# InternetMaximalism/plonky2_bn254

Measured on AMD Instinct MI355X. Metric: G1 scalar-mul STARK proofs/sec (256-bit scalars), higher is better.
Workload: dtype u64 (Goldilocks p = 2^64-2^32+1; BN254 Fq as 10x26-bit Montgomery limbs); 1 GPU; configs[1]: batch of 1024 G1 scalar-muls on 1 GPU per step = 8 proofs x 128 instances, 2^16 rows, W=781, standard_fast_config; instances_per_proof=128, steps_in_flight=4, parallelism=1 GPU, no collective

## Files before the change

### include/bn254_stark.h

```cpp
#ifndef BN254_STARK_H
#define BN254_STARK_H

#include <stddef.h>
#include <stdint.h>

#ifdef __cplusplus
extern "C" {
#endif

#define BN254S_ABI_VERSION 1

enum {
  BN254S_OK = 0,
  BN254S_E_INVALID_ARG = -1,
  BN254S_E_HIP = -2,
  BN254S_E_OOM = -3,
  BN254S_E_INVALID_POINT = -4,
  BN254S_E_UNSUPPORTED = -5,
  BN254S_E_TRANSCRIPT = -6,
  BN254S_E_INTERNAL = -7,
  BN254S_E_VERIFY = -8
};

typedef struct bn254s_ctx bn254s_ctx;
// ... 49 lines not shown
  BN254S_SEC_AUX_CAP = 1,
  BN254S_SEC_QUOTIENT_CAP = 2,
  BN254S_SEC_LOCAL_VALUES = 3,
  BN254S_SEC_NEXT_VALUES = 4,
  BN254S_SEC_AUX_POLYS = 5,
  BN254S_SEC_AUX_POLYS_NEXT = 6,
  BN254S_SEC_CTL_ZS_FIRST = 7,
  BN254S_SEC_QUOTIENT_POLYS = 8,
  BN254S_SEC_FRI_CAPS = 9,
  BN254S_SEC_QUERY_ROUNDS = 10,
  BN254S_SEC_FINAL_POLY = 11,
  BN254S_SEC_POW_WITNESS = 12,
  BN254S_SEC_INIT_CHALLENGER_STATE = 13,
  BN254S_SEC_COUNT = 14
};
int bn254s_proof_section(const bn254s_proof* p, int id, const uint64_t** data, size_t* len);
int bn254s_proof_degree_bits(const bn254s_proof* p);
int bn254s_proof_outputs(const bn254s_proof* p, const uint64_t** data, size_t* len);
int bn254s_proof_stage_ms(const bn254s_proof* p, const float** ms, size_t* n_stages);
const char* bn254s_stage_name(size_t stage);
size_t bn254s_proof_serialize(const bn254s_proof* p, uint8_t* buf, size_t cap);
void bn254s_proof_free(bn254s_proof* p);

int bn254s_verify(bn254s_ctx* ctx, int kind, const bn254s_params* params, uint32_t degree_bits, const uint64_t* words,
                  size_t n_words, const uint64_t* scalars, const uint64_t* x, const uint64_t* offset, const uint64_t* outputs,
                  size_t n);
int bn254s_verify_host(int kind, const bn254s_params* params, uint32_t degree_bits, const uint64_t* words, size_t n_words,
                       const uint64_t* scalars, const uint64_t* x, const uint64_t* offset, const uint64_t* outputs, size_t n,
                       char* err_buf, size_t err_cap);

int bn254s_verify_batch(bn254s_ctx* ctx, int kind, const bn254s_params* params, uint32_t degree_bits, const uint64_t* const* words,
                        size_t n_words, const uint64_t* scalars, const uint64_t* x, const uint64_t* offset, const uint64_t* outputs,
                        const size_t* n_jobs, size_t n_proofs, int32_t* status, char* err, size_t err_stride);

int bn254s_ctl_values(int kind, const uint64_t* scalars, const uint64_t* x, const uint64_t* offset, const uint64_t* outputs,
                      size_t n, uint64_t* in_rows, uint64_t* out_rows);

int bn254s_map_to_g2(bn254s_ctx* ctx, const bn254s_params* params, const uint64_t* u, const uint64_t* offsets, size_t n,
                     uint64_t* out_points, uint64_t* fq_jobs, uint64_t* g2_jobs, bn254s_proof** fq_proofs,
                     bn254s_proof** g2_proofs);

int bn254s_hash_to_fq2(const uint64_t* input, size_t len, uint64_t* out );
int bn254s_hash_to_fq2_batch(bn254s_ctx* ctx, const uint64_t* inputs, size_t n, size_t len, uint64_t* out);

int bn254s_g1_msm_chain(bn254s_ctx* ctx, const uint64_t* scalars , const uint64_t* x ,
                        const uint64_t* offset , size_t n, uint64_t* offsets_out, uint64_t* result );
int bn254s_g1_msm(bn254s_ctx* ctx, const bn254s_params* params, const uint64_t* scalars, const uint64_t* x,
                  const uint64_t* offset, size_t n, size_t per_proof, uint64_t* result, uint64_t* offsets_out,
                  bn254s_proof** proofs);
int bn254s_g2_msm_chain(bn254s_ctx* ctx, const uint64_t* scalars , const uint64_t* x ,
                        const uint64_t* offset , size_t n, uint64_t* offsets_out ,
                        uint64_t* result );
int bn254s_g2_msm(bn254s_ctx* ctx, const bn254s_params* params, const uint64_t* scalars, const uint64_t* x,
                  const uint64_t* offset, size_t n, size_t per_proof, uint64_t* result, uint64_t* offsets_out,
                  bn254s_proof** proofs);

int bn254s_g1_recover_from_x_batch(bn254s_ctx* ctx, const uint64_t* xs , size_t n,
                                   uint64_t* points_out , uint8_t* flags_out ,
                                   uint64_t* fq_jobs );
int bn254s_g1_recover_from_x(bn254s_ctx* ctx, const bn254s_params* params, const uint64_t* xs, size_t n, size_t per_proof,
                             uint64_t* points_out, uint8_t* flags_out, uint64_t* fq_jobs ,
                             bn254s_proof** fq_proofs);
int bn254s_g2_recover_from_x_batch(bn254s_ctx* ctx, const uint64_t* xs ,
                                   const uint8_t* sgns , size_t n,
                                   uint64_t* points_out , uint8_t* flags_out ,
                                   uint64_t* fq_jobs );
int bn254s_g2_recover_from_x(bn254s_ctx* ctx, const bn254s_params* params, const uint64_t* xs, const uint8_t* sgns, size_t n,
                             size_t per_proof, uint64_t* points_out, uint8_t* flags_out, uint64_t* fq_jobs ,
                             bn254s_proof** fq_proofs);
int bn254s_fq_sqrt_batch(bn254s_ctx* ctx, const uint64_t* xs ,
                         const uint8_t* sgns , size_t n, uint64_t* roots_out ,
                         uint8_t* square_out , uint8_t* root_ok_out ,
                         uint64_t* fq_jobs );
int bn254s_fq2_sqrt_batch(bn254s_ctx* ctx, const uint64_t* xs ,
                          const uint8_t* sgns , size_t n, uint64_t* roots_out ,
                          uint8_t* square_out , uint8_t* root_ok_out ,
                          uint64_t* fq_jobs );
int bn254s_fq_sqrt(bn254s_ctx* ctx, const bn254s_params* params, const uint64_t* xs, const uint8_t* sgns, size_t n, size_t per_proof,
                   uint64_t* roots_out, uint8_t* square_out, uint8_t* root_ok_out, uint64_t* fq_jobs ,
                   bn254s_proof** fq_proofs );
int bn254s_fq2_sqrt(bn254s_ctx* ctx, const bn254s_params* params, const uint64_t* xs, const uint8_t* sgns, size_t n, size_t per_proof,
                    uint64_t* roots_out, uint8_t* square_out, uint8_t* root_ok_out, uint64_t* fq_jobs ,
                    bn254s_proof** fq_proofs );
int bn254s_fq_inv_batch(bn254s_ctx* ctx, const uint64_t* xs , size_t n, uint64_t* out );
int bn254s_fq2_inv_batch(bn254s_ctx* ctx, const uint64_t* xs , size_t n, uint64_t* out );
int bn254s_g2_subgroup_check_batch(bn254s_ctx* ctx, const uint64_t* points , size_t n,
                                   uint8_t* flags_out );
int bn254s_g2_subgroup_check(bn254s_ctx* ctx, const bn254s_params* params, const uint64_t* points ,
                             const uint64_t* offsets , size_t n, size_t per_proof, uint8_t* flags_out ,
                             uint64_t* g2_jobs , bn254s_proof** g2_proofs);
int bn254s_g2_clear_cofactor_batch(bn254s_ctx* ctx, const uint64_t* points , size_t n,
                                   uint64_t* images_out , uint8_t* finite_out );
int bn254s_g2_clear_cofactor(bn254s_ctx* ctx, const bn254s_params* params, const uint64_t* points ,
                             const uint64_t* offsets , size_t n, size_t per_proof, uint64_t* images_out ,
                             uint8_t* finite_out , uint64_t* g2_jobs ,
                             bn254s_proof** g2_proofs);
int bn254s_map_to_g2_batch(bn254s_ctx* ctx, const uint64_t* u , size_t n,
                           uint64_t* out_points );
int bn254s_hash_to_g2_batch(bn254s_ctx* ctx, const uint64_t* inputs , size_t n, size_t len,
                            uint64_t* out_points );
int bn254s_hash_to_fq(const uint64_t* input, size_t len, uint64_t* out );
int bn254s_hash_to_fq_batch(bn254s_ctx* ctx, const uint64_t* inputs, size_t n, size_t len, uint64_t* out );
int bn254s_map_to_g1_batch(bn254s_ctx* ctx, const uint64_t* u , size_t n,
                           uint64_t* out_points , uint8_t* sq_flags ,
                           uint64_t* fq_jobs );
int bn254s_hash_to_g1_batch(bn254s_ctx* ctx, const uint64_t* inputs , size_t n, size_t len,
                            uint64_t* out_points );
int bn254s_map_to_g1(bn254s_ctx* ctx, const bn254s_params* params, const uint64_t* u , size_t n, size_t per_proof,
                     uint64_t* out_points , uint8_t* sq_flags ,
                     uint64_t* fq_jobs , bn254s_proof** fq_proofs );
int bn254s_job_outputs_batch(bn254s_ctx* ctx, int kind, const uint64_t* scalars , const uint64_t* x,
                             const uint64_t* offset, size_t n, uint64_t* outputs_out ,
                             uint8_t* finite_out );
int bn254s_job_outputs(bn254s_ctx* ctx, int kind, const bn254s_params* params, const uint64_t* scalars, const uint64_t* x,
                       const uint64_t* offset, size_t n, size_t per_proof, uint64_t* outputs_out, bn254s_proof** proofs_out);
#define BN254S_JOB_STEP_NONE 0xFFFFu
int bn254s_job_check_batch(bn254s_ctx* ctx, int kind, const uint64_t* scalars , const uint64_t* x, const uint64_t* offset,
                           size_t n, uint8_t* provable_out , uint16_t* step_out );
int bn254s_prove_batch_checked(bn254s_ctx* ctx, int kind, const bn254s_params* params, const uint64_t* scalars,
                               const uint64_t* x, const uint64_t* offset, size_t n_total, size_t per_proof,
                               uint8_t* provable_out , uint16_t* step_out ,
                               bn254s_proof** proofs_out);
int bn254s_commit_values(bn254s_ctx* ctx, const uint64_t* values, size_t ncols, uint64_t* coeffs, uint64_t* lde,
                         uint64_t* cap);
int bn254s_bench_ntt(bn254s_ctx* ctx, size_t ncols, int iters, float* ms);
int bn254s_bench_ntt_clock(bn254s_ctx* ctx, size_t ncols, int iters, float* ms, float* mhz, float* mhz_min);
int bn254s_bench_issue(bn254s_ctx* ctx, float* ns_per_issue, float* mhz);
int bn254s_bench_copy(bn254s_ctx* ctx, size_t words, int iters);
int bn254s_bench_leafhash(bn254s_ctx* ctx, size_t ncols, int log_leaves, int iters, float* ms);
int bn254s_poseidon_permute(bn254s_ctx* ctx, uint64_t* states, size_t n);
int bn254s_selftest_field(bn254s_ctx* ctx, const uint64_t* a, const uint64_t* b, size_t n, uint64_t* out);
int bn254s_selftest_poseidon(bn254s_ctx* ctx, int variant, uint64_t* states, size_t n);
int bn254s_selftest_leaf_hash(bn254s_ctx* ctx, const uint64_t* data, size_t ncols, int log_leaves, int kernel, int chunk_cols,
                              uint64_t* digests);
int bn254s_selftest_fq_inv(bn254s_ctx* ctx, const uint64_t* x, size_t n, uint64_t* out);
int bn254s_selftest_fq(bn254s_ctx* ctx, int group, const uint64_t* in, size_t n, uint64_t* out);
int bn254s_selftest_logup(bn254s_ctx* ctx, const uint64_t* trace, size_t rows, int ncols, int rc_begin, int n_rc, int table_col,
                          int freq_col, const uint64_t betas[2], uint64_t* out);
int bn254s_selftest_acc(bn254s_ctx* ctx, const uint64_t* values, const uint64_t* weights, size_t T, size_t rows, uint64_t* out);
int bn254s_selftest_openings(bn254s_ctx* ctx, const uint64_t* coeffs, int npolys, int log_r, const uint64_t zeta[2],
                             const uint64_t zeta_next[2], uint64_t* out);
int bn254s_selftest_fri_combine(bn254s_ctx* ctx, int mode, int W, int n_rc, int n_ctl, size_t n, const uint64_t* cols,
                                const uint64_t* aux_in, const uint64_t* points, uint64_t* out);
int bn254s_selftest_fri_fold(bn254s_ctx* ctx, const uint64_t* in, int log_m, uint64_t shift, const uint64_t beta[2], uint64_t* out);
int bn254s_selftest_fri_rows(bn254s_ctx* ctx, const uint64_t* lde, int ncols, int log_n, int h, size_t k0, size_t rows,
                             const uint32_t* indices, int nq, uint64_t* window, uint64_t* gathered);
#define BN254S_QS_WINDOW 1
#define BN254S_QS_RAW 2
#define BN254S_QS_MAX_PARTS 7
int bn254s_selftest_quotient(bn254s_ctx* ctx, int kind, int log_n, int flags, int h, size_t k0, size_t count, size_t stride,
                             const uint64_t* trace, const uint64_t* aux, const uint64_t alphas[2], const uint64_t betas[2],
                             const uint64_t gammas[2], const uint64_t* x, const uint64_t* lfirst, const uint64_t* llast, uint64_t* out,
                             uint64_t* part);
int bn254s_selftest_point_tables(bn254s_ctx* ctx, int log_n, int window, int h, size_t k0, size_t count, uint64_t* out);
int bn254s_selftest_aux(bn254s_ctx* ctx, int kind, const uint64_t* trace, size_t rows, const uint64_t betas[2], const uint64_t gammas[2],
                        uint64_t* out);
int bn254s_selftest_transforms(bn254s_ctx* ctx, int op, int log_n, int flags, int ncols, int coset_mask, const uint64_t* in,
                               uint64_t* out0, uint64_t* out1);
int bn254s_selftest_mul_2exp(bn254s_ctx* ctx, const uint64_t* x, size_t n, uint64_t* out);
int bn254s_selftest_outer_dft(bn254s_ctx* ctx, int log_r, int inverse, const uint64_t* in, size_t n, uint64_t* out);
#define BN254S_VERIFY_RECORD_HEAD 34
int bn254s_selftest_verify_front(int kind, const bn254s_params* params, uint32_t degree_bits, const uint64_t* words, size_t n_words,
                                 uint64_t* record_out, size_t record_cap);
int bn254s_selftest_query_round(bn254s_ctx* ctx, int kind, const bn254s_params* params, uint32_t degree_bits,
                                const uint64_t* const* words, size_t n_words, const uint64_t* records, size_t n_proofs,
                                size_t chunk_proofs, int32_t* codes_out);
const char* bn254s_selftest_query_text(int n_layers, int code);
int bn254s_selftest_verify_batch_ms(bn254s_ctx* ctx, float ms_out[5]);
#define BN254S_PLAN_WORDS 54
int bn254s_selftest_proof_plan(int kind, size_t n, const bn254s_params* params, uint64_t dev_total_bytes, int force_split,
                               int force_lowmem, int force_stream, int stream_win_log, uint64_t* out, char* err, size_t err_len);
int bn254s_generate_trace(bn254s_ctx* ctx, int kind, const uint64_t* scalars, const uint64_t* x, const uint64_t* offset,
                          size_t n, uint32_t min_rows_log2, uint64_t* trace_out, uint64_t* outputs);
int bn254s_g1_generate_trace(bn254s_ctx* ctx, const uint64_t* scalars, const uint64_t* x, const uint64_t* offset,
                             size_t n, uint32_t min_rows_log2, uint64_t* trace_out, uint64_t* outputs);

#ifdef __cplusplus
}
#endif
#endif
```

### plonky2_bn254_amd/csrc/proof_plan.h

```cpp
#pragma once
#include <string>
#include "aux.h"
#include "fri.h"
#include "ntt.h"

struct PlanOverrides {
  bool force_split = false, force_lowmem = false, force_stream = false;
  int stream_win_log = -1;
};
PlanOverrides plan_overrides_from_env();

struct PlanBuffers {
  size_t in, tvals, tcoef, hist, tmp, ldechunk, sponge, comb, tlde, trees, avals, acoef, alde, scratch, quot, tabs, open, fri,
      fritrees, qout;
  size_t win;
};

struct ProofPlan {
  static constexpr int NQ = 4, CAPW = 64;
  static constexpr int CH = 16;
  int kind = 0;
  size_t n = 0;
  bn254s_params P;
  StarkShape sh;
  int W = 0, A = 0, K = 0, PW = 0;
  size_t N = 0, M2 = 0;
  unsigned log_n = 0, log_m2 = 0;
  unsigned log_s = 0, log_r = 0;
  size_t R = 1, NH = 0;
  int NSPL = 1;
  bool stream = false, lowmem = false;
  unsigned log_bk = 0;
  size_t BK = 0, WROWS = 0;
  int L = 0, arities[FRI_MAX_LAYERS] = {0};
  size_t wpq = 0;
  size_t tree_words = 0, fri_words = 0, fri_tree_words = 0, in_words = 0;
  PlanBuffers words = {};
  size_t pinned_bytes = 0;
  size_t ntt_tmp_words(int width) const { return ntt_scratch_words(log_n, log_s != 0, lowmem ? CH : width); }
  size_t n_part() const { return (size_t)(W + A + NQ) * NSPL * R * 5; }
  size_t n_q() const { return wpq * P.num_queries; }
};

int proof_plan(int kind, size_t n, const bn254s_params& P, size_t dev_total_bytes, const PlanOverrides& ov, ProofPlan& pl,
               std::string& err);
size_t rows_for(size_t n, uint32_t min_rows_log2);
```

### plonky2_bn254_amd/csrc/proof_plan.hip

```cpp
#include <algorithm>
#include <cstdlib>
#include <cstring>
#include "proof_plan.h"
#include "merkle.h"
#include "prover.h"

static bool env_flag(const char* name) { return getenv(name) && atoi(getenv(name)); }
PlanOverrides plan_overrides_from_env() {
  PlanOverrides ov;
  ov.force_split = env_flag("BN254S_FORCE_SPLIT");
  ov.force_lowmem = env_flag("BN254S_FORCE_LOWMEM");
  ov.force_stream = env_flag("BN254S_FORCE_STREAM");
  if (const char* e = getenv("BN254S_STREAM_WIN_LOG")) ov.stream_win_log = atoi(e) < 0 ? 99 : atoi(e);
  return ov;
}

size_t rows_for(size_t n, uint32_t min_rows_log2) {
  size_t r = std::max((size_t)1 << min_rows_log2, n * 512), p = 1;
  while (p < r) p <<= 1;
  return p;
}

int proof_plan(int kind, size_t n, const bn254s_params& P, size_t dev_total_bytes, const PlanOverrides& ov, ProofPlan& pl,
               std::string& err) {
  const StarkKind& sk = stark_kind(kind);
  pl.kind = kind;
  pl.n = n;
  pl.P = P;
  const StarkShape& sh = pl.sh = sk.shape;
  const int W = pl.W = sh.W, A = pl.A = sh.n_aux(), K = pl.K = sh.n_total_constraints(), PW = pl.PW = sk.point_words;
  const int NQ = ProofPlan::NQ, CH = ProofPlan::CH;
  const size_t N = pl.N = rows_for(n, P.min_rows_log2);
  unsigned log_n = 0;
  while (((size_t)1 << log_n) < N) log_n++;
  pl.log_n = log_n;
  if (log_n < 16 || log_n > 23) {
    err = "supported trace heights: 2^16 .. 2^23 rows (up to 16384 instances in one proof)";
    return BN254S_E_UNSUPPORTED;
  }
  if (P.num_challenges != 2 || P.rate_bits != 1 || P.cap_height != 4 || P.arity_bits != 4 || P.min_rows_log2 < 16 ||
      P.pow_bits == 0 || P.pow_bits > 32 || P.num_queries == 0 || P.num_queries > 256) {
    err = "unsupported StarkConfig (only standard_fast_config shapes)";
    return BN254S_E_UNSUPPORTED;
  }
  const unsigned log_s = pl.log_s = (log_n == 23 || (ov.force_split && log_n >= 18)) ? 1 : 0;
  const unsigned log_m2 = pl.log_m2 = log_n + 1, log_r = pl.log_r = log_n - 16 - log_s;
  const size_t R = pl.R = (size_t)1 << log_r;
  const size_t M2 = pl.M2 = 2 * N;
  pl.NH = N >> log_s;
  const int NSPL = pl.NSPL = 1 << log_s;
  const double plain_bytes = 8.0 * (double)N * (4.0 * sh.W + 4.0 * sh.n_aux() + std::max(sh.W, sh.n_aux()));
  const double compact_bytes = 8.0 * ((double)std::max((size_t)sh.W * N, (size_t)sh.n_aux() * 2 * N) + (double)sh.W * N * 3.0 + (double)sh.n_aux() * N);
  const bool stream = pl.stream =
      log_n > 16 && (ov.force_stream || (dev_total_bytes > 0 && compact_bytes + 20e9 > (double)dev_total_bytes));
  const bool lowmem = pl.lowmem = stream || log_s || (log_n > 16 && (ov.force_lowmem || plain_bytes > 200e9));
  pl.log_bk = std::min(22u, log_n - 1);
  if (ov.stream_win_log >= 0) pl.log_bk = std::min(log_n, std::max(8u, (unsigned)ov.stream_win_log));
  pl.BK = (size_t)1 << pl.log_bk;
  const size_t WROWS = pl.WROWS = pl.BK + 1;
  const std::vector<int> arities = fri_arities(P, log_n);
  const int L = pl.L = (int)arities.size();
  if (L > FRI_MAX_LAYERS) return BN254S_E_UNSUPPORTED;
  std::copy(arities.begin(), arities.end(), pl.arities);

  PlanBuffers& b = pl.words = PlanBuffers{};
  pl.in_words = n * (4 + 2 * (size_t)PW);
  b.in = pl.in_words + 16;
  b.tvals = lowmem && !stream ? std::max((size_t)W * N, (size_t)A * M2) : (size_t)W * N;
  b.tcoef = (size_t)W * N;
  b.hist = 65536 / 2;
  b.tmp = pl.ntt_tmp_words(std::max(W, A));
  b.ldechunk = stream ? (size_t)CH * M2 : 0;
  b.sponge = stream ? (size_t)12 * M2 : 0;
  b.comb = (size_t)6 * N + (size_t)6 * M2;
  b.tlde = stream ? 0 : (size_t)W * M2;
  pl.tree_words = merkle_tree_digests(log_m2, P.cap_height) * 4;
  b.trees = 3 * pl.tree_words;
  b.avals = (size_t)A * N;
  b.acoef = lowmem ? 0 : (size_t)A * N;
  b.alde = lowmem ? 0 : (size_t)A * M2;
  b.scratch = std::max(sk.trace_scratch_words(n), aux_scratch_words(sh, N));
  b.quot = (size_t)(3 * NQ) * N + (size_t)NQ * M2 + (size_t)QUOTIENT_MAX_PARTS * 2 * (stream ? WROWS : M2);
  b.tabs = QUOTIENT_W_WORDS(K) + QUOTIENT_MZT_WORDS + 4 * (size_t)(W + A + NQ);
  b.open = std::max((size_t)(W + A + NQ) * NSPL * R * 5 + FRI_OPENING_TABLE_WORDS, n * (size_t)PW);
  pl.fri_words = pl.fri_tree_words = 0;
  {
    size_t m = M2;
    for (int l = 0; l <= L; l++) {
      pl.fri_words += 2 * m;
      if (l < L) pl.fri_tree_words += merkle_tree_digests((int)log_m2 - 4 * (l + 1), P.cap_height) * 4;
      m >>= 4;
    }
  }
  b.fri = pl.fri_words;
  b.fritrees = pl.fri_tree_words;
  pl.wpq = (size_t)(W + A + NQ) + 3 * 4 * (log_m2 - P.cap_height);
  {
    int lg = log_m2;
    for (int l = 0; l < L; l++) {
      lg -= arities[l];
      pl.wpq += 32 + 4 * (lg - P.cap_height);
    }
  }
  b.qout = pl.n_q() + 64;
  b.win = stream ? (size_t)(W + A) * WROWS + 3 * WROWS + (size_t)(W + A) * P.num_queries : 0;
  pl.pinned_bytes = std::max(pl.n_part(), pl.n_q()) * 8;
  return BN254S_OK;
}

extern "C" int bn254s_selftest_proof_plan(int kind, size_t n, const bn254s_params* params, uint64_t dev_total_bytes, int force_split,
                                          int force_lowmem, int force_stream, int stream_win_log, uint64_t* out, char* err,
                                          size_t err_len) {
  if (kind < 0 || kind > 2 || n == 0 || !params || params->struct_size != sizeof(bn254s_params) || !out) return BN254S_E_INVALID_ARG;
  PlanOverrides ov;
  ov.force_split = force_split != 0;
  ov.force_lowmem = force_lowmem != 0;
  ov.force_stream = force_stream != 0;
  ov.stream_win_log = stream_win_log;
  ProofPlan pl;
  std::string msg;
  const int rc = proof_plan(kind, n, *params, (size_t)dev_total_bytes, ov, pl, msg);
  if (err && err_len) {
    strncpy(err, msg.c_str(), err_len - 1);
    err[err_len - 1] = 0;
  }
  if (rc != BN254S_OK) return rc;
  const PlanBuffers& b = pl.words;
  const uint64_t head[] = {(uint64_t)pl.kind, pl.n, (uint64_t)pl.W, (uint64_t)pl.A, (uint64_t)pl.K, (uint64_t)pl.PW, pl.N, pl.log_n, pl.log_s,
                           pl.log_r, pl.R, pl.NH, (uint64_t)pl.NSPL, pl.stream, pl.lowmem, pl.log_bk, pl.BK, pl.WROWS, (uint64_t)pl.L};
  const uint64_t tail[] = {pl.wpq, pl.tree_words, pl.fri_words, pl.fri_tree_words, pl.in_words,
                           b.in, b.tvals, b.tcoef, b.hist, b.tmp, b.ldechunk, b.sponge, b.comb, b.tlde, b.trees, b.avals, b.acoef,
                           b.alde, b.scratch, b.quot, b.tabs, b.open, b.fri, b.fritrees, b.qout, b.win, pl.pinned_bytes};
  static_assert(sizeof(head) / 8 + FRI_MAX_LAYERS + sizeof(tail) / 8 == BN254S_PLAN_WORDS, "bn254s_selftest_proof_plan layout");
  for (uint64_t v : head) *out++ = v;
  for (int l = 0; l < FRI_MAX_LAYERS; l++) *out++ = (uint64_t)pl.arities[l];
  for (uint64_t v : tail) *out++ = v;
  return BN254S_OK;
}
```

### plonky2_bn254_amd/csrc/prover.hip

```cpp
#include <algorithm>
#include <atomic>
#include <cstring>
#include <thread>
#include "ctx.h"
#include "trace.h"
#include "aux.h"
#include "merkle.h"
#include "quotient.h"
#include "fri.h"
#include "transcript.h"
#include "prover.h"
#include "proof_plan.h"
#include "transforms.h"

template <class L>
static StarkShape make_shape(bool input_has_a, int n_constraints) {
  StarkShape s;
  s.W = L::W;
  s.rc_begin = L::RC_BEGIN;
  s.rc_end = L::RC_END;
  s.table_col = L::RANGE;
  s.freq_col = L::FREQ;
  s.n_ctl = 2;
  s.n_constraints = n_constraints;
  memset(&s.ctl, 0, sizeof(s.ctl));
  int m = 0;
  for (int i = 0; i < L::PL; i++, m++) { s.ctl.col_start[0][m] = L::B + i; s.ctl.col_bits[0][m] = 1; }
  if (input_has_a)
    for (int i = 0; i < L::PL; i++, m++) { s.ctl.col_start[0][m] = L::A + i; s.ctl.col_bits[0][m] = 1; }
  for (int k = 0; k < 16; k++, m++) { s.ctl.col_start[0][m] = L::BITS + 16 * k; s.ctl.col_bits[0][m] = 16; }
  s.ctl.col_start[0][m] = L::TIMESTAMP; s.ctl.col_bits[0][m] = 1; m++;
  s.ctl.ncols[0] = m;
  s.ctl.filter_col[0] = L::FLAGS + 0;
  m = 0;
  for (int i = 0; i < L::PL; i++, m++) { s.ctl.col_start[1][m] = L::SUM + i; s.ctl.col_bits[1][m] = 1; }
  s.ctl.col_start[1][m] = L::TIMESTAMP; s.ctl.col_bits[1][m] = 1; m++;
  s.ctl.ncols[1] = m;
  s.ctl.filter_col[1] = L::FLAGS + 1;
  return s;
}
static int fq_generate_trace_no_offset(const u64* d_scalars, const u64* d_x, const u64*, size_t n, u64* d_trace, size_t N,
                                       u64* d_scratch, u64* d_outputs, int* d_err, hipStream_t st, bool with_range) {
  return fq_generate_trace_device(d_scalars, d_x, n, d_trace, N, d_scratch, d_outputs, d_err, st, with_range);
}
const StarkKind& stark_kind(int kind) {
  static const StarkKind kinds[3] = {
      {make_shape<G1L>(true, 1111), 8, true, g1_trace_scratch_words, g1_generate_trace_device, g1_quotient_mz_blocks, g1_quotient_launch},
      {make_shape<G2L>(true, 1693), 16, true, g2_trace_scratch_words, g2_generate_trace_device, g2_quotient_mz_blocks, g2_quotient_launch},
      {make_shape<FQL>(false, 770), 4, false, fq_trace_scratch_words, fq_generate_trace_no_offset, fq_quotient_mz_blocks, fq_quotient_launch}};
  return kinds[kind];
}

enum { ST_TRACE = 0, ST_TRACE_NTT, ST_TRACE_MERKLE, ST_AUX, ST_AUX_NTT, ST_AUX_MERKLE, ST_QUOTIENT, ST_QUOTIENT_COMMIT,
       ST_OPENINGS, ST_FRI, ST_TOTAL, ST_COUNT };
static const char* STAGE_NAMES[ST_COUNT] = {"trace_gen", "trace_ntt", "trace_merkle", "aux_columns", "aux_ntt", "aux_merkle",
                                            "quotient", "quotient_commit", "openings", "fri", "total"};

struct bn254s_proof {
  std::vector<u64> words, outputs;
  size_t sec_off[BN254S_SEC_COUNT + 1] = {0};
  int degree_bits = 0;
  float stage_ms[ST_COUNT] = {0};
};

std::vector<int> fri_arities(const bn254s_params& P, int degree_bits) {
  std::vector<int> a;
  int d = degree_bits;
  while (d > (int)P.final_poly_bits && d + (int)P.rate_bits - (int)P.arity_bits >= (int)P.cap_height) {
    a.push_back(P.arity_bits);
    d -= P.arity_bits;
  }
  return a;
}

__global__ __launch_bounds__(256) void k_quotient_chunks(const u64* __restrict__ ab, u64* __restrict__ out, size_t N, u64 inv2,
                                                         u64 inv2c) {
  size_t i = (size_t)blockIdx.x * blockDim.x + threadIdx.x;
  if (i >= N) return;
  int a = blockIdx.y;
  u64 A = ab[(size_t)(a * 2 + 0) * N + i], B = ab[(size_t)(a * 2 + 1) * N + i];
  out[(size_t)(a * 2 + 0) * N + i] = gl_mul(gl_add(A, B), inv2);
  out[(size_t)(a * 2 + 1) * N + i] = gl_mul(gl_sub(A, B), inv2c);
}

#define CHK(call)                                              \
  do {                                                         \
    hipError_t e_ = (call);                                    \
    if (e_ != hipSuccess) {                                    \
      err = std::string(#call) + ": " + hipGetErrorString(e_); \
      return BN254S_E_HIP;                                     \
    }                                                          \
  } while (0)

struct BigSection {
  bn254s_ctx* c;
  hipStream_t st;
  int cls;
  BigSection(bn254s_ctx* c_, hipStream_t st_, int cls_) : c(c_), st(st_), cls(cls_) { c->big_lock(cls); }
  ~BigSection() {
    hipStreamSynchronize(st);
    c->big_unlock(cls);
  }
};

static int get_point_tables(bn254s_ctx* c, unsigned log_n, QPointTables& pt) {
  static std::mutex mu;
  std::lock_guard<std::mutex> lk(mu);
  std::string key = "pt." + std::to_string(log_n);
  bool fresh = !c->has(key);
  size_t M2 = (size_t)2 << log_n;
  u64* p = c->words(key, 3 * M2);
  if (!p) return BN254S_E_OOM;
  if (fresh) {
    quotient_point_tables(p, p + M2, p + 2 * M2, log_n, c->stream);
    if (hipStreamSynchronize(c->stream) != hipSuccess) return BN254S_E_HIP;
  }
  pt.x = p;
  pt.lfirst = p + M2;
  pt.llast = p + 2 * M2;
  return 0;
}

struct Workspace {
  Slot* sl = nullptr;
  const ProofPlan* pl = nullptr;
  u64 *in, *tvals, *tcoef, *hist, *tmp, *ldechunk, *sponge, *comb, *tlde, *trees, *avals, *acoef, *alde, *scr, *quot, *tabs, *open,
      *fri, *fritrees, *qout;
  int* err;
  unsigned long long* pow;
  u32* qidx;
  u64 *ttree, *atree, *qtree;
  u64 *qv, *ab, *qcoef, *qlde, *qpart;
  u64 *W, *mzt, *apow;
  size_t cap_off;
  u64 *tw = nullptr, *aw = nullptr, *wpt = nullptr, *qrows = nullptr;
  int begin_windows(std::string& err);
};

static int workspace_acquire(Slot& sl, const ProofPlan& pl, Workspace& ws, std::string& err) {
  BufPool& mem = sl.mem;
  const PlanBuffers& b = pl.words;
  const bool stream = pl.stream, lowmem = pl.lowmem;
  ws.sl = &sl;
  ws.pl = &pl;
  if (lowmem) {
    mem.drop("acoef");
    mem.drop("alde");
  }
  ws.in = mem.words("in", b.in);
  ws.tvals = mem.words("tvals", b.tvals);
  ws.tcoef = mem.words("tcoef", b.tcoef);
  ws.hist = mem.words("hist", b.hist);
  ws.tmp = mem.words("tmp", b.tmp);
  mem.drop("win");
  if (stream) {
    mem.drop("tlde");
    mem.drop("alde");
    mem.drop("acoef");
  } else {
    mem.drop("ldechunk");
    mem.drop("sponge");
  }
  ws.ldechunk = stream ? mem.words("ldechunk", b.ldechunk) : nullptr;
  ws.sponge = stream ? mem.words("sponge", b.sponge) : nullptr;
  ws.comb = mem.words("comb", b.comb);
  ws.tlde = stream ? ws.ldechunk : mem.words("tlde", b.tlde);
  ws.trees = mem.words("trees", b.trees);
  ws.avals = mem.words("avals", b.avals);
  ws.acoef = lowmem ? ws.avals : mem.words("acoef", b.acoef);
  ws.alde = stream ? ws.ldechunk : lowmem ? ws.tvals : mem.words("alde", b.alde);
  ws.scr = mem.words("scratch", b.scratch);
  ws.quot = mem.words("quot", b.quot);
  ws.tabs = mem.words("tabs", b.tabs);
  ws.open = mem.words("open", b.open);
  ws.fri = mem.words("fri", b.fri);
  ws.fritrees = mem.words("fritrees", b.fritrees);
  ws.qout = mem.words("qout", b.qout);
  if (sl.pinned_bytes < pl.pinned_bytes) {
    if (sl.pinned) hipHostFree(sl.pinned);
    sl.pinned = nullptr;
    sl.pinned_bytes = 0;
    CHK(hipHostMalloc(&sl.pinned, pl.pinned_bytes));
    sl.pinned_bytes = pl.pinned_bytes;
  }
  if (!ws.hist || !ws.in || !ws.tvals || !ws.tcoef || !ws.tmp || !ws.tlde || !ws.trees || !ws.avals || !ws.acoef || !ws.alde ||
      !ws.scr || !ws.quot || !ws.tabs || !ws.open || !ws.fri || !ws.fritrees || !ws.qout || !ws.comb ||
      (stream && (!ws.ldechunk || !ws.sponge))) {
    err = mem.err;
    mem.release();
    return BN254S_E_OOM;
  }
  {
    static const size_t reserve = (size_t)(getenv("BN254S_MEM_RESERVE_MB") ? atol(getenv("BN254S_MEM_RESERVE_MB")) : 6144) << 20;
    size_t free_b = 0, total_b = 0;
    if (hipMemGetInfo(&free_b, &total_b) == hipSuccess && free_b < reserve) {
      err = "device memory: " + std::to_string(free_b >> 20) + " MB would be left free, below the reserve of " +
            std::to_string(reserve >> 20) + " MB kept for the runtime's own allocations";
      mem.release();
      return BN254S_E_OOM;
    }
  }
  const size_t N = pl.N, M2 = pl.M2;
  const int NQ = ProofPlan::NQ;
  ws.err = (int*)(ws.in + pl.in_words);
  ws.pow = (unsigned long long*)(ws.in + pl.in_words + 2);
  ws.qidx = (u32*)(ws.qout + pl.n_q());
  ws.ttree = ws.trees;
  ws.atree = ws.trees + pl.tree_words;
  ws.qtree = ws.trees + 2 * pl.tree_words;
  ws.qv = ws.quot;
  ws.ab = ws.quot + (size_t)NQ * N;
  ws.qcoef = ws.quot + (size_t)2 * NQ * N;
  ws.qlde = ws.quot + (size_t)3 * NQ * N;
  ws.qpart = ws.qlde + (size_t)NQ * M2;
  ws.W = ws.tabs;
  ws.mzt = ws.tabs + QUOTIENT_W_WORDS(pl.K);
  ws.apow = ws.mzt + QUOTIENT_MZT_WORDS;
  ws.cap_off = 4 * merkle_level_offset(pl.log_m2, pl.log_m2 - pl.P.cap_height);
  return BN254S_OK;
}

int Workspace::begin_windows(std::string& err) {
  BufPool& mem = sl->mem;
  const size_t WROWS = pl->WROWS;
  CHK(hipStreamSynchronize(sl->st));
  mem.drop("tvals");
  tvals = nullptr;
  u64* win = mem.words("win", pl->words.win);
  if (!win) {
    err = mem.err;
    mem.release();
    return BN254S_E_OOM;
  }
  tw = win;
  aw = win + (size_t)pl->W * WROWS;
  wpt = aw + (size_t)pl->A * WROWS;
  qrows = wpt + 3 * WROWS;
  return BN254S_OK;
}

struct Run {
  bn254s_ctx* c;
  Slot& sl;
  hipStream_t st;
  const ProofPlan& pl;
  Workspace& ws;
  const Transforms& tf;
  QPointTables pt;
  void sb(int stage) const { hipEventRecord(sl.events[2 * stage], st); }
  void se(int stage) const { hipEventRecord(sl.events[2 * stage + 1], st); }
  int mmode() const { return c->workers.in_flight.load(std::memory_order_relaxed) >= 4 ? MERKLE_THROUGHPUT : MERKLE_LATENCY; }
};

static int upload_and_generate(const StarkKind& sk, const u64* scalars, const u64* x, const u64* off, size_t n, u64* d_in, u64* d_trace,
                               size_t N, u64* d_scr, u64* d_outs, int* d_err, hipStream_t st, bool with_range, std::string& err) {
  const size_t PW = sk.point_words;
  u64* d_sc = d_in;
  u64* d_x = d_in + 4 * n;
  u64* d_off = d_x + PW * n;
  CHK(hipMemcpyAsync(d_sc, scalars, n * 32, hipMemcpyHostToDevice, st));
  CHK(hipMemcpyAsync(d_x, x, n * PW * 8, hipMemcpyHostToDevice, st));
  if (sk.has_offset) CHK(hipMemcpyAsync(d_off, off, n * PW * 8, hipMemcpyHostToDevice, st));
  if (sk.generate_trace(d_sc, d_x, d_off, n, d_trace, N, d_scr, d_outs, d_err, st, with_range)) {
    err = "trace generation launch failed";
    return BN254S_E_HIP;
  }
  return BN254S_OK;
}

static int stage_trace(const Run& r, const u64* scalars, const u64* x, const u64* off, bn254s_proof* pr, int* h_err, std::string& err) {
  const ProofPlan& pl = r.pl;
  const Workspace& ws = r.ws;
  const StarkShape& sh = pl.sh;
  hipStream_t st = r.st;
  r.sb(ST_TRACE);
  CHK(hipMemsetAsync(ws.err, 0, 16, st));
  u64* d_outs = ws.open;
  if (int rc = upload_and_generate(stark_kind(pl.kind), scalars, x, off, pl.n, ws.in, ws.tvals, pl.N, ws.scr, d_outs, ws.err, st, false, err))
    return rc;
  {
    BigSection big(r.c, st, BIG_EXCL);
    launch_range_columns(ws.tvals, pl.N, sh.rc_begin, sh.rc_end, sh.freq_col, sh.table_col, (u32*)ws.hist, ws.err, st);
  }
  pr->outputs.resize(pl.n * (size_t)pl.PW);
  CHK(hipMemcpyAsync(pr->outputs.data(), d_outs, pl.n * (size_t)pl.PW * 8, hipMemcpyDeviceToHost, st));
  CHK(hipMemcpyAsync(h_err, ws.err, 4, hipMemcpyDeviceToHost, st));
  r.se(ST_TRACE);
  return BN254S_OK;
}

static void hash_sections(const Run& r, const u64* lde, int width, u64* tree, int stage) {
  bn254s_ctx* c = r.c;
  const size_t M2 = r.pl.M2;
  const int S = r.pl.log_n == 16 ? c->hash_split : 1;
  if (S <= 1) {
    BigSection big(c, r.st, BIG_HASH);
    r.sb(stage);
    merkle_leaves(lde, 1, M2, width, r.pl.log_m2, tree, r.st);
    return;
  }
  const size_t cnt = M2 / S;
  for (int k = 0; k < S; k++) {
    BigSection big(c, r.st, BIG_HASH_PART);
    if (k == 0) r.sb(stage);
    merkle_leaves_range(lde, 1, M2, width, (size_t)k * cnt, cnt, tree, r.st);
  }
}

static int commit(const Run& r, const u64* vals, u64* coef, u64* lde, int width, u64* tree, int ntt_stage, int merkle_stage,
                  u64* cap_out, std::string& err) {
  const ProofPlan& pl = r.pl;
  hipStream_t st = r.st;
  if (pl.stream) {
    BigSection big(r.c, st, BIG_NTT);
    r.sb(ntt_stage);
    r.tf.commit_stream(vals, coef, width, tree);
    r.se(ntt_stage);
    r.sb(merkle_stage);
  } else {
    {
      BigSection big(r.c, st, BIG_NTT);
      r.sb(ntt_stage);
      r.tf.commit_ntt(vals, coef, lde, width);
      r.se(ntt_stage);
    }
    hash_sections(r, lde, width, tree, merkle_stage);
  }
  merkle_upper(pl.log_m2, pl.P.cap_height, tree, st, r.mmode());
  CHK(hipMemcpyAsync(cap_out, tree + r.ws.cap_off, ProofPlan::CAPW * 8, hipMemcpyDeviceToHost, st));
  r.se(merkle_stage);
  CHK(hipStreamSynchronize(st));
  return BN254S_OK;
}

static void stage_aux(const Run& r, const u64 betas[2], const u64 gammas[2]) {
  BigSection big(r.c, r.st, BIG_EXCL);
  r.sb(ST_AUX);
  aux_build(r.pl.sh, r.ws.tvals, r.pl.N, betas, gammas, r.ws.avals, r.ws.scr, r.ws.err, r.st);
  r.se(ST_AUX);
}

static void quotient_over_windows(const Run& r, const u64 betas[2], const u64 gammas[2]) {
  const ProofPlan& pl = r.pl;
  const Workspace& ws = r.ws;
  hipStream_t st = r.st;
  const size_t N = pl.N, M2 = pl.M2, BK = pl.BK, WROWS = pl.WROWS;
  BigSection big(r.c, st, BIG_NTT);
  r.sb(ST_QUOTIENT);
  QPointTables wpt;
  wpt.x = ws.wpt;
  wpt.lfirst = ws.wpt + WROWS;
  wpt.llast = ws.wpt + 2 * WROWS;
  for (int h = 0; h < 2; h++)
    for (size_t k0 = 0; k0 < N; k0 += BK) {
      r.tf.for_lde_chunks(ws.tcoef, pl.W, 1 << h, [&](int c0, int cn) {
        fri_extract_window(ws.ldechunk, M2, pl.log_n, h, k0, WROWS, cn, ws.tw + (size_t)c0 * WROWS, st);
      });
      r.tf.for_lde_chunks(ws.acoef, pl.A, 1 << h, [&](int c0, int cn) {
        fri_extract_window(ws.ldechunk, M2, pl.log_n, h, k0, WROWS, cn, ws.aw + (size_t)c0 * WROWS, st);
      });
      quotient_point_tables_window(ws.wpt, ws.wpt + WROWS, ws.wpt + 2 * WROWS, pl.log_n, h, k0, WROWS, st);
      QArgs QA;
      quotient_fill_args(QA, pl.sh, nullptr, nullptr, ws.W, ws.mzt, r.pt, betas, gammas, pl.log_n, ws.qv, ws.qpart);
      quotient_window_args(QA, ws.tw, ws.aw, wpt, ws.qpart, WROWS, BK, k0, h);
      stark_kind(pl.kind).quotient_launch(QA, pl.sh, st);
    }
}

static int stage_quotient(const Run& r, const u64 alphas[2], const u64 betas[2], const u64 gammas[2], u64* cap_out, std::string& err) {
  const ProofPlan& pl = r.pl;
  const Workspace& ws = r.ws;
  const StarkKind& sk = stark_kind(pl.kind);
  hipStream_t st = r.st;
  const size_t N = pl.N;
  {
    std::vector<u64> hW, hmzt;
    const int* mz_e0 = nullptr;
    const int nblk = sk.mz_blocks(&mz_e0);
    quotient_host_tables(pl.K, alphas, mz_e0, nblk, hW, hmzt);
    CHK(hipMemcpyAsync(ws.W, hW.data(), hW.size() * 8, hipMemcpyHostToDevice, st));
    CHK(hipMemcpyAsync(ws.mzt, hmzt.data(), hmzt.size() * 8, hipMemcpyHostToDevice, st));
    CHK(hipStreamSynchronize(st));
  }
  if (pl.stream) {
    quotient_over_windows(r, betas, gammas);
  } else {
    BigSection big(r.c, st, BIG_EXCL);
    r.sb(ST_QUOTIENT);
    QArgs QA;
    quotient_fill_args(QA, pl.sh, ws.tlde, ws.alde, ws.W, ws.mzt, r.pt, betas, gammas, pl.log_n, ws.qv, ws.qpart);
    sk.quotient_launch(QA, pl.sh, st);
  }
  r.tf.quotient_coset_inverse(ws.qv, ws.ab);
  {
    u64 gn = gl_pow(GL_GEN, N);
    u64 inv2 = gl_inv(2), inv2c = gl_inv(gl_mul(2, gn));
    dim3 g((unsigned)((N + 255) / 256), 2);
    k_quotient_chunks<<<g, 256, 0, st>>>(ws.ab, ws.qcoef, N, inv2, inv2c);
  }
  r.se(ST_QUOTIENT);
  r.sb(ST_QUOTIENT_COMMIT);
  r.tf.lde(ws.qcoef, ws.qlde, ProofPlan::NQ);
  merkle_build(ws.qlde, 1, pl.M2, ProofPlan::NQ, pl.log_m2, pl.P.cap_height, ws.qtree, st, r.mmode());
  CHK(hipMemcpyAsync(cap_out, ws.qtree + ws.cap_off, ProofPlan::CAPW * 8, hipMemcpyDeviceToHost, st));
  r.se(ST_QUOTIENT_COMMIT);
  CHK(hipStreamSynchronize(st));
  return BN254S_OK;
}

static int stage_openings(const Run& r, gl2 zeta, gl2 zeta_next, u64* h_part, std::string& err) {
  const ProofPlan& pl = r.pl;
  const Workspace& ws = r.ws;
  hipStream_t st = r.st;
  const int W = pl.W, A = pl.A, NQ = ProofPlan::NQ, NSPL = pl.NSPL;
  const size_t R = pl.R, NH = pl.NH;
  {
    BigSection big(r.c, st, BIG_EXCL);
    r.sb(ST_OPENINGS);
    u64* d_otab = ws.open + pl.n_part();
    fri_opening_tables(pl.log_r, pl.log_s ? gl2_mul(zeta, zeta) : zeta, pl.log_s ? gl2_mul(zeta_next, zeta_next) : zeta_next, d_otab, st);
    fri_openings(ws.tcoef, NH, pl.log_r, W * NSPL, d_otab, ws.open, st);
    fri_openings(ws.acoef, NH, pl.log_r, A * NSPL, d_otab, ws.open + (size_t)W * NSPL * R * 5, st);
    fri_openings(ws.qcoef, NH, pl.log_r, NQ * NSPL, d_otab, ws.open + (size_t)(W + A) * NSPL * R * 5, st);
  }
  CHK(hipMemcpyAsync(h_part, ws.open, pl.n_part() * 8, hipMemcpyDeviceToHost, st));
  r.se(ST_OPENINGS);
  CHK(hipStreamSynchronize(st));
  return BN254S_OK;
}

static std::vector<u64> recombine_openings(const ProofPlan& pl, const u64* h_part, gl2 zeta, gl2 zeta_next) {
  const size_t R = pl.R;
  const int NSPL = pl.NSPL, n_polys = pl.W + pl.A + ProofPlan::NQ;
  std::vector<u64> h_open((size_t)n_polys * 5);
  std::vector<gl2> zp0(R), zp1(R);
  gl2 a = gl2_make(1, 0), b = gl2_make(1, 0);
  const gl2 y0 = pl.log_s ? gl2_mul(zeta, zeta) : zeta, y1 = pl.log_s ? gl2_mul(zeta_next, zeta_next) : zeta_next;
  for (size_t k1 = 0; k1 < R; k1++) {
    zp0[k1] = a;
    zp1[k1] = b;
    a = gl2_mul(a, y0);
    b = gl2_mul(b, y1);
  }
  for (int p = 0; p < n_polys; p++) {
    gl2 v0 = gl2_make(0, 0), v1 = gl2_make(0, 0);
    u64 s1 = 0;
    for (int half = 0; half < NSPL; half++) {
      gl2 e0 = gl2_make(0, 0), e1 = gl2_make(0, 0);
      for (size_t k1 = 0; k1 < R; k1++) {
        const u64* q = &h_part[(((size_t)p * NSPL + half) * R + k1) * 5];
        e0 = gl2_add(e0, gl2_mul(zp0[k1], gl2_make(q[0], q[1])));
        e1 = gl2_add(e1, gl2_mul(zp1[k1], gl2_make(q[2], q[3])));
        s1 = gl_add(s1, q[4]);
      }
      v0 = gl2_add(v0, half ? gl2_mul(zeta, e0) : e0);
      v1 = gl2_add(v1, half ? gl2_mul(zeta_next, e1) : e1);
    }
    u64* o5 = &h_open[(size_t)p * 5];
    o5[0] = v0.c0; o5[1] = v0.c1; o5[2] = v1.c0; o5[3] = v1.c1; o5[4] = s1;
  }
  return h_open;
}

struct Openings {
  const ProofPlan& pl;
  const std::vector<u64>& h_open;
  u64 operator()(int p, int k) const { return h_open[(size_t)p * 5 + k]; }
  int n_ctlz() const { return 2 * pl.sh.n_ctl; }
  u64 ctl_z_first(int i) const { return (*this)(pl.W + pl.sh.n_lookup_cols() + i, 4); }
};

static void observe_openings(Challenger& ch, const Openings& op) {
  const int W = op.pl.W, A = op.pl.A, NQ = ProofPlan::NQ;
  for (int p = 0; p < W + A + NQ; p++) {
    ch.observe(op(p, 0));
    ch.observe(op(p, 1));
  }
  for (int p = 0; p < W + A; p++) {
    ch.observe(op(p, 2));
    ch.observe(op(p, 3));
  }
  for (int i = 0; i < op.n_ctlz(); i++) {
    ch.observe(op.ctl_z_first(i));
    ch.observe(0);
  }
}

struct FriAlphaPowers {
  std::vector<u32> apow;
  gl2 r0, r1, r2;
};
static FriAlphaPowers fri_alpha_powers(const Openings& op, gl2 fri_alpha) {
  const int W = op.pl.W, A = op.pl.A, NQ = ProofPlan::NQ, n_ctlz = op.n_ctlz();
  FriAlphaPowers f;
  f.apow.assign(8 * (size_t)(W + A + NQ), 0);
  gl2 ap = gl2_make(1, 0);
  f.r0 = f.r1 = f.r2 = gl2_make(0, 0);
  for (int p = 0; p < W + A + NQ; p++) {
    fri_weight_record(&f.apow[8 * (size_t)p], ap);
    f.r0 = gl2_add(f.r0, gl2_mul(ap, gl2_make(op(p, 0), op(p, 1))));
    if (p < W + A) f.r1 = gl2_add(f.r1, gl2_mul(ap, gl2_make(op(p, 2), op(p, 3))));
    if (p < n_ctlz) f.r2 = gl2_add(f.r2, gl2_mul_base(ap, op.ctl_z_first(p)));
    ap = gl2_mul(ap, fri_alpha);
  }
  return f;
}

static int stage_fri_combine(const Run& r, const FriAlphaPowers& f, gl2 zeta, gl2 zeta_next, gl2 fri_alpha, std::string& err) {
  const ProofPlan& pl = r.pl;
  const Workspace& ws = r.ws;
  hipStream_t st = r.st;
  CHK(hipMemcpyAsync(ws.apow, f.apow.data(), f.apow.size() * 4, hipMemcpyHostToDevice, st));
  CHK(hipStreamSynchronize(st));
  BigSection big(r.c, st, BIG_EXCL);
  r.sb(ST_FRI);
  fri_combine_coeffs(pl.sh, ws.tcoef, ws.acoef, ws.qcoef, ws.apow, pl.N, ws.comb, st);
  r.tf.lde(ws.comb, ws.comb + (size_t)6 * pl.N, 6);
  fri_combine_final(pl.sh, ws.comb + (size_t)6 * pl.N, r.pt.x, zeta, zeta_next, f.r0, f.r1, f.r2, fri_alpha, pl.M2, ws.fri, st);
  return BN254S_OK;
}

struct FriLayers {
  std::vector<std::vector<u64>> caps;
  std::vector<const u64*> vals, trees;
  const u64* last = nullptr;
  u64 shift = GL_GEN;
  unsigned lm = 0;
};

static int stage_fri_commit(const Run& r, Challenger& ch, FriLayers& fl, std::string& err) {
  const ProofPlan& pl = r.pl;
  hipStream_t st = r.st;
  const int L = pl.L, CAPW = ProofPlan::CAPW;
  fl.caps.assign(L, std::vector<u64>(CAPW));
  fl.vals.resize(L);
  fl.trees.resize(L);
  u64* vals = r.ws.fri;
  u64* ftree = r.ws.fritrees;
  fl.shift = GL_GEN;
  unsigned lm = pl.log_m2;
  const u64 inv16 = gl_inv(16);
  for (int l = 0; l < L; l++) {
    const int lg = (int)lm - 4;
// ... 535 lines not shown
```

### plonky2_bn254_amd/csrc/quotient.h

```cpp
#pragma once
#include <vector>
#include "quotient_sched.h"

void quotient_point_tables(u64* d_x, u64* d_lfirst, u64* d_llast, unsigned log_n, hipStream_t st);
void quotient_point_tables_window(u64* d_x, u64* d_lfirst, u64* d_llast, unsigned log_n, int h, size_t k0, size_t count, hipStream_t st);
void quotient_window_args(QArgs& A, const u64* d_tw, const u64* d_aw, const QPointTables& pt, u64* d_part, size_t stride, size_t count,
                          size_t k0, int h);
int g1_quotient_mz_blocks(const int** e0);
int g2_quotient_mz_blocks(const int** e0);
int fq_quotient_mz_blocks(const int** e0);
void g1_quotient_launch(const QArgs& A, const StarkShape& sh, hipStream_t st);
void g2_quotient_launch(const QArgs& A, const StarkShape& sh, hipStream_t st);
void fq_quotient_launch(const QArgs& A, const StarkShape& sh, hipStream_t st);
```

### plonky2_bn254_amd/csrc/quotient_common.h

```cpp
#pragma once
#include "gl_dev.h"
#include "aux.h"

struct Acc {
  u64 lo, hi;
  u32 ov;
};
__device__ __forceinline__ void acc_init(Acc& a) {
  a.lo = 0;
  a.hi = 0;
  a.ov = 0;
}
__device__ __forceinline__ void acc_mad(Acc& a, u64 x, u64 w) {
  const unsigned __int128 pr = (unsigned __int128)x * w;
  u64 pl = (u64)pr, ph = (u64)(pr >> 64);
  a.lo += pl;
  u64 c = a.lo < pl ? 1 : 0;
  u64 h = a.hi + ph;
  u32 o = h < ph ? 1 : 0;
  h += c;
  o += h < c ? 1 : 0;
  a.hi = h;
  a.ov += o;
}
__device__ __forceinline__ u64 acc_red(const Acc& a) {
  return gl_sub(gl_reduce128(a.lo, a.hi), ((u64)a.ov) << 32);
}
struct Acc2 {
  Acc a0, a1;
};
__device__ __forceinline__ void acc2_init(Acc2& a) {
  acc_init(a.a0);
  acc_init(a.a1);
}
__device__ __forceinline__ void acc2_mad(Acc2& a, u64 x, u64 w0, u64 w1) {
  acc_mad(a.a0, x, w0);
  acc_mad(a.a1, x, w1);
}

static constexpr u32 M22 = (1u << 22) - 1;
struct W3 {
  u32 w0, w1, w2;
};
GL_HD W3 w3_split(u64 w) {
  W3 r;
  r.w0 = (u32)w & M22;
  r.w1 = (u32)(w >> 22) & M22;
  r.w2 = (u32)(w >> 44);
  return r;
}
struct Acc3 {
  u64 c[5];
};
__device__ __forceinline__ void acc3_init(Acc3& a) {
#pragma unroll
  for (int k = 0; k < 5; k++) a.c[k] = 0;
}
__device__ __forceinline__ void acc3_mad(Acc3& a, u32 v0, u32 v1, u32 v2, u32 w0, u32 w1, u32 w2) {
  a.c[0] += (u64)v0 * w0;
  a.c[1] += (u64)v0 * w1;
  a.c[1] += (u64)v1 * w0;
  a.c[2] += (u64)v0 * w2;
  a.c[2] += (u64)v1 * w1;
  a.c[2] += (u64)v2 * w0;
  a.c[3] += (u64)v1 * w2;
  a.c[3] += (u64)v2 * w1;
  a.c[4] += (u64)v2 * w2;
}
__device__ __forceinline__ u64 acc3_red(const Acc3& a) {
  unsigned __int128 t = (unsigned __int128)a.c[0] + ((unsigned __int128)a.c[1] << 22) + ((unsigned __int128)a.c[2] << 44);
  u64 r = gl_reduce128((u64)t, (u64)(t >> 64));
  r = gl_add(r, gl_mul_2exp<66>(gl_reduce128(a.c[3], 0)));
  r = gl_add(r, gl_mul_2exp<88>(gl_reduce128(a.c[4], 0)));
  return r;
}

struct AccW {
  Acc3 a0, a1;
};
__device__ __forceinline__ void accw_init(AccW& a) {
  acc3_init(a.a0);
  acc3_init(a.a1);
}
template <class WP>
__device__ __forceinline__ void accw_mad(AccW& a, u64 x, WP w) {
  const u32 v0 = (u32)x & M22, v1 = (u32)(x >> 22) & M22, v2 = (u32)(x >> 44);
  acc3_mad(a.a0, v0, v1, v2, w[0], w[1], w[2]);
  acc3_mad(a.a1, v0, v1, v2, w[4], w[5], w[6]);
}
GL_HD void w3_store(u64* dst , u64 wa, u64 wb) {
  const W3 a = w3_split(wa), b = w3_split(wb);
  dst[0] = (u64)a.w0 | ((u64)a.w1 << 32);
  dst[1] = (u64)a.w2;
  dst[2] = (u64)b.w0 | ((u64)b.w1 << 32);
  dst[3] = (u64)b.w2;
}

struct QPointTables {
  const u64* x;
  const u64* lfirst;
  const u64* llast;
};

__device__ __forceinline__ size_t next_position(size_t j, unsigned log_n) {
  const size_t N = (size_t)1 << log_n;
  size_t h = j >> log_n;
  u32 k = bitrev32((u32)(j & (N - 1)), log_n);
  k = (k + 1) & (u32)(N - 1);
  return (h << log_n) | bitrev32(k, log_n);
}

__device__ __forceinline__ void lookup_and_ctl_constraints(const StarkShape& sh, const u64* __restrict__ tl,
                                                           const u64* __restrict__ al, size_t M2, size_t j, size_t jn,
                                                           const u32* __restrict__ W3 , int e0,
                                                           const u64 betas[2], const u64 gammas[2], u64 lfirst, u64 llast,
                                                           u64 z_last, u64& tot0, u64& tot1) {
  const int m = sh.n_helpers(), n_rc = sh.n_rc();
  int e = e0;
  AccW acc;
  accw_init(acc);
  const u64 table = tl[(size_t)sh.table_col * M2 + j], freq = tl[(size_t)sh.freq_col * M2 + j];
  u64 hs[2] = {0, 0};
#pragma unroll 4
  for (int k = 0; k < m; k++) {
    u64 f0 = tl[(size_t)(sh.rc_begin + 2 * k) * M2 + j];
    bool two = (2 * k + 1) < n_rc;
    u64 f1 = two ? tl[(size_t)(sh.rc_begin + 2 * k + 1) * M2 + j] : 0;
#pragma unroll
    for (int ch = 0; ch < 2; ch++) {
      u64 h = al[(size_t)(ch * (m + 1) + k) * M2 + j];
      u64 g0 = gl_add(f0, betas[ch]);
      u64 c;
      if (two) {
        u64 g1 = gl_add(f1, betas[ch]);
        c = gl_sub(gl_sub(gl_mul(gl_mul(g1, g0), h), g1), g0);
      } else {
        c = gl_sub(gl_mul(g0, h), 1);
      }
      int ee = e0 + ch * (m + 2) + k;
      accw_mad(acc, c, W3 + 8 * (ee));
      hs[ch] = gl_add(hs[ch], h);
    }
  }
#pragma unroll
  for (int ch = 0; ch < 2; ch++) {
    u64 z = al[(size_t)(ch * (m + 1) + m) * M2 + j], nz = al[(size_t)(ch * (m + 1) + m) * M2 + jn];
    u64 twc = gl_add(table, betas[ch]);
    u64 y = gl_sub(gl_mul(hs[ch], twc), freq);
    int ee = e0 + ch * (m + 2) + m;
    accw_mad(acc, gl_mul(z, lfirst), W3 + 8 * (ee));
    accw_mad(acc, gl_sub(gl_mul(gl_sub(nz, z), twc), y), W3 + 8 * (ee + 1));
  }
  e = e0 + 2 * (m + 2);
  for (int ctl = 0; ctl < sh.n_ctl; ctl++) {
    u64 a0 = 0, a1 = 0;
    for (int mm = sh.ctl.ncols[ctl] - 1; mm >= 0; mm--) {
      int start = sh.ctl.col_start[ctl][mm], nb = sh.ctl.col_bits[ctl][mm];
      u64 v = 0;
      for (int b = nb - 1; b >= 0; b--) v = gl_add(gl_dbl(v), tl[(size_t)(start + b) * M2 + j]);
      a0 = gl_add(gl_mul(a0, betas[0]), v);
      a1 = gl_add(gl_mul(a1, betas[1]), v);
    }
    u64 comb[2] = {gl_add(a0, gammas[0]), gl_add(a1, gammas[1])};
    u64 f0 = tl[(size_t)sh.ctl.filter_col[ctl] * M2 + j];
#pragma unroll
    for (int ch = 0; ch < 2; ch++) {
      int zc = 2 * (m + 1) + ctl * 2 + ch;
      u64 lz = al[(size_t)zc * M2 + j], nz = al[(size_t)zc * M2 + jn];
      u64 c_last = gl_mul(gl_sub(gl_mul(comb[ch], lz), f0), llast);
      u64 c_tr = gl_mul(gl_sub(gl_mul(comb[ch], gl_sub(lz, nz)), f0), z_last);
      accw_mad(acc, c_last, W3 + 8 * (e));
      accw_mad(acc, c_tr, W3 + 8 * (e + 1));
      e += 2;
    }
  }
  tot0 = gl_add(tot0, acc3_red(acc.a0));
  tot1 = gl_add(tot1, acc3_red(acc.a1));
}
```

### plonky2_bn254_amd/csrc/quotient_g1.hip

```cpp
#include "quotient_sched.h"
#include "quotient.h"

static constexpr int G1_K_AIR = 1111;
static constexpr int G1_MZ_E0[5] = {0, 50, 83, 132, 165};

template <int part>
__device__ __forceinline__ void g1_add_part(const QArgs& A, size_t j) {
  const size_t M2 = A.stride;
  const u64* __restrict__ tl = A.tl;
  const qc64 W0 = QCONST(u64, A.W);
  const qc64 W1 = QCONST(u64, A.W + A.K);
  const qc32 W3 = QCONST(u32, A.W + 2 * (size_t)A.K);
  u64 tot0 = 0, tot1 = 0;
  int e = 0;
  const int AUX = G1L::AUX;
  const u64 filter = TL(G1L::FILTER);
  const u64 is_x_eq_filter = TL(AUX + G1_AUX_IS_X_EQ_FILTER);
  u64 ax[16], lam[16], t16[16], u16[16];
  ld16(tl, M2, j, G1L::A, ax);
  if constexpr (part == 0) {
    const u64 is_x_eq = TL(AUX + G1_AUX_IS_X_EQ);
    ld16(tl, M2, j, G1L::B, u16);
#pragma unroll
    for (int i = 0; i < 16; i++) u16[i] = gl_sub(u16[i], ax[i]);
    ld16(tl, M2, j, AUX + G1_AUX_IS_X_EQ_AUX, t16);
    const u64 c0 = gl_sub(is_x_eq, 1);
    mz_block<true>(tl, M2, j, AUX + G1_AUX_IS_X_EQ_AUX + 16, A, G1_MZ_E0[0], 0,
             filter, [&](int i) __attribute__((always_inline)) { u64 v = conv16<true>(u16, t16, i); return i == 0 ? gl_add(v, c0) : v; }, tot0, tot1);
    e = 33;
    AccW g;
    accw_init(g);
#pragma unroll
    for (int i = 0; i < 16; i++) accw_mad(g, u16[i], W3 + 8 * (e + i));
    e += 16;
    u64 f = gl_mul(filter, is_x_eq);
    tot0 = gl_add(tot0, gl_mul(f, acc3_red(g.a0)));
    tot1 = gl_add(tot1, gl_mul(f, acc3_red(g.a1)));
    EMIT(gl_sub(gl_mul(filter, is_x_eq), is_x_eq_filter));
  } else if constexpr (part == 1) {
    ld16(tl, M2, j, AUX + G1_AUX_LAMBDA, lam);
    ld16(tl, M2, j, G1L::B, u16);
#pragma unroll
    for (int i = 0; i < 16; i++) u16[i] = gl_sub(u16[i], ax[i]);
    ld16(tl, M2, j, G1L::B + 16, t16);
    ld16(tl, M2, j, G1L::A + 16, ax);
#pragma unroll
    for (int i = 0; i < 16; i++) t16[i] = gl_sub(t16[i], ax[i]);
    mz_block<true>(tl, M2, j, AUX + G1_AUX_LAMBDA_AUX, A, G1_MZ_E0[1], 1,
             gl_sub(filter, is_x_eq_filter),
             [&](int i) __attribute__((always_inline)) {
               u64 v = conv16<true>(lam, u16, i);
               return i < 16 ? gl_sub(v, t16[i < 16 ? i : 0]) : v;
             },
             tot0, tot1);
  } else if constexpr (part == 2) {
    ld16(tl, M2, j, AUX + G1_AUX_LAMBDA, lam);
    ld16(tl, M2, j, G1L::A + 16, u16);
    mz_block<true>(tl, M2, j, AUX + G1_AUX_LAMBDA_AUX, A, G1_MZ_E0[2], 2,
             is_x_eq_filter,
             [&](int i) __attribute__((always_inline)) {
               u64 ly = conv16<true>(lam, u16, i), xx = conv16<true>(ax, ax, i);
               return gl_sub(gl_dbl(ly), gl_add(gl_dbl(xx), xx));
             },
             tot0, tot1);
    e = 116;
    ld16(tl, M2, j, G1L::B + 16, t16);
    AccW g;
    accw_init(g);
#pragma unroll
    for (int i = 0; i < 16; i++) accw_mad(g, gl_sub(u16[i], t16[i]), W3 + 8 * (e + i));
    tot0 = gl_add(tot0, gl_mul(is_x_eq_filter, acc3_red(g.a0)));
    tot1 = gl_add(tot1, gl_mul(is_x_eq_filter, acc3_red(g.a1)));
  } else if constexpr (part == 3) {
    ld16(tl, M2, j, AUX + G1_AUX_LAMBDA, lam);
    ld16(tl, M2, j, G1L::B, t16);
    ld16(tl, M2, j, G1L::C, u16);
#pragma unroll
    for (int i = 0; i < 16; i++) ax[i] = gl_add(gl_add(ax[i], t16[i]), u16[i]);
    mz_block<true>(tl, M2, j, AUX + G1_AUX_X_AUX, A, G1_MZ_E0[3], 3, filter,
             [&](int i) __attribute__((always_inline)) {
               u64 v = conv16<true>(lam, lam, i);
               return i < 16 ? gl_sub(v, ax[i < 16 ? i : 0]) : v;
             },
             tot0, tot1);
  } else {
    ld16(tl, M2, j, AUX + G1_AUX_LAMBDA, lam);
    ld16(tl, M2, j, G1L::C, u16);
#pragma unroll
    for (int i = 0; i < 16; i++) u16[i] = gl_sub(u16[i], ax[i]);
    ld16(tl, M2, j, G1L::C + 16, t16);
    ld16(tl, M2, j, G1L::A + 16, ax);
#pragma unroll
    for (int i = 0; i < 16; i++) t16[i] = gl_add(t16[i], ax[i]);
    mz_block<true>(tl, M2, j, AUX + G1_AUX_Y_AUX, A, G1_MZ_E0[4], 4, filter,
             [&](int i) __attribute__((always_inline)) {
               u64 v = conv16<true>(lam, u16, i);
               return i < 16 ? gl_add(v, t16[i < 16 ? i : 0]) : v;
             },
             tot0, tot1);
  }
  store_part(A, part, j, tot0, tot1);
}

__global__ __launch_bounds__(256, 2) void k_quotient_g1_parts(QArgs A) {
  const size_t j = (size_t)blockIdx.x * blockDim.x + threadIdx.x;
  if (j >= A.count) return;
  switch (blockIdx.y) {
    case 0: schedule_part<G1L, false>(A, j, q_next(A, j), 198, 5); break;
    case 1: g1_add_part<0>(A, j); break;
    case 2: g1_add_part<1>(A, j); break;
    case 3: g1_add_part<2>(A, j); break;
    case 4: g1_add_part<3>(A, j); break;
    default: g1_add_part<4>(A, j); break;
  }
}

__global__ __launch_bounds__(256) void k_quotient_finish(QArgs A, StarkShape sh) {
  const size_t j = (size_t)blockIdx.x * blockDim.x + threadIdx.x;
  if (j >= A.count) return;
  finish_point(A, sh, j);
}
void quotient_finish_launch(const QArgs& A, const StarkShape& sh, hipStream_t st) {
  k_quotient_finish<<<(unsigned)((A.count + 255) / 256), 256, 0, st>>>(A, sh);
}

__global__ void k_point_tables(u64* x, u64* lfirst, u64* llast, unsigned log_n, u64 w_n, u64 w_2n) {
  const size_t N = (size_t)1 << log_n;
  size_t j = (size_t)blockIdx.x * blockDim.x + threadIdx.x;
  if (j >= 2 * N) return;
  size_t h = j >> log_n;
  u32 k = bitrev32((u32)(j & (N - 1)), log_n);
  u64 shift = h ? gl_mul(GL_GEN, w_2n) : GL_GEN;
  u64 xv = gl_mul(shift, gl_pow(w_n, k));
  u64 gn = gl_pow(GL_GEN, N);
  u64 zh = gl_sub(h ? gl_neg(gn) : gn, 1);
  u64 ninv = gl_inv((u64)N % GL_P);
  u64 winv = gl_inv(w_n);
  x[j] = xv;
  lfirst[j] = gl_mul(gl_mul(zh, ninv), gl_inv(gl_sub(xv, 1)));
  llast[j] = gl_mul(gl_mul(gl_mul(zh, ninv), winv), gl_inv(gl_sub(xv, winv)));
}

__global__ void k_point_tables_window(u64* x, u64* lfirst, u64* llast, unsigned log_n, u32 h, size_t k0, size_t count, u64 w_n,
                                      u64 w_2n) {
  const size_t N = (size_t)1 << log_n;
  size_t j = (size_t)blockIdx.x * blockDim.x + threadIdx.x;
  if (j >= count) return;
  const u64 k = (k0 + j) & (N - 1);
  u64 shift = h ? gl_mul(GL_GEN, w_2n) : GL_GEN;
  u64 xv = gl_mul(shift, gl_pow(w_n, k));
  u64 gn = gl_pow(GL_GEN, N);
  u64 zh = gl_sub(h ? gl_neg(gn) : gn, 1);
  u64 ninv = gl_inv((u64)N % GL_P);
  u64 winv = gl_inv(w_n);
  x[j] = xv;
  lfirst[j] = gl_mul(gl_mul(zh, ninv), gl_inv(gl_sub(xv, 1)));
  llast[j] = gl_mul(gl_mul(gl_mul(zh, ninv), winv), gl_inv(gl_sub(xv, winv)));
}
void quotient_point_tables_window(u64* d_x, u64* d_lfirst, u64* d_llast, unsigned log_n, int h, size_t k0, size_t count, hipStream_t st) {
  k_point_tables_window<<<(unsigned)((count + 255) / 256), 256, 0, st>>>(d_x, d_lfirst, d_llast, log_n, (u32)h, k0, count,
                                                                       gl_root_of_unity(log_n), gl_root_of_unity(log_n + 1));
}
void quotient_window_args(QArgs& A, const u64* d_tw, const u64* d_aw, const QPointTables& pt, u64* d_part, size_t stride, size_t count,
                          size_t k0, int h) {
  A.tl = d_tw;
  A.al = d_aw;
  A.pt = pt;
  A.part = d_part;
  A.stride = stride;
  A.count = count;
  A.k0 = k0;
  A.natural = 1;
  A.hsel = (u32)h;
}

void quotient_point_tables(u64* d_x, u64* d_lfirst, u64* d_llast, unsigned log_n, hipStream_t st) {
  size_t M2 = (size_t)2 << log_n;
  k_point_tables<<<(unsigned)((M2 + 255) / 256), 256, 0, st>>>(d_x, d_lfirst, d_llast, log_n, gl_root_of_unity(log_n),
                                                             gl_root_of_unity(log_n + 1));
}

void quotient_host_tables(int K, const u64 alphas[2], const int* mz_e0, int n_blocks, std::vector<u64>& W, std::vector<u64>& mzt) {
  W.assign(QUOTIENT_W_WORDS(K), 0);
  for (int a = 0; a < 2; a++) {
    u64 v = 1;
    for (int e = K - 1; e >= 0; e--) {
      W[(size_t)a * K + e] = v;
      v = gl_mul(v, alphas[a]);
    }
  }
  static const u64 MOD[16] = {64839, 55420, 35862, 15392, 51853, 26737, 27281, 38785,
                              22621, 33153, 17846, 47184, 41001, 57649, 20082, 12388};
  const u64 B = 1ULL << 16, OFF = 1ULL << 29;
  mzt.assign(QUOTIENT_MZT_WORDS, 0);
  for (int blk = 0; blk < n_blocks; blk++)
    for (int a = 0; a < 2; a++) {
      const u64* w = &W[(size_t)a * K + mz_e0[blk] + 1];
      u64* T = &mzt[(size_t)(blk * 2 + a) * 80];
      for (int jj = 0; jj < 17; jj++) {
        u64 s = 0;
        for (int t = 0; t < 16; t++)
          if (jj + t < 32) s = gl_add(s, gl_mul(w[jj + t], MOD[t]));
        T[jj] = s;
      }
      u64 usum = 0;
      for (int d = 0; d < 31; d++) {
        u64 u = gl_sub(w[d + 1], gl_mul(B, w[d]));
        T[17 + d] = u;
        T[48 + d] = gl_mul(B, u);
        usum = gl_add(usum, u);
      }
      T[79] = gl_mul(OFF, usum);
    }
  for (int e = 0; e < K; e++) w3_store(&W[2 * (size_t)K + 4 * (size_t)e], W[e], W[(size_t)K + e]);
  for (int blk = 0; blk < n_blocks; blk++)
    for (int t = 0; t < 80; t++)
      w3_store(&mzt[QUOTIENT_MZT3_OFF + (size_t)(blk * 80 + t) * 4], mzt[(size_t)(blk * 2) * 80 + t], mzt[(size_t)(blk * 2 + 1) * 80 + t]);
}

void quotient_fill_args(QArgs& A, const StarkShape& sh, const u64* d_tl, const u64* d_al, const u64* d_W, const u64* d_mzt,
                        const QPointTables& pt, const u64 betas[2], const u64 gammas[2], unsigned log_n, u64* d_out,
                        u64* d_part) {
  A.tl = d_tl;
  A.al = d_al;
  A.W = d_W;
  A.mzt = d_mzt;
  A.pt = pt;
  for (int i = 0; i < 2; i++) {
    A.betas[i] = betas[i];
    A.gammas[i] = gammas[i];
  }
  const size_t N = (size_t)1 << log_n;
  u64 gn = gl_pow(GL_GEN, N);
  A.zh_inv[0] = gl_inv(gl_sub(gn, 1));
  A.zh_inv[1] = gl_inv(gl_sub(gl_neg(gn), 1));
  A.w_inv = gl_inv(gl_root_of_unity(log_n));
  A.out = d_out;
  A.part = d_part;
  A.n_parts = 0;
  A.log_n = log_n;
  A.K = sh.n_total_constraints();
  A.stride = A.count = 2 * N;
  A.k0 = 0;
  A.natural = 0;
  A.hsel = 0;
}

int g1_quotient_mz_blocks(const int** e0) {
  *e0 = G1_MZ_E0;
  return 5;
}
void g1_quotient_launch(const QArgs& A0, const StarkShape& sh, hipStream_t st) {
  QArgs A = A0;
  A.n_parts = 6;
  const unsigned g = (unsigned)((A.count + 255) / 256);
  k_quotient_g1_parts<<<dim3(g, 6), 256, 0, st>>>(A);
  quotient_finish_launch(A, sh, st);
}

void quotient_g1_module_warm() {
  hipFuncAttributes a;
  (void)hipFuncGetAttributes(&a, reinterpret_cast<const void*>(&k_point_tables));
}
```

### plonky2_bn254_amd/csrc/quotient_g2fq.hip

```cpp
#include "quotient_sched.h"
#include "quotient.h"

static constexpr int G2_MZ_E0[10] = {1, 50, 100, 133, 166, 199, 264, 297, 330, 363};
static constexpr int FQ_MZ_E0[1] = {0};

__device__ __forceinline__ u64 econv_c0(const u64* x0, const u64* x1, const u64* y0, const u64* y1, int i) {
  return gl_sub(conv16(x0, y0, i), conv16(x1, y1, i));
}
__device__ __forceinline__ u64 econv_c1(const u64* x0, const u64* x1, const u64* y0, const u64* y1, int i) {
  return gl_add(conv16(x0, y1, i), conv16(x1, y0, i));
}

#define MZB(blk, auxcol, FILTER, FN, ...) \
  mz_block(tl, M2, j, (auxcol), A, G2_MZ_E0[blk], (blk), (FILTER), FN, tot0, tot1, ##__VA_ARGS__)

__global__ __launch_bounds__(256, 2) void k_quotient_g2_sched(QArgs A) {
  const size_t j = (size_t)blockIdx.x * blockDim.x + threadIdx.x;
  if (j >= A.count) return;
  schedule_part<G2L, false>(A, j, q_next(A, j), 396, 6);
}

template <int part>
__global__ __launch_bounds__(256, 2) void k_quotient_g2_add(QArgs A) {
  typedef G2L L;
  const size_t M2 = A.stride;
  const size_t j = (size_t)blockIdx.x * blockDim.x + threadIdx.x;
  if (j >= A.count) return;
  const u64* __restrict__ tl = A.tl;
  const qc64 W0 = QCONST(u64, A.W);
  const qc64 W1 = QCONST(u64, A.W + A.K);
  const qc32 W3 = QCONST(u32, A.W + 2 * (size_t)A.K);
  u64 tot0 = 0, tot1 = 0;
  int e = 0;
  const u64 filter = TL(L::FILTER);
  const int AUX = L::AUX;
  u64 is_x_eq_filter = 0;
  if constexpr (part == 1 || part == 2) is_x_eq_filter = TL(AUX + G2_AUX_IS_X_EQ_FILTER);
  auto seed_w = [&](Acc2& sd, int blk, int i, u64 v) { acc2_mad(sd, v, W0[G2_MZ_E0[blk] + 1 + i], W1[G2_MZ_E0[blk] + 1 + i]); };
  if constexpr (part == 0 || part == 5) {
    constexpr int h = part == 0 ? 0 : 1;
    u64 dx[16], t0[16];
    const u64 z = TL(AUX + (h ? G2_AUX_IS_C1_ZERO : G2_AUX_IS_C0_ZERO));
    if constexpr (h == 0) {
      EMIT(gl_mul(filter, gl_sub(gl_mul(z, TL(AUX + G2_AUX_IS_C1_ZERO)), TL(AUX + G2_AUX_IS_X_EQ))));
    }
#pragma unroll
    for (int i = 0; i < 16; i++) dx[i] = gl_sub(TL(L::B + 16 * h + i), TL(L::A + 16 * h + i));
    ld16(tl, M2, j, AUX + (h ? G2_AUX_C1_AUX : G2_AUX_C0_AUX), t0);
    const u64 c0 = gl_sub(z, 1);
    MZB(h, AUX + (h ? G2_AUX_C1_AUX : G2_AUX_C0_AUX) + 16, filter, [&](int i) __attribute__((always_inline)) { u64 v = conv16(dx, t0, i); return i == 0 ? gl_add(v, c0) : v; });
    e = h ? 83 : 34;
    AccW g;
    accw_init(g);
#pragma unroll
    for (int i = 0; i < 16; i++) accw_mad(g, dx[i], W3 + 8 * (e + i));
    const u64 f = gl_mul(filter, z);
    tot0 = gl_add(tot0, gl_mul(f, acc3_red(g.a0)));
    tot1 = gl_add(tot1, gl_mul(f, acc3_red(g.a1)));
    if constexpr (h == 1) {
      e = 99;
      EMIT(gl_sub(gl_mul(filter, TL(AUX + G2_AUX_IS_X_EQ)), TL(AUX + G2_AUX_IS_X_EQ_FILTER)));
    }
  } else {
    Acc2 sd0, sd1;
    acc2_init(sd0);
    acc2_init(sd1);
    u64 l0[16], l1[16], dx0[16], dx1[16];
    if constexpr (part == 1) {
#pragma unroll 4
      for (int i = 0; i < 16; i++) seed_w(sd0, 2, i, gl_sub(TL(L::A + 32 + i), TL(L::B + 32 + i)));
      ld16(tl, M2, j, AUX + G2_AUX_LAMBDA, l0);
      ld16(tl, M2, j, AUX + G2_AUX_LAMBDA + 16, l1);
#pragma unroll
      for (int i = 0; i < 16; i++) {
        dx0[i] = gl_sub(TL(L::B + i), TL(L::A + i));
        dx1[i] = gl_sub(TL(L::B + 16 + i), TL(L::A + 16 + i));
      }
      const u64 f_ne = gl_sub(filter, is_x_eq_filter);
      MZB(2, AUX + G2_AUX_LAMBDA_AUX, f_ne, [&](int i) __attribute__((always_inline)) { return econv_c0(l0, l1, dx0, dx1, i); }, &sd0);
#pragma unroll 4
      for (int i = 0; i < 16; i++) seed_w(sd1, 3, i, gl_sub(TL(L::A + 48 + i), TL(L::B + 48 + i)));
      MZB(3, AUX + G2_AUX_LAMBDA_AUX + 80, f_ne, [&](int i) __attribute__((always_inline)) { return econv_c1(l0, l1, dx0, dx1, i); }, &sd1);
    } else if constexpr (part == 2) {
      ld16(tl, M2, j, L::A, dx0);
      ld16(tl, M2, j, L::A + 16, dx1);
#pragma unroll
      for (int i = 0; i < 31; i++) {
        const u64 xx0 = econv_c0(dx0, dx1, dx0, dx1, i), xx1 = econv_c1(dx0, dx1, dx0, dx1, i);
        seed_w(sd0, 4, i, gl_neg(gl_add(gl_dbl(xx0), xx0)));
        seed_w(sd1, 5, i, gl_neg(gl_add(gl_dbl(xx1), xx1)));
      }
      ld16(tl, M2, j, AUX + G2_AUX_LAMBDA, l0);
      ld16(tl, M2, j, AUX + G2_AUX_LAMBDA + 16, l1);
      ld16(tl, M2, j, L::A + 32, dx0);
      ld16(tl, M2, j, L::A + 48, dx1);
      MZB(4, AUX + G2_AUX_LAMBDA_AUX, is_x_eq_filter, [&](int i) __attribute__((always_inline)) { return gl_dbl(econv_c0(l0, l1, dx0, dx1, i)); }, &sd0);
      MZB(5, AUX + G2_AUX_LAMBDA_AUX + 80, is_x_eq_filter, [&](int i) __attribute__((always_inline)) { return gl_dbl(econv_c1(l0, l1, dx0, dx1, i)); }, &sd1);
      e = 232;
      AccW g;
      accw_init(g);
#pragma unroll
      for (int i = 0; i < 16; i++) accw_mad(g, gl_sub(dx0[i], TL(L::B + 32 + i)), W3 + 8 * (e + i));
#pragma unroll
      for (int i = 0; i < 16; i++) accw_mad(g, gl_sub(dx1[i], TL(L::B + 48 + i)), W3 + 8 * (e + 16 + i));
      tot0 = gl_add(tot0, gl_mul(is_x_eq_filter, acc3_red(g.a0)));
      tot1 = gl_add(tot1, gl_mul(is_x_eq_filter, acc3_red(g.a1)));
    } else if constexpr (part == 3) {
#pragma unroll 4
      for (int i = 0; i < 16; i++) {
        seed_w(sd0, 6, i, gl_neg(gl_add(gl_add(TL(L::A + i), TL(L::B + i)), TL(L::C + i))));
        seed_w(sd1, 7, i, gl_neg(gl_add(gl_add(TL(L::A + 16 + i), TL(L::B + 16 + i)), TL(L::C + 16 + i))));
      }
      ld16(tl, M2, j, AUX + G2_AUX_LAMBDA, l0);
      ld16(tl, M2, j, AUX + G2_AUX_LAMBDA + 16, l1);
      MZB(6, AUX + G2_AUX_X_AUX, filter, [&](int i) __attribute__((always_inline)) { return econv_c0(l0, l1, l0, l1, i); }, &sd0);
      MZB(7, AUX + G2_AUX_X_AUX + 80, filter, [&](int i) __attribute__((always_inline)) { return econv_c1(l0, l1, l0, l1, i); }, &sd1);
    } else {
#pragma unroll 4
      for (int i = 0; i < 16; i++) seed_w(sd0, 8, i, gl_add(TL(L::C + 32 + i), TL(L::A + 32 + i)));
      ld16(tl, M2, j, AUX + G2_AUX_LAMBDA, l0);
      ld16(tl, M2, j, AUX + G2_AUX_LAMBDA + 16, l1);
#pragma unroll
      for (int i = 0; i < 16; i++) {
        dx0[i] = gl_sub(TL(L::C + i), TL(L::A + i));
        dx1[i] = gl_sub(TL(L::C + 16 + i), TL(L::A + 16 + i));
      }
      MZB(8, AUX + G2_AUX_Y_AUX, filter, [&](int i) __attribute__((always_inline)) { return econv_c0(l0, l1, dx0, dx1, i); }, &sd0);
#pragma unroll 4
      for (int i = 0; i < 16; i++) seed_w(sd1, 9, i, gl_add(TL(L::C + 48 + i), TL(L::A + 48 + i)));
      MZB(9, AUX + G2_AUX_Y_AUX + 80, filter, [&](int i) __attribute__((always_inline)) { return econv_c1(l0, l1, dx0, dx1, i); }, &sd1);
    }
  }
  store_part(A, part, j, tot0, tot1);
}

__global__ __launch_bounds__(256, 2) void k_quotient_fq_sched(QArgs A) {
  const size_t j = (size_t)blockIdx.x * blockDim.x + threadIdx.x;
  if (j >= A.count) return;
  schedule_part<FQL, true>(A, j, q_next(A, j), 33, 1);
}
__global__ __launch_bounds__(256) void k_quotient_fq_mul(QArgs A) {
  typedef FQL L;
  const size_t M2 = A.stride;
  const size_t j = (size_t)blockIdx.x * blockDim.x + threadIdx.x;
  if (j >= A.count) return;
  const u64* __restrict__ tl = A.tl;
  const qc64 W0 = QCONST(u64, A.W);
  const qc64 W1 = QCONST(u64, A.W + A.K);
  u64 tot0 = 0, tot1 = 0;
  const u64 filter = TL(L::FILTER);
  u64 a[16], b[16], c[16];
  ld16(tl, M2, j, L::A, a);
  ld16(tl, M2, j, L::B, b);
  ld16(tl, M2, j, L::C, c);
  mz_block(tl, M2, j, L::AUX, A, FQ_MZ_E0[0], 0, filter,
           [&](int i) __attribute__((always_inline)) {
             u64 v = conv16(a, b, i);
             return i < 16 ? gl_sub(v, c[i < 16 ? i : 0]) : v;
           },
           tot0, tot1);
  store_part(A, 0, j, tot0, tot1);
}

int g2_quotient_mz_blocks(const int** e0) {
  *e0 = G2_MZ_E0;
  return 10;
}
int fq_quotient_mz_blocks(const int** e0) {
  *e0 = FQ_MZ_E0;
  return 1;
}
void g2_quotient_launch(const QArgs& A0, const StarkShape& sh, hipStream_t st) {
  QArgs A = A0;
  A.n_parts = 7;
  const unsigned g = (unsigned)((A.count + 255) / 256);
  k_quotient_g2_add<0><<<g, 256, 0, st>>>(A);
  k_quotient_g2_add<5><<<g, 256, 0, st>>>(A);
  k_quotient_g2_add<1><<<g, 256, 0, st>>>(A);
  k_quotient_g2_add<2><<<g, 256, 0, st>>>(A);
  k_quotient_g2_add<3><<<g, 256, 0, st>>>(A);
  k_quotient_g2_add<4><<<g, 256, 0, st>>>(A);
  k_quotient_g2_sched<<<g, 256, 0, st>>>(A);
  quotient_finish_launch(A, sh, st);
}
void fq_quotient_launch(const QArgs& A0, const StarkShape& sh, hipStream_t st) {
  QArgs A = A0;
  A.n_parts = 2;
  const unsigned g = (unsigned)((A.count + 255) / 256);
  k_quotient_fq_mul<<<g, 256, 0, st>>>(A);
  k_quotient_fq_sched<<<g, 256, 0, st>>>(A);
  quotient_finish_launch(A, sh, st);
}

void quotient_g2fq_module_warm() {
  hipFuncAttributes a;
  (void)hipFuncGetAttributes(&a, reinterpret_cast<const void*>(&k_quotient_fq_sched));
}
```

### plonky2_bn254_amd/csrc/quotient_sched.h

```cpp
#pragma once
#include <vector>
#include "quotient_common.h"
#include "layout.h"

#ifndef MZ_CONSTS
#define MZ_CONSTS
static constexpr int QMZ_IQP = 0, QMZ_QUOT = 1, QMZ_LO = 18, QMZ_HI = 49;
#endif

struct QArgs {
  const u64* tl;
  const u64* al;
  const u64* W;
  const u64* mzt;
  QPointTables pt;
  u64 betas[2], gammas[2];
  u64 zh_inv[2];
  u64 w_inv;
  u64* out;
  u64* part;
  int n_parts;
  unsigned log_n;
  int K;
  size_t stride, count, k0;
  u32 natural, hsel;
};
static constexpr size_t QUOTIENT_MZT3_OFF = 10 * 2 * 80, QUOTIENT_MZT_WORDS = 10 * 2 * 80 + 10 * 80 * 4;
static inline size_t QUOTIENT_W_WORDS(int K) { return 6 * (size_t)K; }
__device__ __forceinline__ size_t q_next(const QArgs& A, size_t j) { return A.natural ? j + 1 : next_position(j, A.log_n); }

#define QCONST(T, p) ((const __attribute__((address_space(4))) T*)(p))
typedef const __attribute__((address_space(4))) u64* qc64;
typedef const __attribute__((address_space(4))) u32* qc32;

#define TL(c) tl[(size_t)(c)*M2 + j]
#define TN(c) tl[(size_t)(c)*M2 + jn]

__device__ __forceinline__ void ld16(const u64* __restrict__ tl, size_t M2, size_t j, int col, u64* v) {
#pragma unroll
  for (int i = 0; i < 16; i++) v[i] = tl[(size_t)(col + i) * M2 + j];
}
template <bool FULL = false>
__device__ __forceinline__ u64 conv16(const u64* A, const u64* B, int i) {
  Acc a;
  acc_init(a);
  if constexpr (FULL) {
#pragma clang loop unroll(full)
    for (int s = 0; s < 16; s++) {
      int t = i - s;
      if (t >= 0 && t < 16) acc_mad(a, A[s], B[t]);
    }
  } else {
#pragma unroll
    for (int s = 0; s < 16; s++) {
      int t = i - s;
      if (t >= 0 && t < 16) acc_mad(a, A[s], B[t]);
    }
  }
  return acc_red(a);
}

template <bool FULL = false, class InFn>
__device__ __forceinline__ void mz_block(const u64* __restrict__ tl, size_t M2, size_t j, int auxcol, const QArgs& A, int e0, int blk,
                                         u64 filter, InFn in, u64& tot0, u64& tot1, const Acc2* seed = nullptr) {
  const qc64 w0 = QCONST(u64, A.W + e0);
  const qc64 w1 = QCONST(u64, A.W + A.K + e0);
  const qc64 T0 = QCONST(u64, A.mzt + (size_t)blk * 160);
  const qc64 T1 = T0 + 80;
  const qc32 w3 = QCONST(u32, A.W + 2 * (size_t)A.K) + 8 * (size_t)e0;
  const qc32 T3 = QCONST(u32, A.mzt + QUOTIENT_MZT3_OFF) + 8 * (size_t)(blk * 80);
  u64 n0, n1;
  {
    Acc2 neg;
    if (seed) neg = *seed;
    else acc2_init(neg);
    if constexpr (FULL) {
#pragma clang loop unroll(full)
      for (int i = 0; i < 31; i++) {
        acc2_mad(neg, in(i), w0[1 + i], w1[1 + i]);
        if (i % 8 == 7) {
          asm volatile("" : "+v"(neg.a0.lo), "+v"(neg.a0.hi), "+v"(neg.a0.ov), "+v"(neg.a1.lo), "+v"(neg.a1.hi), "+v"(neg.a1.ov));
          __builtin_amdgcn_sched_barrier(0);
        }
      }
    } else {
#pragma unroll
      for (int i = 0; i < 31; i++) {
        acc2_mad(neg, in(i), w0[1 + i], w1[1 + i]);
        __builtin_amdgcn_sched_barrier(0);
      }
    }
    n0 = acc_red(neg.a0);
    n1 = acc_red(neg.a1);
    asm volatile("" : "+v"(n0), "+v"(n1));
  }
  __builtin_amdgcn_sched_barrier(0);
  const u64 iqp = TL(auxcol + QMZ_IQP);
  const u64 qsign = gl_sub(gl_dbl(iqp), 1);
  u64 s0, s1;
  {
    AccW q;
    accw_init(q);
#pragma unroll 1
    for (int jj = 0; jj < 17; jj++) accw_mad(q, TL(auxcol + QMZ_QUOT + jj), T3 + 8 * jj);
    s0 = gl_mul(qsign, acc3_red(q.a0));
    s1 = gl_mul(qsign, acc3_red(q.a1));
  }
  __builtin_amdgcn_sched_barrier(0);
  {
    AccW pos;
    accw_init(pos);
    accw_mad(pos, gl_sub(gl_mul(iqp, iqp), iqp), w3);
#pragma unroll 1
    for (int d = 0; d < 31; d++) {
      accw_mad(pos, TL(auxcol + QMZ_LO + d), T3 + 8 * (17 + d));
      accw_mad(pos, TL(auxcol + QMZ_HI + d), T3 + 8 * (48 + d));
    }
    s0 = gl_add(s0, acc3_red(pos.a0));
    s1 = gl_add(s1, acc3_red(pos.a1));
  }
  s0 = gl_sub(gl_sub(s0, T0[79]), n0);
  s1 = gl_sub(gl_sub(s1, T1[79]), n1);
  tot0 = gl_add(tot0, gl_mul(filter, s0));
  tot1 = gl_add(tot1, gl_mul(filter, s1));
  asm volatile("" : "+v"(tot0), "+v"(tot1));
}

#define EQ_GROUP(filter, n, AEXPR, BEXPR)                         \
  {                                                               \
    static_assert((n) % 16 == 0, "EQ_GROUP: n % 16");             \
    AccW g_;                                                      \
    accw_init(g_);                                                \
    constexpr int CH_ = 16;                                       \
    _Pragma("unroll 1") for (int i0_ = 0; i0_ < (n); i0_ += CH_) { \
      u64 d_[CH_];                                                \
      _Pragma("unroll") for (int k_ = 0; k_ < CH_; k_++) {        \
        const int i = i0_ + k_;                                   \
        d_[k_] = gl_sub((AEXPR), (BEXPR));                        \
      }                                                           \
      _Pragma("unroll") for (int k_ = 0; k_ < CH_; k_++) accw_mad(g_, d_[k_], W3 + 8 * (e + i0_ + k_)); \
    }                                                             \
    e += (n);                                                     \
    u64 f_ = (filter);                                            \
    tot0 = gl_add(tot0, gl_mul(f_, acc3_red(g_.a0)));             \
    tot1 = gl_add(tot1, gl_mul(f_, acc3_red(g_.a1)));             \
    asm volatile("" : "+v"(tot0), "+v"(tot1));  \
  }
#define EMIT(c)                                  \
  {                                              \
    u64 c_ = (c);                                \
    tot0 = gl_add(tot0, gl_mul(c_, W0[e]));      \
    tot1 = gl_add(tot1, gl_mul(c_, W1[e]));      \
    e += 1;                                      \
  }


__device__ __forceinline__ void store_part(const QArgs& A, int part, size_t j, u64 tot0, u64 tot1) {
  const size_t M2 = A.stride;
  A.part[((size_t)part * 2 + 0) * M2 + j] = tot0;
  A.part[((size_t)part * 2 + 1) * M2 + j] = tot1;
}

template <class L, bool FIRST_A_IS_ONE>
__device__ __forceinline__ void schedule_part(const QArgs& A, size_t j, size_t jn, int e, int part) {
  u64 tot0 = 0, tot1 = 0;
  const size_t M2 = A.stride;
  const u64* __restrict__ tl = A.tl;
  const qc64 W0 = QCONST(u64, A.W);
  const qc64 W1 = QCONST(u64, A.W + A.K);
  const qc32 W3 = QCONST(u32, A.W + 2 * (size_t)A.K);
  const u64 filter = TL(L::FILTER);
  const u64 is_first = TL(L::FLAGS + 0), is_last = TL(L::FLAGS + 1);
  const u64 n_filter = TN(L::FILTER), n_is_last = TN(L::FLAGS + 1);
  const u64 is_not_last_round = gl_sub(filter, is_last);
  const u64 is_next_not_last_round = gl_sub(n_filter, n_is_last);
  const u64 is_adding = TL(L::IS_ADDING), idnl = TL(L::IDNL);
  const u64 n_is_adding = TN(L::IS_ADDING), n_idnl = TN(L::IDNL);
  const u64 bit0 = TL(L::BITS), n_bit0 = TN(L::BITS);

  EMIT(gl_mul(is_first, gl_sub(is_adding, 1)));
  EQ_GROUP(is_first, L::PL, TL(L::DOUBLE + i), TL(L::B + i));
  EQ_GROUP(gl_mul(bit0, is_first), L::PL, TL(L::SUM + i), TL(L::C + i));
  EQ_GROUP(gl_mul(gl_sub(1, bit0), is_first), L::PL, TL(L::SUM + i), TL(L::A + i));
  if (FIRST_A_IS_ONE) {
    EQ_GROUP(is_first, L::PL, TL(L::A + i), (u64)(i == 0 ? 1 : 0));
  }
  EQ_GROUP(idnl, L::PL, TN(L::A + i), TL(L::SUM + i));
  EQ_GROUP(idnl, L::PL, TN(L::B + i), TL(L::DOUBLE + i));
  EQ_GROUP(gl_mul(n_bit0, idnl), L::PL, TN(L::SUM + i), TN(L::C + i));
  EQ_GROUP(gl_mul(gl_sub(1, n_bit0), idnl), L::PL, TN(L::SUM + i), TN(L::A + i));
  EQ_GROUP(idnl, L::PL, TN(L::DOUBLE + i), TL(L::DOUBLE + i));
  EMIT(gl_mul(idnl, gl_sub(n_is_adding, 1)));
  EMIT(gl_mul(idnl, n_idnl));
  EQ_GROUP(idnl, 256, TN(L::BITS + i), TL(L::BITS + ((i + 1) & 255)));
  EQ_GROUP(is_adding, L::PL, TN(L::A + i), TL(L::DOUBLE + i));
  EQ_GROUP(is_adding, L::PL, TN(L::B + i), TL(L::DOUBLE + i));
  EQ_GROUP(is_adding, L::PL, TN(L::SUM + i), TL(L::SUM + i));
  EQ_GROUP(is_adding, L::PL, TN(L::DOUBLE + i), TN(L::C + i));
  EMIT(gl_mul(is_adding, n_is_adding));
  EMIT(gl_mul(is_adding, gl_sub(n_idnl, is_next_not_last_round)));
  EQ_GROUP(is_adding, 256, TN(L::BITS + i), TL(L::BITS + i));
  {
    const u64 counter = TL(L::FLAGS + 2), inv_c = TL(L::FLAGS + 3), inv_cp = TL(L::FLAGS + 4);
    const u64 n_counter = TN(L::FLAGS + 2);
    const u64 not_filter = gl_sub(1, filter);
    EMIT(gl_mul(not_filter, is_first));
    EMIT(gl_mul(not_filter, is_last));
    EMIT(gl_mul(filter, gl_sub(gl_mul(counter, inv_c), gl_sub(1, is_first))));
    EMIT(gl_mul(gl_mul(filter, counter), is_first));
    const u64 cp = gl_sub(counter, 511);
    EMIT(gl_mul(filter, gl_sub(gl_mul(cp, inv_cp), gl_sub(1, is_last))));
    EMIT(gl_mul(gl_mul(filter, cp), is_last));
    EMIT(gl_mul(gl_mul(filter, gl_sub(1, is_last)), gl_sub(gl_sub(n_counter, counter), 1)));
    EMIT(gl_mul(gl_mul(filter, is_last), n_counter));
  }
  EMIT(gl_mul(is_not_last_round, gl_sub(TN(L::TIMESTAMP), TL(L::TIMESTAMP))));
  EMIT(gl_mul(is_not_last_round, gl_sub(n_filter, filter)));
  const u64 x = A.pt.x[j], llast = A.pt.llast[j];
  const u64 z_last = gl_sub(x, A.w_inv);
  {
    const u64 rc = TL(L::RANGE), diff = gl_sub(TN(L::RANGE), rc);
    EMIT(gl_mul(gl_sub(gl_mul(diff, diff), diff), z_last));
    EMIT(gl_mul(gl_sub(rc, 65535), llast));
  }
  store_part(A, part, j, tot0, tot1);
}

__device__ __forceinline__ void finish_point(const QArgs& A, const StarkShape& sh, size_t j) {
  const unsigned log_n = A.log_n;
  const size_t N = (size_t)1 << log_n, M2 = A.stride;
  const size_t jn = q_next(A, j);
  u64 tot0 = 0, tot1 = 0;
  for (int p = 0; p < A.n_parts; p++) {
    tot0 = gl_add(tot0, A.part[((size_t)p * 2 + 0) * M2 + j]);
    tot1 = gl_add(tot1, A.part[((size_t)p * 2 + 1) * M2 + j]);
  }
  const u64 x = A.pt.x[j], lfirst = A.pt.lfirst[j], llast = A.pt.llast[j];
  const u64 z_last = gl_sub(x, A.w_inv);
  lookup_and_ctl_constraints(sh, A.tl, A.al, M2, j, jn, (const u32*)(A.W + 2 * (size_t)A.K), sh.n_constraints, A.betas, A.gammas,
                             lfirst, llast, z_last, tot0, tot1);
  const size_t h = A.natural ? A.hsel : j >> log_n;
  const size_t k = A.natural ? A.k0 + j : (size_t)bitrev32((u32)(j & (N - 1)), log_n);
  A.out[(0 * 2 + h) * N + k] = gl_mul(tot0, A.zh_inv[h]);
  A.out[(1 * 2 + h) * N + k] = gl_mul(tot1, A.zh_inv[h]);
}

void quotient_host_tables(int K, const u64 alphas[2], const int* mz_e0, int n_blocks, std::vector<u64>& W, std::vector<u64>& mzt);
void quotient_fill_args(QArgs& A, const StarkShape& sh, const u64* d_tl, const u64* d_al, const u64* d_W, const u64* d_mzt,
                        const QPointTables& pt, const u64 betas[2], const u64 gammas[2], unsigned log_n, u64* d_out,
                        u64* d_part);
static constexpr int QUOTIENT_MAX_PARTS = 7;
void quotient_finish_launch(const QArgs& A, const StarkShape& sh, hipStream_t st);
```

### plonky2_bn254_amd/csrc/quotient_selftest.hip

```cpp
#include <string>
#include <vector>
#include "ctx.h"
#include "prover.h"

static bool qs_canonical(const uint64_t* w, size_t n) {
  for (size_t k = 0; k < n; k++)
    if (w[k] >= GL_P) return false;
  return true;
}

static constexpr int QS_LOG_MIN = 3, QS_LOG_WHOLE_MAX = 12, QS_LOG_WINDOW_MAX = 20;
static constexpr size_t QS_STRIDE_MAX = 8192;
static_assert(QUOTIENT_MAX_PARTS == BN254S_QS_MAX_PARTS, "the part buffer of bn254s_selftest_quotient");

extern "C" {

int bn254s_selftest_quotient(bn254s_ctx* c, int kind, int log_n, int flags, int h, size_t k0, size_t count, size_t stride,
                             const uint64_t* trace, const uint64_t* aux, const uint64_t alphas[2], const uint64_t betas[2],
                             const uint64_t gammas[2], const uint64_t* x, const uint64_t* lfirst, const uint64_t* llast, uint64_t* out,
                             uint64_t* part) {
  if (!c || !trace || !aux || !alphas || !betas || !gammas || !out || !part) return BN254S_E_INVALID_ARG;
  if (kind < 0 || kind > 2 || (flags & ~(BN254S_QS_WINDOW | BN254S_QS_RAW))) return BN254S_E_INVALID_ARG;
  const bool window = flags & BN254S_QS_WINDOW, raw = flags & BN254S_QS_RAW;
  if (log_n < QS_LOG_MIN || log_n > (window ? QS_LOG_WINDOW_MAX : QS_LOG_WHOLE_MAX)) return BN254S_E_INVALID_ARG;
  const size_t N = (size_t)1 << log_n;
  if (window) {
    if (h < 0 || h > 1 || count < 1 || count > N || k0 > N - count || stride < count + 1 || stride > QS_STRIDE_MAX)
      return BN254S_E_INVALID_ARG;
  } else {
    count = stride = 2 * N;
  }
  const bool own_tables = x || lfirst || llast;
  if (own_tables && !(x && lfirst && llast)) return BN254S_E_INVALID_ARG;
  const StarkKind& sk = stark_kind(kind);
  const StarkShape& sh = sk.shape;
  const size_t W = (size_t)sh.W, A = (size_t)sh.n_aux();
  const int K = sh.n_total_constraints();
  if (!qs_canonical(alphas, 2) || !qs_canonical(betas, 2) || !qs_canonical(gammas, 2)) return BN254S_E_INVALID_ARG;
  if (!qs_canonical(trace, W * stride) || !qs_canonical(aux, A * stride)) return BN254S_E_INVALID_ARG;
  if (own_tables && (!qs_canonical(x, count) || !qs_canonical(lfirst, count) || !qs_canonical(llast, count))) return BN254S_E_INVALID_ARG;

  std::vector<u64> hW, hmzt;
  const int* mz_e0 = nullptr;
  const int nblk = sk.mz_blocks(&mz_e0);
  quotient_host_tables(K, alphas, mz_e0, nblk, hW, hmzt);

  const size_t pw = (size_t)QUOTIENT_MAX_PARTS * 2 * stride;
  HIP_TRY(c, hipSetDevice(c->device));
  u64* d_tl = c->words("qs.tl", W * stride);
  u64* d_al = c->words("qs.al", A * stride);
  u64* d_pt = c->words("qs.pt", 3 * count);
  u64* d_W = c->words("qs.W", hW.size());
  u64* d_mzt = c->words("qs.mzt", hmzt.size());
  u64* d_out = c->words("qs.out", 4 * N);
  u64* d_part = c->words("qs.part", pw);
  if (!d_tl || !d_al || !d_pt || !d_W || !d_mzt || !d_out || !d_part) return BN254S_E_OOM;
  hipStream_t st = c->stream;
  HIP_TRY(c, hipMemcpyAsync(d_tl, trace, 8 * W * stride, hipMemcpyHostToDevice, st));
  HIP_TRY(c, hipMemcpyAsync(d_al, aux, 8 * A * stride, hipMemcpyHostToDevice, st));
  HIP_TRY(c, hipMemcpyAsync(d_W, hW.data(), 8 * hW.size(), hipMemcpyHostToDevice, st));
  HIP_TRY(c, hipMemcpyAsync(d_mzt, hmzt.data(), 8 * hmzt.size(), hipMemcpyHostToDevice, st));
  HIP_TRY(c, hipMemcpyAsync(d_out, out, 8 * 4 * N, hipMemcpyHostToDevice, st));
  HIP_TRY(c, hipMemcpyAsync(d_part, part, 8 * pw, hipMemcpyHostToDevice, st));
  QPointTables pt;
  pt.x = d_pt;
  pt.lfirst = d_pt + count;
  pt.llast = d_pt + 2 * count;
  if (own_tables) {
    HIP_TRY(c, hipMemcpyAsync(d_pt, x, 8 * count, hipMemcpyHostToDevice, st));
    HIP_TRY(c, hipMemcpyAsync(d_pt + count, lfirst, 8 * count, hipMemcpyHostToDevice, st));
    HIP_TRY(c, hipMemcpyAsync(d_pt + 2 * count, llast, 8 * count, hipMemcpyHostToDevice, st));
  } else if (window) {
    quotient_point_tables_window(d_pt, d_pt + count, d_pt + 2 * count, (unsigned)log_n, h, k0, count, st);
  } else {
    quotient_point_tables(d_pt, d_pt + count, d_pt + 2 * count, (unsigned)log_n, st);
  }
  QArgs QA;
  quotient_fill_args(QA, sh, d_tl, d_al, d_W, d_mzt, pt, betas, gammas, (unsigned)log_n, d_out, d_part);
  if (window) quotient_window_args(QA, d_tl, d_al, pt, d_part, stride, count, k0, h);
  if (raw) {
    QA.zh_inv[0] = QA.zh_inv[1] = 1;
    QA.w_inv = 0;
  }
  sk.quotient_launch(QA, sh, st);
  HIP_TRY(c, hipGetLastError());
  HIP_TRY(c, hipMemcpyAsync(out, d_out, 8 * 4 * N, hipMemcpyDeviceToHost, st));
  HIP_TRY(c, hipMemcpyAsync(part, d_part, 8 * pw, hipMemcpyDeviceToHost, st));
  HIP_TRY(c, hipStreamSynchronize(st));
  return BN254S_OK;
}

int bn254s_selftest_point_tables(bn254s_ctx* c, int log_n, int window, int h, size_t k0, size_t count, uint64_t* out) {
  if (!c || !out || log_n < QS_LOG_MIN || log_n > QS_LOG_WINDOW_MAX || window < 0 || window > 1) return BN254S_E_INVALID_ARG;
  const size_t N = (size_t)1 << log_n;
  if (window) {
    if (h < 0 || h > 1 || count < 1 || count > N || k0 >= N) return BN254S_E_INVALID_ARG;
  } else {
    count = 2 * N;
  }
  HIP_TRY(c, hipSetDevice(c->device));
  u64* d = c->words("qs.pt", 3 * count);
  if (!d) return BN254S_E_OOM;
  if (window) quotient_point_tables_window(d, d + count, d + 2 * count, (unsigned)log_n, h, k0, count, c->stream);
  else quotient_point_tables(d, d + count, d + 2 * count, (unsigned)log_n, c->stream);
  HIP_TRY(c, hipGetLastError());
  HIP_TRY(c, hipMemcpyAsync(out, d, 8 * 3 * count, hipMemcpyDeviceToHost, c->stream));
  HIP_TRY(c, hipStreamSynchronize(c->stream));
  return BN254S_OK;
}

int bn254s_selftest_aux(bn254s_ctx* c, int kind, const uint64_t* trace, size_t rows, const uint64_t betas[2], const uint64_t gammas[2],
                        uint64_t* out) {
  if (!c || !trace || !betas || !gammas || !out || kind < 0 || kind > 2) return BN254S_E_INVALID_ARG;
  if (rows < 64 || rows > ((size_t)1 << 16) || (rows & (rows - 1))) return BN254S_E_INVALID_ARG;
  const StarkShape& sh = stark_kind(kind).shape;
  const size_t tw = (size_t)sh.W * rows, aw = (size_t)sh.n_aux() * rows, sw = aux_scratch_words(sh, rows);
  if (!qs_canonical(betas, 2) || !qs_canonical(gammas, 2) || !qs_canonical(trace, tw)) return BN254S_E_INVALID_ARG;
  HIP_TRY(c, hipSetDevice(c->device));
  u64* d = c->words("qs.aux", tw + aw + sw + 2);
  if (!d) return BN254S_E_OOM;
  u64* d_aux = d + tw;
  u64* d_scr = d_aux + aw;
  int* d_err = (int*)(d_scr + sw);
  int h_err = 0;
  HIP_TRY(c, hipMemcpyAsync(d, trace, 8 * tw, hipMemcpyHostToDevice, c->stream));
  HIP_TRY(c, hipMemsetAsync(d_err, 0, 8, c->stream));
  aux_build(sh, d, rows, betas, gammas, d_aux, d_scr, d_err, c->stream);
  HIP_TRY(c, hipGetLastError());
  HIP_TRY(c, hipMemcpyAsync(out, d_aux, 8 * aw, hipMemcpyDeviceToHost, c->stream));
  HIP_TRY(c, hipMemcpyAsync(&h_err, d_err, 4, hipMemcpyDeviceToHost, c->stream));
  HIP_TRY(c, hipStreamSynchronize(c->stream));
  if (h_err) {
    c->set_err("auxiliary columns: device error " + std::to_string(h_err) +
               " (a range-checked or table value above 65535, or a CTL filter that is neither 0 nor 1)");
    return h_err;
  }
  return BN254S_OK;
}

}
```

### plonky2_bn254_amd/csrc/verify.hip

```cpp
#include <cstring>
#include <string>
#include <vector>
#include "ctx.h"
#include "prover.h"
#include "quotient.h"
#include "transcript.h"
#include "verify_air_host.h"
#include "verify_query.h"

namespace {

inline gl2 ext(const u64* w) { return gl2_make(w[0], w[1]); }
inline gl2 base(u64 x) { return gl2_make(x, 0); }

constexpr unsigned VLOG = 7;
constexpr int VT = 5, VS = 4, VPTS = VT * VS;

#define VCHK(call)                                             \
  do {                                                         \
    hipError_t e_ = (call);                                    \
    if (e_ != hipSuccess) {                                    \
      err = std::string(#call) + ": " + hipGetErrorString(e_); \
      return BN254S_E_HIP;                                     \
    }                                                          \
  } while (0)

int vanishing_on_gpu(bn254s_ctx* c, int kind, const StarkShape& sh, const u64* words, const View& v, const u64 alphas[2],
                     const u64 betas[2], const u64 gammas[2], gl2 z_last, gl2 l_first, gl2 l_last, gl2 out[2], std::string& err) {
  const size_t M2 = (size_t)2 << VLOG, N = (size_t)1 << VLOG;
  const int W = v.W, A = v.A, K = sh.n_total_constraints();
  hipStream_t st = c->stream;
  std::vector<u64> tl((size_t)W * M2, 0), al((size_t)A * M2, 0), px(M2, 0), pf(M2, 0), pl(M2, 0);
  size_t jn[VPTS];
  for (int j = 0; j < VPTS; j++) {
    u32 k = bitrev32((u32)j, VLOG);
    jn[j] = bitrev32((k + 1) & (u32)(N - 1), VLOG);
    if (jn[j] < (size_t)VPTS) {
      err = "internal: synthetic next position collides";
      return BN254S_E_INTERNAL;
    }
  }
  auto fill = [&](std::vector<u64>& buf, int ncols, size_t off_local, size_t off_next) {
    for (int col = 0; col < ncols; col++) {
      const u64 *lv = words + off_local + 2 * (size_t)col, *nv = words + off_next + 2 * (size_t)col;
      for (int j = 0; j < VPTS; j++) {
        u64 t = (u64)(j % VT);
        buf[(size_t)col * M2 + j] = gl_add(lv[0], gl_mul(t, lv[1]));
        buf[(size_t)col * M2 + jn[j]] = gl_add(nv[0], gl_mul(t, nv[1]));
      }
    }
  };
  fill(tl, W, v.local, v.next);
  fill(al, A, v.aux, v.aux_next);
  for (int t = 0; t < VT; t++) {
    px[VT * 1 + t] = 1;
    pf[VT * 2 + t] = 1;
    pl[VT * 3 + t] = 1;
  }
  std::vector<u64> hW, hmzt;
  const int* mz_e0 = nullptr;
  int nblk = stark_kind(kind).mz_blocks(&mz_e0);
  quotient_host_tables(K, alphas, mz_e0, nblk, hW, hmzt);

  u64* d_tl = c->words("vf_tl", tl.size());
  u64* d_al = c->words("vf_al", al.size());
  u64* d_pt = c->words("vf_pt", 3 * M2);
  u64* d_W = c->words("vf_W", hW.size());
  u64* d_mzt = c->words("vf_mzt", hmzt.size());
  u64* d_out = c->words("vf_out", 4 * N);
  u64* d_part = c->words("vf_part", (size_t)QUOTIENT_MAX_PARTS * 2 * M2);
  if (!d_tl || !d_al || !d_pt || !d_W || !d_mzt || !d_out || !d_part) {
    err = c->BufPool::err;
    return BN254S_E_OOM;
  }
  VCHK(hipMemcpyAsync(d_tl, tl.data(), tl.size() * 8, hipMemcpyHostToDevice, st));
  VCHK(hipMemcpyAsync(d_al, al.data(), al.size() * 8, hipMemcpyHostToDevice, st));
  VCHK(hipMemcpyAsync(d_pt, px.data(), M2 * 8, hipMemcpyHostToDevice, st));
  VCHK(hipMemcpyAsync(d_pt + M2, pf.data(), M2 * 8, hipMemcpyHostToDevice, st));
  VCHK(hipMemcpyAsync(d_pt + 2 * M2, pl.data(), M2 * 8, hipMemcpyHostToDevice, st));
  VCHK(hipMemcpyAsync(d_W, hW.data(), hW.size() * 8, hipMemcpyHostToDevice, st));
  VCHK(hipMemcpyAsync(d_mzt, hmzt.data(), hmzt.size() * 8, hipMemcpyHostToDevice, st));
  QPointTables pt;
  pt.x = d_pt;
  pt.lfirst = d_pt + M2;
  pt.llast = d_pt + 2 * M2;
  QArgs QA;
  quotient_fill_args(QA, sh, d_tl, d_al, d_W, d_mzt, pt, betas, gammas, VLOG, d_out, d_part);
  QA.zh_inv[0] = QA.zh_inv[1] = 1;
  QA.w_inv = 0;
  stark_kind(kind).quotient_launch(QA, sh, st);
  std::vector<u64> ho(4 * N);
  VCHK(hipMemcpyAsync(ho.data(), d_out, ho.size() * 8, hipMemcpyDeviceToHost, st));
  VCHK(hipStreamSynchronize(st));
  VCHK(hipGetLastError());
  const u64 inv2 = gl_inv(2), inv6 = gl_inv(6);
  const gl2 sel[VS] = {gl2_make(1, 0), z_last, l_first, l_last};
  for (int a = 0; a < 2; a++) {
    gl2 tot = gl2_make(0, 0);
    u64 plain[VT];
    for (int s = 0; s < VS; s++) {
      u64 y[VT];
      for (int t = 0; t < VT; t++) {
        int j = VT * s + t;
        u64 e = ho[(size_t)(a * 2 + 0) * N + bitrev32((u32)j, VLOG)];
        if (s == 0) plain[t] = e;
        y[t] = s == 0 ? e : gl_sub(e, plain[t]);
      }
      u64 d1 = gl_sub(y[1], y[0]);
      u64 d2 = gl_add(gl_sub(y[2], gl_dbl(y[1])), y[0]);
      u64 d3 = gl_sub(gl_add(gl_sub(y[3], gl_mul(3, y[2])), gl_mul(3, y[1])), y[0]);
      u64 p4 = gl_add(gl_add(y[0], gl_mul(4, d1)), gl_add(gl_mul(6, d2), gl_mul(4, d3)));
      if (p4 != y[4]) {
        err = "internal: a constraint class is not cubic in the openings";
        return BN254S_E_INTERNAL;
      }
      u64 h2 = gl_mul(d2, inv2), h3 = gl_mul(d3, inv6);
      gl2 g = gl2_make(gl_sub(gl_add(y[0], gl_mul(7, h2)), gl_mul(21, h3)), gl_add(gl_sub(d1, h2), gl_mul(9, h3)));
      tot = gl2_add(tot, gl2_mul(sel[s], g));
    }
    out[a] = tot;
  }
  return BN254S_OK;
}

void limbs16(const u64* words4, u64* out) {
  for (int i = 0; i < 16; i++) out[i] = (words4[i >> 2] >> (16 * (i & 3))) & 0xFFFF;
}
void ctl_rows(int kind, const u64* scalars, const u64* x, const u64* off, const u64* outputs, size_t k, std::vector<u64>& in,
              std::vector<u64>& out) {
  const int PW = stark_kind(kind).point_words, PL = 4 * PW;
  in.assign((kind == KIND_FQ ? PL : 2 * PL) + 17, 0);
  out.assign(PL + 1, 0);
  size_t m = 0;
  for (int w = 0; w < PW; w += 4, m += 16) limbs16(x + PW * k + w, &in[m]);
  if (kind != KIND_FQ)
    for (int w = 0; w < PW; w += 4, m += 16) limbs16(off + PW * k + w, &in[m]);
  limbs16(scalars + 4 * k, &in[m]);
  m += 16;
  in[m] = k;
  m = 0;
  for (int w = 0; w < PW; w += 4, m += 16) limbs16(outputs + PW * k + w, &out[m]);
  out[m] = k;
}

}

int verify_front(bn254s_ctx* c, int kind, const bn254s_params& P, int degree_bits, const u64* w, size_t n_words, View& v, u64* rec,
                 u64 ctl_ch[4], std::string& err) {
  if (!make_view(kind, P, degree_bits, v) || v.total != n_words) {
    err = "bad proof shape";
    return BN254S_E_VERIFY;
  }
  const StarkShape& sh = stark_kind(kind).shape;
  const size_t N = (size_t)1 << degree_bits, M2 = (size_t)1 << v.log_m2;
  const int W = v.W, A = v.A, NQ = v.NQ;
  for (size_t i = 0; i < n_words; i++)
    if (w[i] >= GL_P && i != v.pow) {
      err = "non-canonical field element";
      return BN254S_E_VERIFY;
    }
  Challenger ch;
  ch.observe_n(w + v.caps, 64);
  u64 betas[2], gammas[2], alphas[2];
  for (int i = 0; i < 2; i++) {
    betas[i] = ch.challenge();
    gammas[i] = ch.challenge();
  }
  ctl_ch[0] = betas[0], ctl_ch[1] = betas[1], ctl_ch[2] = gammas[0], ctl_ch[3] = gammas[1];
  u64 st12[12];
  ch.compact(st12);
  if (memcmp(st12, w + v.init, sizeof(st12))) {
    err = "init_challenger_state mismatch";
    return BN254S_E_VERIFY;
  }
  ch.observe_n(w + v.caps + 64, 64);
  for (int i = 0; i < 2; i++) alphas[i] = ch.challenge();
  ch.observe_n(w + v.caps + 128, 64);
  gl2 zeta = ch.challenge_ext();
  ch.observe_n(w + v.local, 2 * (size_t)W);
  ch.observe_n(w + v.aux, 2 * (size_t)A);
  ch.observe_n(w + v.quot, 2 * (size_t)NQ);
  ch.observe_n(w + v.next, 2 * (size_t)W);
  ch.observe_n(w + v.aux_next, 2 * (size_t)A);
  for (int i = 0; i < v.NCTLZ; i++) {
    ch.observe(w[v.ctlz + i]);
    ch.observe(0);
  }
  gl2 fri_alpha = ch.challenge_ext();
  for (size_t i = 0; i < vq_record_words(P.num_queries); i++) rec[i] = 0;
  for (int l = 0; l < v.L; l++) {
    ch.observe_n(w + v.fri_caps + 64 * (size_t)l, 64);
    gl2 b = ch.challenge_ext();
    rec[VQ_REC_BETAS + 2 * l] = b.c0;
    rec[VQ_REC_BETAS + 2 * l + 1] = b.c1;
  }
  ch.observe_n(w + v.final_poly, 2 * v.final_len);
  ch.observe(w[v.pow]);
  u64 pow_response = ch.challenge();
  for (uint32_t q = 0; q < P.num_queries; q++) rec[VQ_REC_QUERIES + q] = ch.challenge() % M2;

  const u64 g = gl_root_of_unity(degree_bits);
  gl2 zeta_pow = zeta;
  for (int i = 0; i < degree_bits; i++) zeta_pow = gl2_mul(zeta_pow, zeta_pow);
  const gl2 one = gl2_make(1, 0);
  gl2 z_h = gl2_sub(zeta_pow, one);
  if (gl2_eq(z_h, gl2_make(0, 0))) {
    err = "Opening point is in the subgroup.";
    return BN254S_E_VERIFY;
  }
  const u64 nF = (u64)N % GL_P;
  gl2 l_first = gl2_mul(z_h, gl2_inv(gl2_mul_base(gl2_sub(zeta, one), nF)));
  gl2 l_last = gl2_mul(z_h, gl2_inv(gl2_mul_base(gl2_sub(gl2_mul_base(zeta, g), one), nF)));
  gl2 z_last = gl2_sub(zeta, base(gl_inv(g)));
  gl2 van[2];
  if (c) {
    int rc = vanishing_on_gpu(c, kind, sh, w, v, alphas, betas, gammas, z_last, l_first, l_last, van, err);
    if (rc != BN254S_OK) return rc;
  } else {
    if (!host_air::vanishing_on_host(kind, sh, w + v.local, w + v.next, w + v.aux, w + v.aux_next, alphas, betas, gammas, z_last,
                                     l_first, l_last, van, err))
      return BN254S_E_INTERNAL;
  }
  for (int j = 0; j < 2; j++) {
    gl2 t = gl2_add(ext(w + v.quot + 4 * j), gl2_mul(ext(w + v.quot + 4 * j + 2), zeta_pow));
    if (!gl2_eq(van[j], gl2_mul(z_h, t))) {
      err = "Mismatch between evaluation and opening of quotient polynomial";
      return BN254S_E_VERIFY;
    }
  }

  if (pow_response >> (64 - P.pow_bits)) {
    err = "Invalid proof of work witness";
    return BN254S_E_VERIFY;
  }
  std::vector<gl2> opened[3];
  for (int p = 0; p < W; p++) opened[0].push_back(ext(w + v.local + 2 * (size_t)p));
  for (int p = 0; p < A; p++) opened[0].push_back(ext(w + v.aux + 2 * (size_t)p));
  for (int p = 0; p < NQ; p++) opened[0].push_back(ext(w + v.quot + 2 * (size_t)p));
  for (int p = 0; p < W; p++) opened[1].push_back(ext(w + v.next + 2 * (size_t)p));
  for (int p = 0; p < A; p++) opened[1].push_back(ext(w + v.aux_next + 2 * (size_t)p));
// ... 119 lines not shown
```

### plonky2_bn254_amd/lib.py

```python
from __future__ import annotations

import ctypes as C
import os
from typing import Optional

import numpy as np

_HERE = os.path.dirname(os.path.abspath(__file__))
LIB_PATH = os.environ.get("BN254S_LIB") or os.path.join(_HERE, "libbn254stark.so")

U64P = C.POINTER(C.c_uint64)


class LibraryMissing(RuntimeError):
    pass


class VerifyError(RuntimeError):
    """bn254s_verify rejected the proof; the message is the reference verifier's error text."""


class UnprovableJobs(RuntimeError):

    def __init__(self, msg, provable, step):
        super().__init__(msg)
        self.provable, self.step = provable, step


JOB_STEP_NONE = 0xFFFF


class Params(C.Structure):
    _fields_ = [(n, C.c_uint32) for n in (
        "struct_size", "security_bits", "num_challenges", "rate_bits", "cap_height", "pow_bits",
        "arity_bits", "final_poly_bits", "num_queries", "min_rows_log2")]


_lib = None


def load_library():
    global _lib
    if _lib is not None:
        return _lib
    if not os.path.exists(LIB_PATH):
        raise LibraryMissing(
            f"{LIB_PATH} not found: build it with `python -c 'import __graft_entry__ as g; g.build()'` "
            "(there is no CPU fallback for the proving path)")
    lib = C.CDLL(LIB_PATH)
    vp = C.c_void_p
    lib.bn254s_abi_version.restype = C.c_int
    lib.bn254s_params_default.argtypes = [C.POINTER(Params)]
    lib.bn254s_ctx_create.argtypes = [C.c_int, C.POINTER(vp)]
    lib.bn254s_ctx_destroy.argtypes = [vp]
    lib.bn254s_ctx_trim.argtypes = [vp]
    lib.bn254s_last_error.argtypes = [vp]
    lib.bn254s_last_error.restype = C.c_char_p
    for name in ("bn254s_prove_g1", "bn254s_prove_g2"):
        getattr(lib, name).argtypes = [vp, C.POINTER(Params), vp, vp, vp, C.c_size_t, C.POINTER(vp)]
    lib.bn254s_prove_fq_exp.argtypes = [vp, C.POINTER(Params), vp, vp, C.c_size_t, C.POINTER(vp)]
    lib.bn254s_generate_trace.argtypes = [vp, C.c_int, vp, vp, vp, C.c_size_t, C.c_uint32, vp, vp]
    lib.bn254s_prove_g1_batch.argtypes = [vp, C.POINTER(Params), vp, vp, vp, C.c_size_t, C.c_size_t, C.POINTER(vp)]
    lib.bn254s_prove_batch.argtypes = [vp, C.c_int, C.POINTER(Params), vp, vp, vp, C.c_size_t, C.c_size_t, C.POINTER(vp)]
    lib.bn254s_prove_batch_begin.argtypes = [vp, C.c_int, C.POINTER(Params), vp, vp, vp, C.c_size_t, C.c_size_t, C.POINTER(vp),
                                             C.POINTER(vp)]
    lib.bn254s_prove_batch_end.argtypes = [vp]
    lib.bn254s_prove_batch_multi.argtypes = [C.POINTER(vp), C.c_size_t, C.c_int, C.POINTER(Params), vp, vp, vp, C.c_size_t,
                                             C.c_size_t, C.POINTER(vp)]
    lib.bn254s_proof_words.argtypes = [vp, C.POINTER(U64P), C.POINTER(C.c_size_t)]
    lib.bn254s_proof_outputs.argtypes = [vp, C.POINTER(U64P), C.POINTER(C.c_size_t)]
    lib.bn254s_proof_degree_bits.argtypes = [vp]
    lib.bn254s_proof_section.argtypes = [vp, C.c_int, C.POINTER(U64P), C.POINTER(C.c_size_t)]
    lib.bn254s_proof_stage_ms.argtypes = [vp, C.POINTER(C.POINTER(C.c_float)), C.POINTER(C.c_size_t)]
    lib.bn254s_stage_name.argtypes = [C.c_size_t]
    lib.bn254s_stage_name.restype = C.c_char_p
    lib.bn254s_proof_free.argtypes = [vp]
    lib.bn254s_proof_serialize.argtypes = [vp, vp, C.c_size_t]
    lib.bn254s_proof_serialize.restype = C.c_size_t
    lib.bn254s_verify.argtypes = [vp, C.c_int, C.POINTER(Params), C.c_uint32, vp, C.c_size_t, vp, vp, vp, vp, C.c_size_t]
    lib.bn254s_verify_host.argtypes = [C.c_int, C.POINTER(Params), C.c_uint32, vp, C.c_size_t, vp, vp, vp, vp, C.c_size_t, C.c_char_p,
                                       C.c_size_t]
    if hasattr(lib, "bn254s_verify_batch"):
        lib.bn254s_verify_batch.argtypes = [vp, C.c_int, C.POINTER(Params), C.c_uint32, vp, C.c_size_t, vp, vp, vp, vp, vp, C.c_size_t,
                                            vp, vp, C.c_size_t]
        lib.bn254s_selftest_verify_front.argtypes = [C.c_int, C.POINTER(Params), C.c_uint32, vp, C.c_size_t, vp, C.c_size_t]
        lib.bn254s_selftest_query_round.argtypes = [vp, C.c_int, C.POINTER(Params), C.c_uint32, vp, C.c_size_t, vp, C.c_size_t,
                                                    C.c_size_t, vp]
        lib.bn254s_selftest_verify_batch_ms.argtypes = [vp, vp]
        lib.bn254s_selftest_query_text.argtypes = [C.c_int, C.c_int]
        lib.bn254s_selftest_query_text.restype = C.c_char_p
    lib.bn254s_map_to_g2.argtypes = [vp, C.POINTER(Params), vp, vp, C.c_size_t, vp, vp, vp, C.POINTER(vp), C.POINTER(vp)]
    lib.bn254s_hash_to_fq2.argtypes = [vp, C.c_size_t, vp]
    lib.bn254s_g1_msm_chain.argtypes = [vp, vp, vp, vp, C.c_size_t, vp, vp]
    lib.bn254s_g1_msm.argtypes = [vp, C.POINTER(Params), vp, vp, vp, C.c_size_t, C.c_size_t, vp, vp, C.POINTER(vp)]
    lib.bn254s_g2_msm_chain.argtypes = [vp, vp, vp, vp, C.c_size_t, vp, vp]
    lib.bn254s_g2_msm.argtypes = [vp, C.POINTER(Params), vp, vp, vp, C.c_size_t, C.c_size_t, vp, vp, C.POINTER(vp)]
    lib.bn254s_g1_recover_from_x_batch.argtypes = [vp, vp, C.c_size_t, vp, vp, vp]
    lib.bn254s_g1_recover_from_x.argtypes = [vp, C.POINTER(Params), vp, C.c_size_t, C.c_size_t, vp, vp, vp, C.POINTER(vp)]
    lib.bn254s_g2_recover_from_x_batch.argtypes = [vp, vp, vp, C.c_size_t, vp, vp, vp]
    lib.bn254s_g2_recover_from_x.argtypes = [vp, C.POINTER(Params), vp, vp, C.c_size_t, C.c_size_t, vp, vp, vp, C.POINTER(vp)]
    for name in ("bn254s_fq_sqrt", "bn254s_fq2_sqrt"):
        getattr(lib, name + "_batch").argtypes = [vp, vp, vp, C.c_size_t, vp, vp, vp, vp]
        getattr(lib, name).argtypes = [vp, C.POINTER(Params), vp, vp, C.c_size_t, C.c_size_t, vp, vp, vp, vp, C.POINTER(vp)]
    lib.bn254s_fq_inv_batch.argtypes = [vp, vp, C.c_size_t, vp]
    lib.bn254s_fq2_inv_batch.argtypes = [vp, vp, C.c_size_t, vp]
    lib.bn254s_g2_subgroup_check_batch.argtypes = [vp, vp, C.c_size_t, vp]
    lib.bn254s_g2_subgroup_check.argtypes = [vp, C.POINTER(Params), vp, vp, C.c_size_t, C.c_size_t, vp, vp, C.POINTER(vp)]
    lib.bn254s_g2_clear_cofactor_batch.argtypes = [vp, vp, C.c_size_t, vp, vp]
    lib.bn254s_g2_clear_cofactor.argtypes = [vp, C.POINTER(Params), vp, vp, C.c_size_t, C.c_size_t, vp, vp, vp, C.POINTER(vp)]
    lib.bn254s_map_to_g2_batch.argtypes = [vp, vp, C.c_size_t, vp]
    lib.bn254s_hash_to_g2_batch.argtypes = [vp, vp, C.c_size_t, C.c_size_t, vp]
    lib.bn254s_job_outputs_batch.argtypes = [vp, C.c_int, vp, vp, vp, C.c_size_t, vp, vp]
    lib.bn254s_job_outputs.argtypes = [vp, C.c_int, C.POINTER(Params), vp, vp, vp, C.c_size_t, C.c_size_t, vp, C.POINTER(vp)]
    lib.bn254s_job_check_batch.argtypes = [vp, C.c_int, vp, vp, vp, C.c_size_t, vp, vp]
    lib.bn254s_prove_batch_checked.argtypes = [vp, C.c_int, C.POINTER(Params), vp, vp, vp, C.c_size_t, C.c_size_t, vp, vp,
                                               C.POINTER(vp)]
    lib.bn254s_hash_to_fq2_batch.argtypes = [vp, vp, C.c_size_t, C.c_size_t, vp]
    if hasattr(lib, "bn254s_map_to_g1"):
        lib.bn254s_hash_to_fq.argtypes = [vp, C.c_size_t, vp]
        lib.bn254s_hash_to_fq_batch.argtypes = [vp, vp, C.c_size_t, C.c_size_t, vp]
        lib.bn254s_map_to_g1_batch.argtypes = [vp, vp, C.c_size_t, vp, vp, vp]
        lib.bn254s_hash_to_g1_batch.argtypes = [vp, vp, C.c_size_t, C.c_size_t, vp]
        lib.bn254s_map_to_g1.argtypes = [vp, C.POINTER(Params), vp, C.c_size_t, C.c_size_t, vp, vp, vp, C.POINTER(vp)]
    lib.bn254s_ctl_values.argtypes = [C.c_int, vp, vp, vp, vp, C.c_size_t, vp, vp]
    lib.bn254s_commit_values.argtypes = [vp, vp, C.c_size_t, vp, vp, vp]
    lib.bn254s_bench_ntt.argtypes = [vp, C.c_size_t, C.c_int, C.POINTER(C.c_float)]
    lib.bn254s_bench_ntt_clock.argtypes = [vp, C.c_size_t, C.c_int, C.POINTER(C.c_float), C.POINTER(C.c_float), C.POINTER(C.c_float)]
    lib.bn254s_bench_issue.argtypes = [vp, C.POINTER(C.c_float), C.POINTER(C.c_float)]
    lib.bn254s_poseidon_permute.argtypes = [vp, vp, C.c_size_t]
    lib.bn254s_selftest_field.argtypes = [vp, vp, vp, C.c_size_t, vp]
    lib.bn254s_selftest_poseidon.argtypes = [vp, C.c_int, vp, C.c_size_t]
    lib.bn254s_selftest_leaf_hash.argtypes = [vp, vp, C.c_size_t, C.c_int, C.c_int, C.c_int, vp]
    lib.bn254s_selftest_fq_inv.argtypes = [vp, vp, C.c_size_t, vp]
    lib.bn254s_selftest_fq.argtypes = [vp, C.c_int, vp, C.c_size_t, vp]
    if hasattr(lib, "bn254s_selftest_logup"):
        lib.bn254s_selftest_logup.argtypes = [vp, vp, C.c_size_t, C.c_int, C.c_int, C.c_int, C.c_int, C.c_int, vp, vp]
    if hasattr(lib, "bn254s_selftest_fri_fold"):
        lib.bn254s_selftest_acc.argtypes = [vp, vp, vp, C.c_size_t, C.c_size_t, vp]
        lib.bn254s_selftest_openings.argtypes = [vp, vp, C.c_int, C.c_int, vp, vp, vp]
        lib.bn254s_selftest_fri_combine.argtypes = [vp, C.c_int, C.c_int, C.c_int, C.c_int, C.c_size_t, vp, vp, vp, vp]
        lib.bn254s_selftest_fri_fold.argtypes = [vp, vp, C.c_int, C.c_uint64, vp, vp]
        lib.bn254s_selftest_fri_rows.argtypes = [vp, vp, C.c_int, C.c_int, C.c_int, C.c_size_t, C.c_size_t, vp, C.c_int, vp, vp]
    if hasattr(lib, "bn254s_selftest_transforms"):
        lib.bn254s_selftest_transforms.argtypes = [vp, C.c_int, C.c_int, C.c_int, C.c_int, C.c_int, vp, vp, vp]
        lib.bn254s_selftest_mul_2exp.argtypes = [vp, vp, C.c_size_t, vp]
        lib.bn254s_selftest_outer_dft.argtypes = [vp, C.c_int, C.c_int, vp, C.c_size_t, vp]
    if hasattr(lib, "bn254s_selftest_quotient"):
        lib.bn254s_selftest_quotient.argtypes = [vp, C.c_int, C.c_int, C.c_int, C.c_int, C.c_size_t, C.c_size_t, C.c_size_t, vp, vp,
                                                 vp, vp, vp, vp, vp, vp, vp, vp]
        lib.bn254s_selftest_point_tables.argtypes = [vp, C.c_int, C.c_int, C.c_int, C.c_size_t, C.c_size_t, vp]
        lib.bn254s_selftest_aux.argtypes = [vp, C.c_int, vp, C.c_size_t, vp, vp, vp]
    if hasattr(lib, "bn254s_selftest_proof_plan"):
        lib.bn254s_selftest_proof_plan.argtypes = [C.c_int, C.c_size_t, C.POINTER(Params), C.c_uint64, C.c_int, C.c_int, C.c_int,
                                                   C.c_int, vp, C.c_char_p, C.c_size_t]
    lib.bn254s_bench_copy.argtypes = [vp, C.c_size_t, C.c_int]
    lib.bn254s_bench_leafhash.argtypes = [vp, C.c_size_t, C.c_int, C.c_int, C.POINTER(C.c_float)]
    lib.bn254s_g1_generate_trace.argtypes = [vp, vp, vp, vp, C.c_size_t, C.c_uint32, vp, vp]
    _lib = lib
    return lib


def default_params() -> Params:
    p = Params()
    load_library().bn254s_params_default(C.byref(p))
    return p


def _ptr(a: Optional[np.ndarray]):
    if a is None:
        return None
    assert a.dtype == np.uint64 and a.flags["C_CONTIGUOUS"]
    return a.ctypes.data_as(C.c_void_p)


def _slots(n_jobs, per_proof):
    return (C.c_void_p * ((n_jobs + per_proof - 1) // per_proof))()


def _proofs(lib, slots):
    return [Proof(lib, C.c_void_p(h)) for h in slots]


class Proof:

    _stage_names = None

    def __init__(self, lib, handle):
        self._lib, self._h = lib, handle
        self._words = self._outputs = None
        self.degree_bits = lib.bn254s_proof_degree_bits(handle)
        ms, k = C.POINTER(C.c_float)(), C.c_size_t()
        lib.bn254s_proof_stage_ms(handle, C.byref(ms), C.byref(k))
        if Proof._stage_names is None or len(Proof._stage_names) != k.value:
            Proof._stage_names = [lib.bn254s_stage_name(i).decode() for i in range(k.value)]
        self.stage_ms = dict(zip(Proof._stage_names, ms[:k.value]))

    def _fetch(self, fn, what):
        if not self._h:
            raise RuntimeError(f"Proof.{what}: the proof was closed before its {what} were read")
        data, n = U64P(), C.c_size_t()
        rc = fn(self._h, C.byref(data), C.byref(n))
        if rc != 0:
            raise RuntimeError(f"bn254s_proof_{what} failed with {rc}")
        return data, n.value

    @property
    def words(self) -> np.ndarray:
        if self._words is None:
            data, n = self._fetch(self._lib.bn254s_proof_words, "words")
            self._words = np.ctypeslib.as_array(data, shape=(n,)).copy()
        return self._words

    @property
    def outputs(self) -> np.ndarray:
        if self._outputs is None:
            data, n = self._fetch(self._lib.bn254s_proof_outputs, "outputs")
            self._outputs = np.ctypeslib.as_array(data, shape=(n,)).copy() if n else np.zeros(0, np.uint64)
        return self._outputs

    def caps(self) -> np.ndarray:
        if self._words is not None:
            return self._words[:192].copy()
        data, n = self._fetch(self._lib.bn254s_proof_words, "words")
        assert n >= 192
        return np.ctypeslib.as_array(data, shape=(192,)).copy()

    SECTIONS = ("trace_cap", "auxiliary_polys_cap", "quotient_polys_cap", "local_values", "next_values", "auxiliary_polys",
                "auxiliary_polys_next", "ctl_zs_first", "quotient_polys", "commit_phase_merkle_caps", "query_round_proofs",
                "final_poly", "pow_witness", "init_challenger_state")

    def section(self, name: str) -> np.ndarray:
        data, n = U64P(), C.c_size_t()
        rc = self._lib.bn254s_proof_section(self._h, self.SECTIONS.index(name), C.byref(data), C.byref(n))
        if rc != 0:
            raise RuntimeError(f"bn254s_proof_section({name}) failed with {rc}")
        return np.ctypeslib.as_array(data, shape=(n.value,)).copy() if n.value else np.zeros(0, np.uint64)

    def serialize(self) -> bytes:
        need = self._lib.bn254s_proof_serialize(self._h, None, 0)
        buf = C.create_string_buffer(need)
        assert self._lib.bn254s_proof_serialize(self._h, buf, need) == need
        return buf.raw

    def close(self):
        if self._h:
            try:
                self.words, self.outputs
            finally:
                self._lib.bn254s_proof_free(self._h)
                self._h = None

    def __del__(self):
        if getattr(self, "_h", None):
            self._lib.bn254s_proof_free(self._h)
            self._h = None


class Context:

    def __init__(self, device: int = 0):
        self._h = None
        self._lib = load_library()
        h = C.c_void_p()
        rc = self._lib.bn254s_ctx_create(device, C.byref(h))
        if rc != 0:
            raise RuntimeError(f"bn254s_ctx_create(device={device}) failed with {rc} (is a GPU visible?)")
        self._h = h
        self.device = device

    def close(self):
        if self._h:
            self._lib.bn254s_ctx_destroy(self._h)
            self._h = None

    def __del__(self):
        self.close()

    def trim(self):
        self._check(self._lib.bn254s_ctx_trim(self._h), "bn254s_ctx_trim")

    def _check(self, rc, what):
        if rc != 0:
            raise RuntimeError(f"{what} failed with {rc}: {self._lib.bn254s_last_error(self._h).decode()}")

    def prove_g1(self, scalars, x, offset, params: Optional[Params] = None) -> Proof:
        params = params or default_params()
        n = scalars.shape[0]
        out = C.c_void_p()
        self._check(self._lib.bn254s_prove_g1(self._h, C.byref(params), _ptr(scalars), _ptr(x), _ptr(offset), n,
                                              C.byref(out)), "bn254s_prove_g1")
        return Proof(self._lib, out)

    def prove_g2(self, scalars, x, offset, params: Optional[Params] = None) -> Proof:
        params = params or default_params()
        out = C.c_void_p()
        self._check(self._lib.bn254s_prove_g2(self._h, C.byref(params), _ptr(scalars), _ptr(x), _ptr(offset),
                                              scalars.shape[0], C.byref(out)), "bn254s_prove_g2")
        return Proof(self._lib, out)

    def prove_fq_exp(self, scalars, x, params: Optional[Params] = None) -> Proof:
        params = params or default_params()
        out = C.c_void_p()
        self._check(self._lib.bn254s_prove_fq_exp(self._h, C.byref(params), _ptr(scalars), _ptr(x), scalars.shape[0],
# ... 254 lines not shown
        return pts

    def map_to_g1(self, u, per_proof=128, params: Optional[Params] = None):
        params = params or default_params()
        u = np.ascontiguousarray(u, dtype=np.uint64)
        n = u.shape[0]
        pts, flags, jobs = np.zeros((n, 8), np.uint64), np.zeros(2 * n, np.uint8), np.zeros((2 * n, 8), np.uint64)
        outs = _slots(2 * n, per_proof)
        self._check(self._lib.bn254s_map_to_g1(self._h, C.byref(params), _ptr(u), n, per_proof, _ptr(pts),
                                               flags.ctypes.data_as(C.c_void_p), _ptr(jobs), outs), "bn254s_map_to_g1")
        return pts, flags, jobs, _proofs(self._lib, outs)

    def _job_arrays(self, kind, scalars, x, offset):
        scalars, x = (np.ascontiguousarray(a, dtype=np.uint64) for a in (scalars, x))
        pw = {0: 8, 1: 16, 2: 4}.get(kind, x.shape[-1] if x.ndim == 2 else 0)
        offset = None if kind == 2 or offset is None else np.ascontiguousarray(offset, dtype=np.uint64)
        n = scalars.shape[0]
        if scalars.shape != (n, 4) or x.shape != (n, pw) or (offset is not None and offset.shape != (n, pw)):
            raise ValueError(f"job_outputs: scalars {scalars.shape}, x {x.shape}, offset {None if offset is None else offset.shape}")
        return pw, n, scalars, x, offset

    def job_outputs_batch(self, kind, scalars, x, offset=None):
        pw, n, scalars, x, offset = self._job_arrays(kind, scalars, x, offset)
        outs, finite = np.zeros((n, pw), np.uint64), np.zeros(n, np.uint8)
        self._check(self._lib.bn254s_job_outputs_batch(self._h, kind, _ptr(scalars), _ptr(x), _ptr(offset), n, _ptr(outs),
                                                       finite.ctypes.data_as(C.c_void_p)), "bn254s_job_outputs_batch")
        return outs, finite

    def job_outputs(self, kind, scalars, x, offset=None, per_proof=128, params: Optional[Params] = None):
        params = params or default_params()
        pw, n, scalars, x, offset = self._job_arrays(kind, scalars, x, offset)
        outs = np.zeros((n, pw), np.uint64)
        slots = _slots(n, per_proof)
        self._check(self._lib.bn254s_job_outputs(self._h, kind, C.byref(params), _ptr(scalars), _ptr(x), _ptr(offset), n, per_proof,
                                                 _ptr(outs), slots), "bn254s_job_outputs")
        return outs, _proofs(self._lib, slots)

    def job_check_batch(self, kind, scalars, x, offset=None):
        _, n, scalars, x, offset = self._job_arrays(kind, scalars, x, offset)
        provable, step = np.zeros(n, np.uint8), np.zeros(n, np.uint16)
        self._check(self._lib.bn254s_job_check_batch(self._h, kind, _ptr(scalars), _ptr(x), _ptr(offset), n,
                                                     provable.ctypes.data_as(C.c_void_p), step.ctypes.data_as(C.c_void_p)),
                    "bn254s_job_check_batch")
        return provable, step

    def prove_batch_checked(self, kind, scalars, x, offset=None, per_proof=128, params: Optional[Params] = None):
        params = params or default_params()
        _, n, scalars, x, offset = self._job_arrays(kind, scalars, x, offset)
        provable, step = np.zeros(n, np.uint8), np.zeros(n, np.uint16)
        slots = _slots(n, per_proof)
        rc = self._lib.bn254s_prove_batch_checked(self._h, kind, C.byref(params), _ptr(scalars), _ptr(x), _ptr(offset), n, per_proof,
                                                  provable.ctypes.data_as(C.c_void_p), step.ctypes.data_as(C.c_void_p), slots)
        if rc == -4 and not provable.all():
            raise UnprovableJobs(f"bn254s_prove_batch_checked failed with -4: {self._lib.bn254s_last_error(self._h).decode()}",
                                 provable, step)
        self._check(rc, "bn254s_prove_batch_checked")
        return _proofs(self._lib, slots), provable, step

    def ctl_values(self, kind, scalars, x, offset, outputs):
        n = scalars.shape[0]
        pl = {0: 32, 1: 64, 2: 16}[kind]
        rows_in = np.zeros((n, (pl if kind == 2 else 2 * pl) + 17), np.uint64)
        rows_out = np.zeros((n, pl + 1), np.uint64)
        outputs = np.ascontiguousarray(outputs, dtype=np.uint64)
        self._check(self._lib.bn254s_ctl_values(kind, _ptr(scalars), _ptr(x), _ptr(offset), _ptr(outputs), n, _ptr(rows_in),
                                                _ptr(rows_out)), "bn254s_ctl_values")
        return rows_in, rows_out

    def commit_values(self, values: np.ndarray, want_coeffs=True, want_lde=True):
        ncols, n = values.shape
        assert n == 65536
        coeffs = np.zeros((ncols, n), np.uint64) if want_coeffs else None
        lde = np.zeros((ncols, 2 * n), np.uint64) if want_lde else None
        cap = np.zeros((16, 4), np.uint64)
        self._check(self._lib.bn254s_commit_values(self._h, _ptr(values), ncols, _ptr(coeffs), _ptr(lde), _ptr(cap)),
                    "bn254s_commit_values")
        return coeffs, lde, cap

    def bench_ntt(self, ncols: int, iters: int = 10) -> float:
        ms = C.c_float()
        self._check(self._lib.bn254s_bench_ntt(self._h, ncols, iters, C.byref(ms)), "bn254s_bench_ntt")
        return ms.value

    def bench_ntt_clock(self, ncols: int, iters: int = 10):
        ms, mhz, mn = C.c_float(), C.c_float(), C.c_float()
        self._check(self._lib.bn254s_bench_ntt_clock(self._h, ncols, iters, C.byref(ms), C.byref(mhz), C.byref(mn)), "bn254s_bench_ntt_clock")
        return ms.value, mhz.value, mn.value

    def bench_issue(self):
        ns, mhz = C.c_float(), C.c_float()
        self._check(self._lib.bn254s_bench_issue(self._h, C.byref(ns), C.byref(mhz)), "bn254s_bench_issue")
        return ns.value, mhz.value

    def bench_copy(self, words: int, iters: int = 3):
        self._check(self._lib.bn254s_bench_copy(self._h, words, iters), "bn254s_bench_copy")

    def bench_leafhash(self, ncols: int, log_leaves: int = 17, iters: int = 5) -> float:
        ms = C.c_float()
        self._check(self._lib.bn254s_bench_leafhash(self._h, ncols, log_leaves, iters, C.byref(ms)), "bn254s_bench_leafhash")
        return ms.value

    def selftest_field(self, a: np.ndarray, b: np.ndarray) -> np.ndarray:
        a = np.ascontiguousarray(a, dtype=np.uint64)
        b = np.ascontiguousarray(b, dtype=np.uint64)
        out = np.zeros((a.shape[0], 17), np.uint64)
        self._check(self._lib.bn254s_selftest_field(self._h, _ptr(a), _ptr(b), a.shape[0], _ptr(out)), "bn254s_selftest_field")
        return out

    def selftest_poseidon(self, variant: int, states: np.ndarray) -> np.ndarray:
        st = np.ascontiguousarray(states, dtype=np.uint64).copy()
        assert st.ndim == 2 and st.shape[1] == 12
        self._check(self._lib.bn254s_selftest_poseidon(self._h, variant, _ptr(st), st.shape[0]), "bn254s_selftest_poseidon")
        return st

    def selftest_leaf_hash(self, data: np.ndarray, kernel: int, chunk_cols: int = 0) -> np.ndarray:
        data = np.ascontiguousarray(data, dtype=np.uint64)
        ncols, n = data.shape
        assert n > 0 and n & (n - 1) == 0, "the number of leaves must be a power of two"
        out = np.zeros((n, 4), np.uint64)
        self._check(self._lib.bn254s_selftest_leaf_hash(self._h, _ptr(data), ncols, n.bit_length() - 1, kernel, chunk_cols, _ptr(out)),
                    "bn254s_selftest_leaf_hash")
        return out

    def selftest_fq_inv(self, x: np.ndarray) -> np.ndarray:
        x = np.ascontiguousarray(x, dtype=np.uint64)
        out = np.zeros((x.shape[0], 8), np.uint64)
        self._check(self._lib.bn254s_selftest_fq_inv(self._h, _ptr(x), x.shape[0], _ptr(out)), "bn254s_selftest_fq_inv")
        return out

    SELFTEST_FQ_WORDS = ((16, 68), (16, 60), (32, 92), (72, 74))

    def selftest_fq(self, group: int, rows: np.ndarray) -> np.ndarray:
        rows = np.ascontiguousarray(rows, dtype=np.uint64)
        if not 0 <= group < len(self.SELFTEST_FQ_WORDS):
            raise ValueError(f"selftest_fq: unknown group {group}")
        wi, wo = self.SELFTEST_FQ_WORDS[group]
        assert rows.ndim == 2 and rows.shape[1] == wi, (rows.shape, wi)
        out = np.zeros((rows.shape[0], wo), np.uint64)
        self._check(self._lib.bn254s_selftest_fq(self._h, group, _ptr(rows), rows.shape[0], _ptr(out)), "bn254s_selftest_fq")
        return out

    def selftest_logup(self, trace: np.ndarray, rc_begin: int, n_rc: int, table_col: int, freq_col: int, betas) -> np.ndarray:
        trace = np.ascontiguousarray(trace, dtype=np.uint64)
        assert trace.ndim == 2
        ncols, rows = trace.shape
        b = np.array([int(betas[0]), int(betas[1])], dtype=np.uint64)
        out = np.zeros((2 * ((n_rc + 1) // 2 + 1), rows), np.uint64)
        self._check(self._lib.bn254s_selftest_logup(self._h, _ptr(trace), rows, ncols, rc_begin, n_rc, table_col, freq_col, _ptr(b),
                                                    _ptr(out)), "bn254s_selftest_logup")
        return out

    STARK_SHAPES = {0: (781, 456, 1111, 1573), 1: (1295, 906, 1693, 2605), 2: (427, 134, 770, 910)}
    QS_MAX_PARTS = 7
    QS_N_PARTS = {0: 6, 1: 7, 2: 2}

    def selftest_quotient(self, kind: int, log_n: int, trace: np.ndarray, aux: np.ndarray, alphas, betas, gammas, raw: bool = False,
                          window=None, tables=None, fill: int = 0):
        w, a, _, _ = self.STARK_SHAPES[kind]
        trace = np.ascontiguousarray(trace, dtype=np.uint64)
        aux = np.ascontiguousarray(aux, dtype=np.uint64)
        stride = trace.shape[1]
        assert trace.shape == (w, stride) and aux.shape == (a, stride), (trace.shape, aux.shape)
        n = 1 << log_n
        flags = (2 if raw else 0) | (1 if window is not None else 0)
        h, k0, count = window if window is not None else (0, 0, 0)
        if window is None:
            assert stride == 2 * n, (stride, n)
        ch = [np.array([int(v[0]), int(v[1])], dtype=np.uint64) for v in (alphas, betas, gammas)]
        tabs = [None, None, None] if tables is None else [np.ascontiguousarray(t, dtype=np.uint64) for t in tables]
        if tables is not None:
            want = count if window is not None else 2 * n
            assert all(t.shape == (want,) for t in tabs), [t.shape for t in tabs]
        out = np.full((2, 2, n), fill, np.uint64)
        part = np.full((self.QS_MAX_PARTS, 2, stride), fill, np.uint64)
        self._check(self._lib.bn254s_selftest_quotient(self._h, kind, log_n, flags, h, k0, count, stride if window is not None else 0,
                                                       _ptr(trace), _ptr(aux), _ptr(ch[0]), _ptr(ch[1]), _ptr(ch[2]), _ptr(tabs[0]),
                                                       _ptr(tabs[1]), _ptr(tabs[2]), _ptr(out), _ptr(part)), "bn254s_selftest_quotient")
        return out, part

    def selftest_point_tables(self, log_n: int, window=None) -> np.ndarray:
        h, k0, count = window if window is not None else (0, 0, 2 << log_n)
        out = np.zeros((3, count), np.uint64)
        self._check(self._lib.bn254s_selftest_point_tables(self._h, log_n, int(window is not None), h, k0, count, _ptr(out)),
                    "bn254s_selftest_point_tables")
        return out

    def selftest_aux(self, kind: int, trace: np.ndarray, betas, gammas) -> np.ndarray:
        w, a, _, _ = self.STARK_SHAPES[kind]
        trace = np.ascontiguousarray(trace, dtype=np.uint64)
        assert trace.ndim == 2 and trace.shape[0] == w, trace.shape
        rows = trace.shape[1]
        b = np.array([int(betas[0]), int(betas[1])], dtype=np.uint64)
        g = np.array([int(gammas[0]), int(gammas[1])], dtype=np.uint64)
        out = np.zeros((a, rows), np.uint64)
        self._check(self._lib.bn254s_selftest_aux(self._h, kind, _ptr(trace), rows, _ptr(b), _ptr(g), _ptr(out)), "bn254s_selftest_aux")
        return out

    def selftest_acc(self, values: np.ndarray, weights: np.ndarray) -> np.ndarray:
        values = np.ascontiguousarray(values, dtype=np.uint64)
        weights = np.ascontiguousarray(weights, dtype=np.uint64)
        rows, t = values.shape
        assert weights.shape == (t,)
        out = np.zeros((rows, 2), np.uint64)
        self._check(self._lib.bn254s_selftest_acc(self._h, _ptr(values), _ptr(weights), t, rows, _ptr(out)), "bn254s_selftest_acc")
        return out

    def selftest_openings(self, coeffs: np.ndarray, log_r: int, zeta, zeta_next) -> np.ndarray:
        coeffs = np.ascontiguousarray(coeffs, dtype=np.uint64)
        npolys, n = coeffs.shape
        assert n == 1 << (16 + log_r), (n, log_r)
        z0 = np.array([int(v) for v in zeta], dtype=np.uint64)
        z1 = np.array([int(v) for v in zeta_next], dtype=np.uint64)
        out = np.zeros((npolys, 1 << log_r, 5), np.uint64)
        self._check(self._lib.bn254s_selftest_openings(self._h, _ptr(coeffs), npolys, log_r, _ptr(z0), _ptr(z1), _ptr(out)),
                    "bn254s_selftest_openings")
        return out

    def selftest_fri_combine_coeffs(self, cols: np.ndarray, w: int, n_rc: int, n_ctl: int, weights: np.ndarray) -> np.ndarray:
        cols = np.ascontiguousarray(cols, dtype=np.uint64)
        weights = np.ascontiguousarray(weights, dtype=np.uint64)
        n_polys, n = cols.shape
        assert n_polys == w + 2 * ((n_rc + 1) // 2 + 1) + 2 * n_ctl + 4 and weights.shape == (n_polys, 2), (cols.shape, weights.shape)
        out = np.zeros((6, n), np.uint64)
        self._check(self._lib.bn254s_selftest_fri_combine(self._h, 0, w, n_rc, n_ctl, n, _ptr(cols), _ptr(weights), None, _ptr(out)),
                    "bn254s_selftest_fri_combine")
        return out

    def selftest_fri_combine_final(self, cl: np.ndarray, xs: np.ndarray, w: int, n_rc: int, n_ctl: int, zeta, zeta_next, r0, r1, r2,
                                   alpha) -> np.ndarray:
        cl = np.ascontiguousarray(cl, dtype=np.uint64)
        xs = np.ascontiguousarray(xs, dtype=np.uint64)
        m = xs.shape[0]
        assert cl.shape == (6, m)
        pts = np.array([int(v) for e in (zeta, zeta_next, r0, r1, r2, alpha) for v in e], dtype=np.uint64)
        out = np.zeros((m, 2), np.uint64)
        self._check(self._lib.bn254s_selftest_fri_combine(self._h, 1, w, n_rc, n_ctl, m, _ptr(cl), _ptr(xs), _ptr(pts), _ptr(out)),
                    "bn254s_selftest_fri_combine")
        return out

    def selftest_fri_fold(self, vals: np.ndarray, shift: int, beta) -> np.ndarray:
        vals = np.ascontiguousarray(vals, dtype=np.uint64)
        m = vals.shape[0]
        assert vals.shape == (m, 2) and m >= 16 and m & (m - 1) == 0
        b = np.array([int(beta[0]), int(beta[1])], dtype=np.uint64)
        out = np.zeros((m >> 4, 2), np.uint64)
        self._check(self._lib.bn254s_selftest_fri_fold(self._h, _ptr(vals), m.bit_length() - 1, int(shift), _ptr(b), _ptr(out)),
                    "bn254s_selftest_fri_fold")
        return out

    def selftest_fri_rows(self, lde: np.ndarray, h: int, k0: int, rows: int, indices):
        lde = np.ascontiguousarray(lde, dtype=np.uint64)
        ncols, m2 = lde.shape
        assert m2 >= 4 and m2 & (m2 - 1) == 0
        idx = np.ascontiguousarray(indices, dtype=np.uint32)
        win = np.zeros((ncols, rows), np.uint64)
        gat = np.zeros((ncols, idx.shape[0]), np.uint64)
        self._check(self._lib.bn254s_selftest_fri_rows(self._h, _ptr(lde), ncols, m2.bit_length() - 2, h, k0, rows,
                                                       idx.ctypes.data_as(C.c_void_p), idx.shape[0], _ptr(win), _ptr(gat)),
                    "bn254s_selftest_fri_rows")
        return win, gat

    TRANSFORM_SPLIT, TRANSFORM_COMPACT = 1, 2

    def selftest_transforms(self, op: int, log_n: int, flags: int, data: np.ndarray, coset_mask: int = 3):
        data = np.ascontiguousarray(data, dtype=np.uint64)
        ncols, n = data.shape
        assert n == 1 << log_n, (n, log_n)
        out0 = np.zeros((ncols, n if op in (0, 3) else 2 * n), np.uint64)
        out1 = np.zeros((ncols, 2 * n), np.uint64) if op == 0 else None
        self._check(self._lib.bn254s_selftest_transforms(self._h, op, log_n, flags, ncols, coset_mask, _ptr(data), _ptr(out0),
                                                         _ptr(out1)), "bn254s_selftest_transforms")
        return (out0, out1) if op == 0 else out0

    def selftest_mul_2exp(self, x: np.ndarray) -> np.ndarray:
        x = np.ascontiguousarray(x, dtype=np.uint64)
        out = np.zeros((x.shape[0], 64), np.uint64)
        self._check(self._lib.bn254s_selftest_mul_2exp(self._h, _ptr(x), x.shape[0], _ptr(out)), "bn254s_selftest_mul_2exp")
        return out

    def selftest_outer_dft(self, log_r: int, inverse: bool, rows: np.ndarray) -> np.ndarray:
        rows = np.ascontiguousarray(rows, dtype=np.uint64)
        assert rows.ndim == 2 and rows.shape[1] == 1 << log_r, (rows.shape, log_r)
        out = np.zeros_like(rows)
        self._check(self._lib.bn254s_selftest_outer_dft(self._h, log_r, int(inverse), _ptr(rows), rows.shape[0], _ptr(out)),
                    "bn254s_selftest_outer_dft")
        return out

    def poseidon_permute(self, states: np.ndarray) -> np.ndarray:
        st = np.ascontiguousarray(states, dtype=np.uint64).copy()
        self._check(self._lib.bn254s_poseidon_permute(self._h, _ptr(st), st.shape[0]), "bn254s_poseidon_permute")
        return st

    def generate_trace(self, kind, scalars, x, offset=None, min_rows_log2=16):
        width, pw = {0: (781, 8), 1: (1295, 16), 2: (427, 4)}[kind]
        n = scalars.shape[0]
        rows = max(1 << min_rows_log2, 512 * n)
        rows = 1 << (rows - 1).bit_length()
        trace = np.zeros((width, rows), np.uint64)
        outs = np.zeros((n, pw), np.uint64)
        self._check(self._lib.bn254s_generate_trace(self._h, kind, _ptr(scalars), _ptr(x), _ptr(offset), n, min_rows_log2,
                                                    _ptr(trace), _ptr(outs)), "bn254s_generate_trace")
        return trace, outs

    def g1_generate_trace(self, scalars, x, offset, min_rows_log2=16, width=781):
        n = scalars.shape[0]
        rows = max(1 << min_rows_log2, 512 * n)
        rows = 1 << (rows - 1).bit_length()
        trace = np.zeros((width, rows), np.uint64)
        outs = np.zeros((n, 8), np.uint64)
        self._check(self._lib.bn254s_g1_generate_trace(self._h, _ptr(scalars), _ptr(x), _ptr(offset), n, min_rows_log2,
                                                       _ptr(trace), _ptr(outs)), "bn254s_g1_generate_trace")
        return trace, outs


def verify_host(kind, words, degree_bits, scalars, x, offset, outputs, params: Optional[Params] = None):
    lib = load_library()
    params = params or default_params()
    words = np.ascontiguousarray(words, dtype=np.uint64)
    outputs = np.ascontiguousarray(outputs, dtype=np.uint64)
    buf = C.create_string_buffer(256)
    rc = lib.bn254s_verify_host(kind, C.byref(params), degree_bits, _ptr(words), words.size, _ptr(scalars), _ptr(x), _ptr(offset),
                                _ptr(outputs), scalars.shape[0], buf, 256)
    if rc == -8:
        raise VerifyError(buf.value.decode())
    if rc != 0:
        raise RuntimeError(f"bn254s_verify_host failed with {rc}: {buf.value.decode()}")

# ... 528 lines not shown
```

Measured before the change: 91.70 proofs/s.

## Split lookup constraints into parallel slices in a separate quotient kernel

The lookup and CTL constraint work that ran serially per point inside the quotient finish kernel moves into a new kernel. That kernel splits the helper loop into 4 slices plus a Z/CTL slice across grid.y, and each slice writes partial sums to a new look buffer. The finish kernel then only sums the parts and slices. This exposes more parallelism for the long serial helper loop, at the cost of an extra launch, an extra buffer of (slices+1)*2*M2 words, and more global memory traffic.

New measurement: 90.66 proofs/s. 0.989x the previous value.

```diff
diff --git a/include/bn254_stark.h b/include/bn254_stark.h
--- a/include/bn254_stark.h
+++ b/include/bn254_stark.h
@@ -225,6 +225,11 @@
                              const uint64_t* trace, const uint64_t* aux, const uint64_t alphas[2], const uint64_t betas[2],
                              const uint64_t gammas[2], const uint64_t* x, const uint64_t* lfirst, const uint64_t* llast, uint64_t* out,
                              uint64_t* part);
+#define BN254S_QS_MAX_SLICES 32
+int bn254s_selftest_quotient_lookups(bn254s_ctx* ctx, int kind, int log_n, int flags, int h, size_t k0, size_t count, size_t stride,
+                                     const uint64_t* trace, const uint64_t* aux, const uint64_t alphas[2], const uint64_t betas[2],
+                                     const uint64_t gammas[2], const uint64_t* x, const uint64_t* lfirst, const uint64_t* llast,
+                                     int n_slices, uint64_t* out, uint64_t* part, uint64_t* look, int* slices, int* ranges);
 int bn254s_selftest_point_tables(bn254s_ctx* ctx, int log_n, int window, int h, size_t k0, size_t count, uint64_t* out);
 int bn254s_selftest_aux(bn254s_ctx* ctx, int kind, const uint64_t* trace, size_t rows, const uint64_t betas[2], const uint64_t gammas[2],
                         uint64_t* out);
diff --git a/plonky2_bn254_amd/csrc/proof_plan.h b/plonky2_bn254_amd/csrc/proof_plan.h
--- a/plonky2_bn254_amd/csrc/proof_plan.h
+++ b/plonky2_bn254_amd/csrc/proof_plan.h
@@ -13,6 +13,7 @@
 struct PlanBuffers {
   size_t in, tvals, tcoef, hist, tmp, ldechunk, sponge, comb, tlde, trees, avals, acoef, alde, scratch, quot, tabs, open, fri,
       fritrees, qout;
+  size_t qlook;
   size_t win;
 };
 
diff --git a/plonky2_bn254_amd/csrc/proof_plan.hip b/plonky2_bn254_amd/csrc/proof_plan.hip
--- a/plonky2_bn254_amd/csrc/proof_plan.hip
+++ b/plonky2_bn254_amd/csrc/proof_plan.hip
@@ -81,6 +81,7 @@
   b.alde = lowmem ? 0 : (size_t)A * M2;
   b.scratch = std::max(sk.trace_scratch_words(n), aux_scratch_words(sh, N));
   b.quot = (size_t)(3 * NQ) * N + (size_t)NQ * M2 + (size_t)QUOTIENT_MAX_PARTS * 2 * (stream ? WROWS : M2);
+  b.qlook = QUOTIENT_LOOK_WORDS(QUOTIENT_SLICES, stream ? WROWS : M2);
   b.tabs = QUOTIENT_W_WORDS(K) + QUOTIENT_MZT_WORDS + 4 * (size_t)(W + A + NQ);
   b.open = std::max((size_t)(W + A + NQ) * NSPL * R * 5 + FRI_OPENING_TABLE_WORDS, n * (size_t)PW);
   pl.fri_words = pl.fri_tree_words = 0;
diff --git a/plonky2_bn254_amd/csrc/prover.hip b/plonky2_bn254_amd/csrc/prover.hip
--- a/plonky2_bn254_amd/csrc/prover.hip
+++ b/plonky2_bn254_amd/csrc/prover.hip
@@ -131,6 +131,7 @@
   u32* qidx;
   u64 *ttree, *atree, *qtree;
   u64 *qv, *ab, *qcoef, *qlde, *qpart;
+  u64* qlook;
   u64 *W, *mzt, *apow;
   size_t cap_off;
   u64 *tw = nullptr, *aw = nullptr, *wpt = nullptr, *qrows = nullptr;
@@ -171,6 +172,7 @@
   ws.alde = stream ? ws.ldechunk : lowmem ? ws.tvals : mem.words("alde", b.alde);
   ws.scr = mem.words("scratch", b.scratch);
   ws.quot = mem.words("quot", b.quot);
+  ws.qlook = mem.words("qlook", b.qlook);
   ws.tabs = mem.words("tabs", b.tabs);
   ws.open = mem.words("open", b.open);
   ws.fri = mem.words("fri", b.fri);
@@ -184,7 +186,7 @@
     sl.pinned_bytes = pl.pinned_bytes;
   }
   if (!ws.hist || !ws.in || !ws.tvals || !ws.tcoef || !ws.tmp || !ws.tlde || !ws.trees || !ws.avals || !ws.acoef || !ws.alde ||
-      !ws.scr || !ws.quot || !ws.tabs || !ws.open || !ws.fri || !ws.fritrees || !ws.qout || !ws.comb ||
+      !ws.scr || !ws.quot || !ws.qlook || !ws.tabs || !ws.open || !ws.fri || !ws.fritrees || !ws.qout || !ws.comb ||
       (stream && (!ws.ldechunk || !ws.sponge))) {
     err = mem.err;
     mem.release();
@@ -361,8 +363,8 @@
       });
       quotient_point_tables_window(ws.wpt, ws.wpt + WROWS, ws.wpt + 2 * WROWS, pl.log_n, h, k0, WROWS, st);
       QArgs QA;
-      quotient_fill_args(QA, pl.sh, nullptr, nullptr, ws.W, ws.mzt, r.pt, betas, gammas, pl.log_n, ws.qv, ws.qpart);
-      quotient_window_args(QA, ws.tw, ws.aw, wpt, ws.qpart, WROWS, BK, k0, h);
+      quotient_fill_args(QA, pl.sh, nullptr, nullptr, ws.W, ws.mzt, r.pt, betas, gammas, pl.log_n, ws.qv, ws.qpart, ws.qlook);
+      quotient_window_args(QA, ws.tw, ws.aw, wpt, ws.qpart, ws.qlook, WROWS, BK, k0, h);
       stark_kind(pl.kind).quotient_launch(QA, pl.sh, st);
     }
 }
@@ -388,7 +390,7 @@
     BigSection big(r.c, st, BIG_EXCL);
     r.sb(ST_QUOTIENT);
     QArgs QA;
-    quotient_fill_args(QA, pl.sh, ws.tlde, ws.alde, ws.W, ws.mzt, r.pt, betas, gammas, pl.log_n, ws.qv, ws.qpart);
+    quotient_fill_args(QA, pl.sh, ws.tlde, ws.alde, ws.W, ws.mzt, r.pt, betas, gammas, pl.log_n, ws.qv, ws.qpart, ws.qlook);
     sk.quotient_launch(QA, pl.sh, st);
   }
   r.tf.quotient_coset_inverse(ws.qv, ws.ab);
diff --git a/plonky2_bn254_amd/csrc/quotient.h b/plonky2_bn254_amd/csrc/quotient.h
--- a/plonky2_bn254_amd/csrc/quotient.h
+++ b/plonky2_bn254_amd/csrc/quotient.h
@@ -4,8 +4,8 @@
 
 void quotient_point_tables(u64* d_x, u64* d_lfirst, u64* d_llast, unsigned log_n, hipStream_t st);
 void quotient_point_tables_window(u64* d_x, u64* d_lfirst, u64* d_llast, unsigned log_n, int h, size_t k0, size_t count, hipStream_t st);
-void quotient_window_args(QArgs& A, const u64* d_tw, const u64* d_aw, const QPointTables& pt, u64* d_part, size_t stride, size_t count,
-                          size_t k0, int h);
+void quotient_window_args(QArgs& A, const u64* d_tw, const u64* d_aw, const QPointTables& pt, u64* d_part, u64* d_look, size_t stride,
+                          size_t count, size_t k0, int h);
 int g1_quotient_mz_blocks(const int** e0);
 int g2_quotient_mz_blocks(const int** e0);
 int fq_quotient_mz_blocks(const int** e0);
diff --git a/plonky2_bn254_amd/csrc/quotient_common.h b/plonky2_bn254_amd/csrc/quotient_common.h
--- a/plonky2_bn254_amd/csrc/quotient_common.h
+++ b/plonky2_bn254_amd/csrc/quotient_common.h
@@ -110,19 +110,16 @@
   return (h << log_n) | bitrev32(k, log_n);
 }
 
-__device__ __forceinline__ void lookup_and_ctl_constraints(const StarkShape& sh, const u64* __restrict__ tl,
-                                                           const u64* __restrict__ al, size_t M2, size_t j, size_t jn,
-                                                           const u32* __restrict__ W3 , int e0,
-                                                           const u64 betas[2], const u64 gammas[2], u64 lfirst, u64 llast,
-                                                           u64 z_last, u64& tot0, u64& tot1) {
+template <class WP>
+__device__ __forceinline__ void lookup_helper_slice(const StarkShape& sh, const u64* __restrict__ tl, const u64* __restrict__ al,
+                                                    size_t M2, size_t j, WP W3 , int e0,
+                                                    const u64 betas[2], int ka, int kb, u64& tot0, u64& tot1) {
   const int m = sh.n_helpers(), n_rc = sh.n_rc();
-  int e = e0;
   AccW acc;
   accw_init(acc);
-  const u64 table = tl[(size_t)sh.table_col * M2 + j], freq = tl[(size_t)sh.freq_col * M2 + j];
   u64 hs[2] = {0, 0};
 #pragma unroll 4
-  for (int k = 0; k < m; k++) {
+  for (int k = ka; k < kb; k++) {
     u64 f0 = tl[(size_t)(sh.rc_begin + 2 * k) * M2 + j];
     bool two = (2 * k + 1) < n_rc;
     u64 f1 = two ? tl[(size_t)(sh.rc_begin + 2 * k + 1) * M2 + j] : 0;
@@ -142,16 +139,33 @@
       hs[ch] = gl_add(hs[ch], h);
     }
   }
+  const u64 table = tl[(size_t)sh.table_col * M2 + j];
+#pragma unroll
+  for (int ch = 0; ch < 2; ch++) {
+    u64 twc = gl_add(table, betas[ch]);
+    accw_mad(acc, gl_neg(gl_mul(hs[ch], twc)), W3 + 8 * (e0 + ch * (m + 2) + m + 1));
+  }
+  tot0 = acc3_red(acc.a0);
+  tot1 = acc3_red(acc.a1);
+}
+
+template <class WP>
+__device__ __forceinline__ void lookup_z_and_ctl_slice(const StarkShape& sh, const u64* __restrict__ tl, const u64* __restrict__ al,
+                                                       size_t M2, size_t j, size_t jn, WP W3, int e0, const u64 betas[2],
+                                                       const u64 gammas[2], u64 lfirst, u64 llast, u64 z_last, u64& tot0, u64& tot1) {
+  const int m = sh.n_helpers();
+  AccW acc;
+  accw_init(acc);
+  const u64 table = tl[(size_t)sh.table_col * M2 + j], freq = tl[(size_t)sh.freq_col * M2 + j];
 #pragma unroll
   for (int ch = 0; ch < 2; ch++) {
     u64 z = al[(size_t)(ch * (m + 1) + m) * M2 + j], nz = al[(size_t)(ch * (m + 1) + m) * M2 + jn];
     u64 twc = gl_add(table, betas[ch]);
-    u64 y = gl_sub(gl_mul(hs[ch], twc), freq);
     int ee = e0 + ch * (m + 2) + m;
     accw_mad(acc, gl_mul(z, lfirst), W3 + 8 * (ee));
-    accw_mad(acc, gl_sub(gl_mul(gl_sub(nz, z), twc), y), W3 + 8 * (ee + 1));
+    accw_mad(acc, gl_add(gl_mul(gl_sub(nz, z), twc), freq), W3 + 8 * (ee + 1));
   }
-  e = e0 + 2 * (m + 2);
+  int e = e0 + 2 * (m + 2);
   for (int ctl = 0; ctl < sh.n_ctl; ctl++) {
     u64 a0 = 0, a1 = 0;
     for (int mm = sh.ctl.ncols[ctl] - 1; mm >= 0; mm--) {
@@ -174,6 +188,6 @@
       e += 2;
     }
   }
-  tot0 = gl_add(tot0, acc3_red(acc.a0));
-  tot1 = gl_add(tot1, acc3_red(acc.a1));
+  tot0 = acc3_red(acc.a0);
+  tot1 = acc3_red(acc.a1);
 }
diff --git a/plonky2_bn254_amd/csrc/quotient_g1.hip b/plonky2_bn254_amd/csrc/quotient_g1.hip
--- a/plonky2_bn254_amd/csrc/quotient_g1.hip
+++ b/plonky2_bn254_amd/csrc/quotient_g1.hip
@@ -115,13 +115,22 @@
   }
 }
 
-__global__ __launch_bounds__(256) void k_quotient_finish(QArgs A, StarkShape sh) {
+__global__ __launch_bounds__(256) void k_quotient_lookups(QArgs A, StarkShape sh) {
   const size_t j = (size_t)blockIdx.x * blockDim.x + threadIdx.x;
   if (j >= A.count) return;
-  finish_point(A, sh, j);
-}
-void quotient_finish_launch(const QArgs& A, const StarkShape& sh, hipStream_t st) {
-  k_quotient_finish<<<(unsigned)((A.count + 255) / 256), 256, 0, st>>>(A, sh);
+  lookups_point(A, sh, j, blockIdx.y == 0 ? A.n_slices : (int)blockIdx.y - 1);
+}
+void quotient_lookups_launch(const QArgs& A, const StarkShape& sh, hipStream_t st) {
+  k_quotient_lookups<<<dim3((unsigned)((A.count + 255) / 256), (unsigned)A.n_slices + 1), 256, 0, st>>>(A, sh);
+}
+
+__global__ __launch_bounds__(256) void k_quotient_finish(QArgs A) {
+  const size_t j = (size_t)blockIdx.x * blockDim.x + threadIdx.x;
+  if (j >= A.count) return;
+  finish_point(A, j);
+}
+void quotient_finish_launch(const QArgs& A, hipStream_t st) {
+  k_quotient_finish<<<(unsigned)((A.count + 255) / 256), 256, 0, st>>>(A);
 }
 
 __global__ void k_point_tables(u64* x, u64* lfirst, u64* llast, unsigned log_n, u64 w_n, u64 w_2n) {
@@ -161,12 +170,13 @@
   k_point_tables_window<<<(unsigned)((count + 255) / 256), 256, 0, st>>>(d_x, d_lfirst, d_llast, log_n, (u32)h, k0, count,
                                                                        gl_root_of_unity(log_n), gl_root_of_unity(log_n + 1));
 }
-void quotient_window_args(QArgs& A, const u64* d_tw, const u64* d_aw, const QPointTables& pt, u64* d_part, size_t stride, size_t count,
-                          size_t k0, int h) {
+void quotient_window_args(QArgs& A, const u64* d_tw, const u64* d_aw, const QPointTables& pt, u64* d_part, u64* d_look, size_t stride,
+                          size_t count, size_t k0, int h) {
   A.tl = d_tw;
   A.al = d_aw;
   A.pt = pt;
   A.part = d_part;
+  A.look = d_look;
   A.stride = stride;
   A.count = count;
   A.k0 = k0;
@@ -220,7 +230,7 @@
 
 void quotient_fill_args(QArgs& A, const StarkShape& sh, const u64* d_tl, const u64* d_al, const u64* d_W, const u64* d_mzt,
                         const QPointTables& pt, const u64 betas[2], const u64 gammas[2], unsigned log_n, u64* d_out,
-                        u64* d_part) {
+                        u64* d_part, u64* d_look) {
   A.tl = d_tl;
   A.al = d_al;
   A.W = d_W;
@@ -238,6 +248,8 @@
   A.out = d_out;
   A.part = d_part;
   A.n_parts = 0;
+  A.look = d_look;
+  A.n_slices = QUOTIENT_SLICES;
   A.log_n = log_n;
   A.K = sh.n_total_constraints();
   A.stride = A.count = 2 * N;
@@ -254,8 +266,9 @@
   QArgs A = A0;
   A.n_parts = 6;
   const unsigned g = (unsigned)((A.count + 255) / 256);
+  quotient_lookups_launch(A, sh, st);
   k_quotient_g1_parts<<<dim3(g, 6), 256, 0, st>>>(A);
-  quotient_finish_launch(A, sh, st);
+  quotient_finish_launch(A, st);
 }
 
 void quotient_g1_module_warm() {
diff --git a/plonky2_bn254_amd/csrc/quotient_g2fq.hip b/plonky2_bn254_amd/csrc/quotient_g2fq.hip
--- a/plonky2_bn254_amd/csrc/quotient_g2fq.hip
+++ b/plonky2_bn254_amd/csrc/quotient_g2fq.hip
@@ -174,6 +174,7 @@
   QArgs A = A0;
   A.n_parts = 7;
   const unsigned g = (unsigned)((A.count + 255) / 256);
+  quotient_lookups_launch(A, sh, st);
   k_quotient_g2_add<0><<<g, 256, 0, st>>>(A);
   k_quotient_g2_add<5><<<g, 256, 0, st>>>(A);
   k_quotient_g2_add<1><<<g, 256, 0, st>>>(A);
@@ -181,15 +182,16 @@
   k_quotient_g2_add<3><<<g, 256, 0, st>>>(A);
   k_quotient_g2_add<4><<<g, 256, 0, st>>>(A);
   k_quotient_g2_sched<<<g, 256, 0, st>>>(A);
-  quotient_finish_launch(A, sh, st);
+  quotient_finish_launch(A, st);
 }
 void fq_quotient_launch(const QArgs& A0, const StarkShape& sh, hipStream_t st) {
   QArgs A = A0;
   A.n_parts = 2;
   const unsigned g = (unsigned)((A.count + 255) / 256);
+  quotient_lookups_launch(A, sh, st);
   k_quotient_fq_mul<<<g, 256, 0, st>>>(A);
   k_quotient_fq_sched<<<g, 256, 0, st>>>(A);
-  quotient_finish_launch(A, sh, st);
+  quotient_finish_launch(A, st);
 }
 
 void quotient_g2fq_module_warm() {
diff --git a/plonky2_bn254_amd/csrc/quotient_sched.h b/plonky2_bn254_amd/csrc/quotient_sched.h
--- a/plonky2_bn254_amd/csrc/quotient_sched.h
+++ b/plonky2_bn254_amd/csrc/quotient_sched.h
@@ -20,6 +20,8 @@
   u64* out;
   u64* part;
   int n_parts;
+  u64* look;
+  int n_slices;
   unsigned log_n;
   int K;
   size_t stride, count, k0;
@@ -226,19 +228,40 @@
   store_part(A, part, j, tot0, tot1);
 }
 
-__device__ __forceinline__ void finish_point(const QArgs& A, const StarkShape& sh, size_t j) {
+GL_HD void lookup_slice_range(int m, int n_slices, int slice, int& ka, int& kb) {
+  const int len = (m + n_slices - 1) / n_slices;
+  ka = slice * len < m ? slice * len : m;
+  kb = ka + len < m ? ka + len : m;
+}
+__device__ __forceinline__ void lookups_point(const QArgs& A, const StarkShape& sh, size_t j, int slice) {
+  const size_t M2 = A.stride;
+  const qc32 W3 = QCONST(u32, A.W + 2 * (size_t)A.K);
+  u64 tot0, tot1;
+  if (slice < A.n_slices) {
+    int ka, kb;
+    lookup_slice_range(sh.n_helpers(), A.n_slices, slice, ka, kb);
+    lookup_helper_slice(sh, A.tl, A.al, M2, j, W3, sh.n_constraints, A.betas, ka, kb, tot0, tot1);
+  } else {
+    const u64 x = A.pt.x[j], lfirst = A.pt.lfirst[j], llast = A.pt.llast[j];
+    lookup_z_and_ctl_slice(sh, A.tl, A.al, M2, j, q_next(A, j), W3, sh.n_constraints, A.betas, A.gammas, lfirst, llast,
+                           gl_sub(x, A.w_inv), tot0, tot1);
+  }
+  A.look[((size_t)slice * 2 + 0) * M2 + j] = tot0;
+  A.look[((size_t)slice * 2 + 1) * M2 + j] = tot1;
+}
+
+__device__ __forceinline__ void finish_point(const QArgs& A, size_t j) {
   const unsigned log_n = A.log_n;
   const size_t N = (size_t)1 << log_n, M2 = A.stride;
-  const size_t jn = q_next(A, j);
   u64 tot0 = 0, tot1 = 0;
   for (int p = 0; p < A.n_parts; p++) {
     tot0 = gl_add(tot0, A.part[((size_t)p * 2 + 0) * M2 + j]);
     tot1 = gl_add(tot1, A.part[((size_t)p * 2 + 1) * M2 + j]);
   }
-  const u64 x = A.pt.x[j], lfirst = A.pt.lfirst[j], llast = A.pt.llast[j];
-  const u64 z_last = gl_sub(x, A.w_inv);
-  lookup_and_ctl_constraints(sh, A.tl, A.al, M2, j, jn, (const u32*)(A.W + 2 * (size_t)A.K), sh.n_constraints, A.betas, A.gammas,
-                             lfirst, llast, z_last, tot0, tot1);
+  for (int s = 0; s <= A.n_slices; s++) {
+    tot0 = gl_add(tot0, A.look[((size_t)s * 2 + 0) * M2 + j]);
+    tot1 = gl_add(tot1, A.look[((size_t)s * 2 + 1) * M2 + j]);
+  }
   const size_t h = A.natural ? A.hsel : j >> log_n;
   const size_t k = A.natural ? A.k0 + j : (size_t)bitrev32((u32)(j & (N - 1)), log_n);
   A.out[(0 * 2 + h) * N + k] = gl_mul(tot0, A.zh_inv[h]);
@@ -248,6 +271,9 @@
 void quotient_host_tables(int K, const u64 alphas[2], const int* mz_e0, int n_blocks, std::vector<u64>& W, std::vector<u64>& mzt);
 void quotient_fill_args(QArgs& A, const StarkShape& sh, const u64* d_tl, const u64* d_al, const u64* d_W, const u64* d_mzt,
                         const QPointTables& pt, const u64 betas[2], const u64 gammas[2], unsigned log_n, u64* d_out,
-                        u64* d_part);
+                        u64* d_part, u64* d_look);
 static constexpr int QUOTIENT_MAX_PARTS = 7;
-void quotient_finish_launch(const QArgs& A, const StarkShape& sh, hipStream_t st);
+static constexpr int QUOTIENT_SLICES = 4;
+static inline size_t QUOTIENT_LOOK_WORDS(int n_slices, size_t stride) { return (size_t)(n_slices + 1) * 2 * stride; }
+void quotient_lookups_launch(const QArgs& A, const StarkShape& sh, hipStream_t st);
+void quotient_finish_launch(const QArgs& A, hipStream_t st);
diff --git a/plonky2_bn254_amd/csrc/quotient_selftest.hip b/plonky2_bn254_amd/csrc/quotient_selftest.hip
--- a/plonky2_bn254_amd/csrc/quotient_selftest.hip
+++ b/plonky2_bn254_amd/csrc/quotient_selftest.hip
@@ -12,14 +12,14 @@
 static constexpr int QS_LOG_MIN = 3, QS_LOG_WHOLE_MAX = 12, QS_LOG_WINDOW_MAX = 20;
 static constexpr size_t QS_STRIDE_MAX = 8192;
 static_assert(QUOTIENT_MAX_PARTS == BN254S_QS_MAX_PARTS, "the part buffer of bn254s_selftest_quotient");
+static_assert(QUOTIENT_SLICES <= BN254S_QS_MAX_SLICES, "the slice buffer of bn254s_selftest_quotient_lookups");
 
-extern "C" {
-
-int bn254s_selftest_quotient(bn254s_ctx* c, int kind, int log_n, int flags, int h, size_t k0, size_t count, size_t stride,
-                             const uint64_t* trace, const uint64_t* aux, const uint64_t alphas[2], const uint64_t betas[2],
-                             const uint64_t gammas[2], const uint64_t* x, const uint64_t* lfirst, const uint64_t* llast, uint64_t* out,
-                             uint64_t* part) {
+static int qs_run(bn254s_ctx* c, int kind, int log_n, int flags, int h, size_t k0, size_t count, size_t stride, const uint64_t* trace,
+                  const uint64_t* aux, const uint64_t alphas[2], const uint64_t betas[2], const uint64_t gammas[2], const uint64_t* x,
+                  const uint64_t* lfirst, const uint64_t* llast, int n_slices, uint64_t* out, uint64_t* part, uint64_t* look,
+                  int* slices_out, int* ranges) {
   if (!c || !trace || !aux || !alphas || !betas || !gammas || !out || !part) return BN254S_E_INVALID_ARG;
+  if (n_slices < 0 || n_slices > BN254S_QS_MAX_SLICES) return BN254S_E_INVALID_ARG;
   if (kind < 0 || kind > 2 || (flags & ~(BN254S_QS_WINDOW | BN254S_QS_RAW))) return BN254S_E_INVALID_ARG;
   const bool window = flags & BN254S_QS_WINDOW, raw = flags & BN254S_QS_RAW;
   if (log_n < QS_LOG_MIN || log_n > (window ? QS_LOG_WINDOW_MAX : QS_LOG_WHOLE_MAX)) return BN254S_E_INVALID_ARG;
@@ -54,7 +54,9 @@
   u64* d_mzt = c->words("qs.mzt", hmzt.size());
   u64* d_out = c->words("qs.out", 4 * N);
   u64* d_part = c->words("qs.part", pw);
-  if (!d_tl || !d_al || !d_pt || !d_W || !d_mzt || !d_out || !d_part) return BN254S_E_OOM;
+  const size_t lw = QUOTIENT_LOOK_WORDS(BN254S_QS_MAX_SLICES, stride);
+  u64* d_look = c->words("qs.look", lw);
+  if (!d_tl || !d_al || !d_pt || !d_W || !d_mzt || !d_out || !d_part || !d_look) return BN254S_E_OOM;
   hipStream_t st = c->stream;
   HIP_TRY(c, hipMemcpyAsync(d_tl, trace, 8 * W * stride, hipMemcpyHostToDevice, st));
   HIP_TRY(c, hipMemcpyAsync(d_al, aux, 8 * A * stride, hipMemcpyHostToDevice, st));
@@ -62,6 +64,7 @@
   HIP_TRY(c, hipMemcpyAsync(d_mzt, hmzt.data(), 8 * hmzt.size(), hipMemcpyHostToDevice, st));
   HIP_TRY(c, hipMemcpyAsync(d_out, out, 8 * 4 * N, hipMemcpyHostToDevice, st));
   HIP_TRY(c, hipMemcpyAsync(d_part, part, 8 * pw, hipMemcpyHostToDevice, st));
+  if (look) HIP_TRY(c, hipMemcpyAsync(d_look, look, 8 * lw, hipMemcpyHostToDevice, st));
   QPointTables pt;
   pt.x = d_pt;
   pt.lfirst = d_pt + count;
@@ -76,8 +79,12 @@
     quotient_point_tables(d_pt, d_pt + count, d_pt + 2 * count, (unsigned)log_n, st);
   }
   QArgs QA;
-  quotient_fill_args(QA, sh, d_tl, d_al, d_W, d_mzt, pt, betas, gammas, (unsigned)log_n, d_out, d_part);
-  if (window) quotient_window_args(QA, d_tl, d_al, pt, d_part, stride, count, k0, h);
+  quotient_fill_args(QA, sh, d_tl, d_al, d_W, d_mzt, pt, betas, gammas, (unsigned)log_n, d_out, d_part, d_look);
+  if (window) quotient_window_args(QA, d_tl, d_al, pt, d_part, d_look, stride, count, k0, h);
+  if (n_slices) QA.n_slices = n_slices;
+  if (slices_out) *slices_out = QA.n_slices;
+  if (ranges)
+    for (int y = 0; y < QA.n_slices; y++) lookup_slice_range(sh.n_helpers(), QA.n_slices, y, ranges[2 * y], ranges[2 * y + 1]);
   if (raw) {
     QA.zh_inv[0] = QA.zh_inv[1] = 1;
     QA.w_inv = 0;
@@ -86,8 +93,28 @@
   HIP_TRY(c, hipGetLastError());
   HIP_TRY(c, hipMemcpyAsync(out, d_out, 8 * 4 * N, hipMemcpyDeviceToHost, st));
   HIP_TRY(c, hipMemcpyAsync(part, d_part, 8 * pw, hipMemcpyDeviceToHost, st));
+  if (look) HIP_TRY(c, hipMemcpyAsync(look, d_look, 8 * lw, hipMemcpyDeviceToHost, st));
   HIP_TRY(c, hipStreamSynchronize(st));
   return BN254S_OK;
+}
+
+extern "C" {
+
+int bn254s_selftest_quotient(bn254s_ctx* c, int kind, int log_n, int flags, int h, size_t k0, size_t count, size_t stride,
+                             const uint64_t* trace, const uint64_t* aux, const uint64_t alphas[2], const uint64_t betas[2],
+                             const uint64_t gammas[2], const uint64_t* x, const uint64_t* lfirst, const uint64_t* llast, uint64_t* out,
+                             uint64_t* part) {
+  return qs_run(c, kind, log_n, flags, h, k0, count, stride, trace, aux, alphas, betas, gammas, x, lfirst, llast, 0, out, part, nullptr,
+                nullptr, nullptr);
+}
+
+int bn254s_selftest_quotient_lookups(bn254s_ctx* c, int kind, int log_n, int flags, int h, size_t k0, size_t count, size_t stride,
+                                     const uint64_t* trace, const uint64_t* aux, const uint64_t alphas[2], const uint64_t betas[2],
+                                     const uint64_t gammas[2], const uint64_t* x, const uint64_t* lfirst, const uint64_t* llast,
+                                     int n_slices, uint64_t* out, uint64_t* part, uint64_t* look, int* slices, int* ranges) {
+  if (!look || !slices || !ranges) return BN254S_E_INVALID_ARG;
+  return qs_run(c, kind, log_n, flags, h, k0, count, stride, trace, aux, alphas, betas, gammas, x, lfirst, llast, n_slices, out, part,
+                look, slices, ranges);
 }
 
 int bn254s_selftest_point_tables(bn254s_ctx* c, int log_n, int window, int h, size_t k0, size_t count, uint64_t* out) {
diff --git a/plonky2_bn254_amd/csrc/verify.hip b/plonky2_bn254_amd/csrc/verify.hip
--- a/plonky2_bn254_amd/csrc/verify.hip
+++ b/plonky2_bn254_amd/csrc/verify.hip
@@ -69,7 +69,8 @@
   u64* d_mzt = c->words("vf_mzt", hmzt.size());
   u64* d_out = c->words("vf_out", 4 * N);
   u64* d_part = c->words("vf_part", (size_t)QUOTIENT_MAX_PARTS * 2 * M2);
-  if (!d_tl || !d_al || !d_pt || !d_W || !d_mzt || !d_out || !d_part) {
+  u64* d_look = c->words("vf_look", QUOTIENT_LOOK_WORDS(QUOTIENT_SLICES, M2));
+  if (!d_tl || !d_al || !d_pt || !d_W || !d_mzt || !d_out || !d_part || !d_look) {
     err = c->BufPool::err;
     return BN254S_E_OOM;
   }
@@ -85,7 +86,7 @@
   pt.lfirst = d_pt + M2;
   pt.llast = d_pt + 2 * M2;
   QArgs QA;
-  quotient_fill_args(QA, sh, d_tl, d_al, d_W, d_mzt, pt, betas, gammas, VLOG, d_out, d_part);
+  quotient_fill_args(QA, sh, d_tl, d_al, d_W, d_mzt, pt, betas, gammas, VLOG, d_out, d_part, d_look);
   QA.zh_inv[0] = QA.zh_inv[1] = 1;
   QA.w_inv = 0;
   stark_kind(kind).quotient_launch(QA, sh, st);
diff --git a/plonky2_bn254_amd/lib.py b/plonky2_bn254_amd/lib.py
--- a/plonky2_bn254_amd/lib.py
+++ b/plonky2_bn254_amd/lib.py
@@ -149,6 +149,9 @@
         lib.bn254s_selftest_quotient.argtypes = [vp, C.c_int, C.c_int, C.c_int, C.c_int, C.c_size_t, C.c_size_t, C.c_size_t, vp, vp,
                                                  vp, vp, vp, vp, vp, vp, vp, vp]
         lib.bn254s_selftest_point_tables.argtypes = [vp, C.c_int, C.c_int, C.c_int, C.c_size_t, C.c_size_t, vp]
+    if hasattr(lib, "bn254s_selftest_quotient_lookups"):
+        lib.bn254s_selftest_quotient_lookups.argtypes = [vp, C.c_int, C.c_int, C.c_int, C.c_int, C.c_size_t, C.c_size_t, C.c_size_t,
+                                                         vp, vp, vp, vp, vp, vp, vp, vp, C.c_int, vp, vp, vp, vp, vp]
         lib.bn254s_selftest_aux.argtypes = [vp, C.c_int, vp, C.c_size_t, vp, vp, vp]
     if hasattr(lib, "bn254s_selftest_proof_plan"):
         lib.bn254s_selftest_proof_plan.argtypes = [C.c_int, C.c_size_t, C.POINTER(Params), C.c_uint64, C.c_int, C.c_int, C.c_int,
@@ -709,10 +712,11 @@
 
     STARK_SHAPES = {0: (781, 456, 1111, 1573), 1: (1295, 906, 1693, 2605), 2: (427, 134, 770, 910)}
     QS_MAX_PARTS = 7
+    QS_MAX_SLICES = 32
     QS_N_PARTS = {0: 6, 1: 7, 2: 2}
 
     def selftest_quotient(self, kind: int, log_n: int, trace: np.ndarray, aux: np.ndarray, alphas, betas, gammas, raw: bool = False,
-                          window=None, tables=None, fill: int = 0):
+                          window=None, tables=None, fill: int = 0, slices=None):
         w, a, _, _ = self.STARK_SHAPES[kind]
         trace = np.ascontiguousarray(trace, dtype=np.uint64)
         aux = np.ascontiguousarray(aux, dtype=np.uint64)
@@ -730,6 +734,17 @@
             assert all(t.shape == (want,) for t in tabs), [t.shape for t in tabs]
         out = np.full((2, 2, n), fill, np.uint64)
         part = np.full((self.QS_MAX_PARTS, 2, stride), fill, np.uint64)
+        if slices is not None:
+            look = np.full((self.QS_MAX_SLICES + 1, 2, stride), fill, np.uint64)
+            n_sl = C.c_int(0)
+            ranges = np.zeros((self.QS_MAX_SLICES, 2), np.int32)
+            self._check(self._lib.bn254s_selftest_quotient_lookups(
+                self._h, kind, log_n, flags, h, k0, count, stride if window is not None else 0, _ptr(trace), _ptr(aux), _ptr(ch[0]),
+                _ptr(ch[1]), _ptr(ch[2]), _ptr(tabs[0]), _ptr(tabs[1]), _ptr(tabs[2]), int(slices), _ptr(out), _ptr(part), _ptr(look),
+                C.byref(n_sl), ranges.ctypes.data_as(C.c_void_p)), "bn254s_selftest_quotient_lookups")
+            s_ = n_sl.value
+            assert (look[s_ + 1:] == np.uint64(fill)).all(), "slice rows above S were written"
+            return out, part, look[:s_ + 1], ranges[:s_]
         self._check(self._lib.bn254s_selftest_quotient(self._h, kind, log_n, flags, h, k0, count, stride if window is not None else 0,
                                                        _ptr(trace), _ptr(aux), _ptr(ch[0]), _ptr(ch[1]), _ptr(ch[2]), _ptr(tabs[0]),
                                                        _ptr(tabs[1]), _ptr(tabs[2]), _ptr(out), _ptr(part)), "bn254s_selftest_quotient")
```
